# deryrahman/image-caption-emotion-indonesia

Measured on NVIDIA B200. Metric: decoder_train_tokens_per_sec, higher is better.
Workload: dtype bf16

## Files before the change

### image-caption-emotion-indonesia_b200/_lib.py

```python
import ctypes
import os
from ctypes import c_char_p, c_double, c_float, c_int32, c_int64, c_uint64, c_void_p

HERE = os.path.dirname(os.path.abspath(__file__))
LIB_PATH = os.path.join(HERE, "libsn100.so")

OP_NT, OP_NN, OP_TN = 0, 1, 2
CELL_FACTORED, CELL_LSTM = 0, 1

_P = c_void_p
_I32, _I64, _F, _D = c_int32, c_int64, c_float, c_double

SIGNATURES = {
    "sn_version": (_I32, []),
    "sn_last_error": (c_char_p, []),
    "sn_device_info": (_I32, [_P, _P, _P, _P]),
    "sn_gather_pack_fwd": (_I32, [_P, _I64, _P, _I64, _P, _I64, _I32, _P, _P, _P, _I64, _P, _I64, _F, c_uint64, _P, _P, _I64, _P]),
    "sn_gather_pack_bwd": (_I32, [_P, _I64, _P, _I64, _P, _I64, _I32, _P, _P, _P, _I64, _P, _I64, _F, c_uint64, _P, _I64, _P, _P, _P]),
    "sn_gemm": (_I32, [_I32, _I64, _I64, _I64, _P, _I64, _P, _I64, _P, _I64, _P, _F, _I32, _I64, _I64, _I64, _I64, _P]),
    "sn_gemm_bf16": (_I32, [_I32, _I64, _I64, _I64, _P, _I64, _P, _I64, _P, _I64, _P, _I64, _P, _F, _I32, _I64, _I64, _I64, _I64, _I64, _P]),
    "sn_gemm_bf16_splitk": (_I32, [_I32, _I64, _I64, _I64, _P, _I64, _P, _I64, _P, _I64, _P, _I64, _P, _F, _I32, _I64, _I64, _I64, _I64, _I64, _I32, _P]),
    "sn_gemm2_ws_bytes": (_I64, [_I64, _I64, _I32, _I32]),
    "sn_gemm2_bf16": (_I32, [_I32, _I64, _I64, _I64, _P, _I64, _P, _I64, _P, _I64, _P, _I64, _P, _F, _I32, _I64, _I64, _I64, _I64, _I64, _I32, _P, _I64, _I32, _P]),
    "sn_vocab_ws_bytes": (_I64, [_I64, _I64]),
    "sn_vocab_nll_fwd": (_I32, [_I64, _I64, _I64, _P, _I64, _P, _I64, _P, _P, _P, _I64, _P, _P, _P, _P, _P, _P]),
    "sn_vocab_nll_bwd": (_I32, [_I64, _I64, _I64, _P, _I64, _P, _I64, _P, _P, _P, _P, _F, _P, _P, _I64, _P, _P, _P]),
    "sn_cast_bf16": (_I32, [_P, _I64, _I64, _I64, _P, _I64, _I64, _P]),
    "sn_cast_bf16_ex": (_I32, [_P, _I64, _I64, _I64, _P, _I64, _I64, _I32, _P]),
    "sn_colsum": (_I32, [_P, _I64, _I64, _I64, _P, _F, _P]),
    "sn_colsum_ex": (_I32, [_P, _I64, _I64, _I64, _P, _F, _I32, _P]),
    "sn_colsum_bf16_ex": (_I32, [_P, _I64, _I64, _I64, _P, _F, _I32, _P]),
    "sn_embed_plan": (_I32, [_P, _I64, _I32, _P, _P, _P, _I64, _I64, _P, _P]),
    "sn_embed_grad": (_I32, [_P, _I64, _P, _I64, _I32, _P, _P, _P, _I64, _P, _I64, _F, c_uint64, _P, _I64, _P, _P, _I32, _P]),
    "sn_adam_clamp_dev_ex": (_I32, [_P, _P, _P, _P, _I32, _P, _P, _P, _P, _P, _F, _F, _F, _F, _I32, _P]),
    "sn_recur_ws_bytes": (_I64, [_I64, _I64]),
    "sn_recur_fwd": (_I32, [_I32, _I64, _I64, _P, _P, _I32, _I32, _P, _P, _P, _P, _P, _P, _P, _P, _P, _P, _P]),
    "sn_recur_bwd": (_I32, [_I32, _I64, _I64, _P, _P, _I32, _I32, _P, _P, _P, _P, _P, _P, _P, _P, _P, _P]),
    "sn_recur_fwd_bf16": (_I32, [_I32, _I64, _I64, _P, _P, _I32, _I32] + [_P] * 12),
    "sn_recur_bwd_bf16": (_I32, [_I32, _I64, _I64, _P, _P, _I32, _I32] + [_P] * 11),
    "sn_recur_cl_max_clusters": (_I32, [_I64]),
    "sn_recur_fwd_cl": (_I32, [_I32, _I64, _I64, _P, _P, _I32, _I32] + [_P] * 11),
    "sn_recur_bwd_cl": (_I32, [_I32, _I64, _I64, _P, _P, _I32, _I32] + [_P] * 11),
    "sn_gate_wait": (_I32, [_P, _I64, _P]),
    "sn_cast_bf16_gate_interleave": (_I32, [_P, _I64, _I64, _I64, _P, _I64, _P]),
    "sn_recur_fwd_gemm": (_I32, [_I32, _I64, _I64, _P, _P, _I32, _P, _P, _P, _P, _P, _P, _P, _P, _P]),
    "sn_recur_hprev": (_I32, [_P, _P, _P, _P, _I64, _I64, _P, _P]),
    "sn_recur_bwd_gemm": (_I32, [_I32, _I64, _I64, _P, _P, _I32, _P, _P, _P, _P, _P, _P, _P, _P, _P]),
    "sn_softmax_nll": (_I32, [_P, _I64, _I64, _I64, _P, _P, _P, _I64, _F, _P, _P, _P, _P, _I64, _P]),
    "sn_colsum_bf16": (_I32, [_P, _I64, _I64, _I64, _P, _F, _P]),
    "sn_reduce_sum": (_I32, [_P, _I64, _F, _P, _P, _I32, _P]),
    "sn_adam_clamp": (_I32, [_P, _P, _P, _P, _I32, _P, _P, _P, _F, _F, _F, _F, _P]),
    "sn_adam_clamp_dev": (_I32, [_P, _P, _P, _P, _I32, _P, _P, _P, _P, _P, _F, _F, _F, _F, _P]),
    "sn_enable_peer_access": (_I32, [_I32]),
    "sn_ipc_export": (_I32, [_P, _P, _P]),
    "sn_ipc_open": (_I32, [_P, _P]),
    "sn_ipc_close": (_I32, [_P]),
    "sn_dp_adam_fused": (_I32, [_I32, _I32, _P, _P, _P, _P, _P, _I32, _P, _P, _P, _P, _P, _F, _F, _F, _F, _P]),
    "sn_dp_slot_elems": (_I64, [_I64, _I32]),
    "sn_dp_push": (_I32, [_I32, _I32, _P, _P, _I64, _I32, _P, _I32, _P, _I32, _P]),
    "sn_dp_adam_recv": (_I32, [_I32, _I32, _P, _P, _P, _I64, _I32, _P, _P, _I32, _P, _P, _I32, _P, _P, _P, _P, _P, _F, _F, _F, _F, _I32, _P]),
    "sn_att_step_fwd": (_I32, [_P, _P, _P, _P, _F, _P, _I64, _I64, _I64, _I64, _P, _I64, _P, _I64, _P]),
    "sn_att_step_bwd": (_I32, [_P, _P, _P, _P, _F, _P, _P, _I64, _P, _I64, _P, _I64, _I64, _I64, _I64, _I64, _P, _P, _P, _P, _P, _P]),
    "sn_att_step_fwd_b16": (_I32, [_P, _P, _P, _P, _F, _P, _I64, _I64, _I64, _I64, _P, _I64, _P, _I64, _P]),
    "sn_att_step_bwd_b16": (_I32, [_P, _P, _P, _P, _P, _P, _I64, _P, _I64, _P, _I64, _I64, _I64, _I64, _I64, _P, _P, _P, _P, _P]),
    "sn_mean_pixels": (_I32, [_P, _I64, _I64, _I64, _P, _P]),
    "sn_beam_split_ws_floats": (_I64, [_I32, _I32, _I32]),
    "sn_beam_step_split": (_I32, [_P, _I64, _I64, _I32, _I32, _I32, _I32, _I32] + [_P] * 14 + [_I32, _P, _I32, _P]),
    "sn_split_limbs_cols": (_I32, [_P, _I64, _I64, _I64, _I64, _P, _I64, _I32, _P]),
    "sn_split_limbs_rows": (_I32, [_P, _I64, _I64, _I64, _I64, _P, _I64, _I64, _I32, _P]),
    "sn_skinny_max_rows": (_I32, []),
    "sn_skinny_linear": (_I32, [_P, _I64, _I64, _I64, _P, _I64, _I64, _I64, _I64, _P, _P, _I64, _P, _P]),
    "sn_decode_cell": (_I32, [_I32, _I64, _I64, _P, _I64, _I64, _P, _I64, _I64, _P, _P, _P, _P, _P, _P, _P, _P, _P, _P]),
    "sn_decode_cell_groups": (_I32, [_I32, _I64, _I64, _P, _I64, _P, _I64, _I64, _I64, _P, _I64, _I64, _P, _I64, _P, _P,
                                     _P, _P, _P, _P, _P, _P, _P]),
    "sn_pool_nhwc_fwd": (_I32, [_P, _I64, _I64, _I64, _I64, _I64, _P, _P, _P, _P]),
    "sn_pool_nhwc_bwd": (_I32, [_P, _I64, _I64, _I64, _I64, _I64, _P, _P]),
    "sn_bn1d_fwd": (_I32, [_P, _I64, _I64, _P, _P, _P, _P, _F, _F, _I32, _P, _P, _P, _P]),
    "sn_bn1d_bwd": (_I32, [_P, _P, _I64, _I64, _P, _P, _P, _I32, _P, _P, _P, _P]),
    "sn_beam_step": (_I32, [_P, _I64, _I64, _I32, _I32, _I32, _I32, _I32] + [_P] * 15),
    "sn_bleu_counts": (_I32, [_P, _P, _I64, _P, _P, _P, _I32, _I64, _P, _P]),
    "sn_cider_df": (_I32, [_P, _P, _P, _I64, _I32, _I32, _I64, _P, _P, _I64, _P, _P]),
    "sn_cider_scores": (_I32, [_P, _P, _I64, _P, _P, _P, _I32, _D, _I32, _I64, _P, _P, _I64, _P, _P, _P]),
    "sn_cider_scores_rows": (_I32, [_P, _I64, _P, _I64, _I32, _P, _I64, _P, _P, _P, _I32, _D, _I32, _I64, _P, _P, _I64,
                                    _P, _P]),
    "sn_rouge_l": (_I32, [_P, _P, _I64, _P, _P, _P, _I32, _D, _P, _P]),
    "sn_rouge_l_rows": (_I32, [_P, _I64, _P, _I64, _I32, _P, _I64, _P, _P, _P, _I32, _D, _P, _P]),
    "sn_sample_step": (_I32, [_P, _I64, _I64, _I32, _I32, _I32, _D, _I32] + [_P] * 9),
}

_lib = None


def load():
    global _lib
    if _lib is not None:
        return _lib
    if not os.path.exists(LIB_PATH):
        raise RuntimeError(
            "libsn100.so is not built (%s). Run `python -c 'import __graft_entry__ as g; g.build()'`; "
# ... 31 lines not shown
```

### image-caption-emotion-indonesia_b200/csrc/sn_common.cu

```cuda
#include <stdlib.h>

#include "sn_common.cuh"

#include <cuda.h>

#include <mutex>
#include <string.h>

namespace sn {

char* err_buf() {
  static thread_local char buf[512] = {0};
  return buf;
}

int32_t fail(int32_t code, const char* fmt, ...) {
  va_list ap;
  va_start(ap, fmt);
  vsnprintf(err_buf(), 512, fmt, ap);
  va_end(ap);
  return code;
}

int32_t check_launch(const char* what) {
  cudaError_t e = cudaGetLastError();
  if (e != cudaSuccess) return fail((int32_t)e, "%s: %s", what, cudaGetErrorString(e));
  return 0;
}

static DevInfo g_info[64];
static std::once_flag g_once[64];

const DevInfo& dev_info() {
  int dev = 0;
  cudaGetDevice(&dev);
  if (dev < 0 || dev >= 64) dev = 0;
  std::call_once(g_once[dev], [dev]() {
    DevInfo& d = g_info[dev];
    cudaDeviceGetAttribute(&d.sm_count, cudaDevAttrMultiProcessorCount, dev);
    cudaDeviceGetAttribute(&d.smem_optin, cudaDevAttrMaxSharedMemoryPerBlockOptin, dev);
    cudaDeviceGetAttribute(&d.cc_major, cudaDevAttrComputeCapabilityMajor, dev);
    cudaDeviceGetAttribute(&d.cc_minor, cudaDevAttrComputeCapabilityMinor, dev);
  });
  return g_info[dev];
}

}

namespace sn {
bool recur_cooperative() {
  static const bool coop = [] {
    const char* e = getenv("SN_RECUR_COOP");
    return e && e[0] == '1';
  }();
  return coop;
}
}

extern "C" {

int32_t sn_version(void) { return SN_VERSION; }
const char* sn_last_error(void) { return sn::err_buf(); }

int32_t sn_device_info(int32_t* sm_count, int32_t* smem_optin, int32_t* cc_major, int32_t* cc_minor) {
  int n = 0;
  cudaError_t e = cudaGetDeviceCount(&n);
  if (e != cudaSuccess || n == 0) return sn::fail(e ? (int32_t)e : -2, "no CUDA device (libsn100 has no CPU fallback)");
  const sn::DevInfo& d = sn::dev_info();
  if (sm_count) *sm_count = d.sm_count;
  if (smem_optin) *smem_optin = d.smem_optin;
  if (cc_major) *cc_major = d.cc_major;
  if (cc_minor) *cc_minor = d.cc_minor;
  if (d.cc_major != 10) return sn::fail(-3, "device is sm_%d%d; libsn100 is built for sm_100a only", d.cc_major, d.cc_minor);
  return 0;
}

int32_t sn_ipc_export(const void* ptr, uint8_t* handle64, int64_t* offset) {
  SN_REQUIRE(ptr && handle64 && offset, "sn_ipc_export: null argument");
  CUdeviceptr base = 0;
  size_t size = 0;
  typedef CUresult (*RangeFn)(CUdeviceptr*, size_t*, CUdeviceptr);
  static RangeFn range_fn = nullptr;
  if (!range_fn) {
    void* fp = nullptr;
    cudaDriverEntryPointQueryResult q;
    if (cudaGetDriverEntryPoint("cuMemGetAddressRange", &fp, cudaEnableDefault, &q) != cudaSuccess || !fp)
      return sn::fail(-6, "cuMemGetAddressRange entry point not available");
    range_fn = (RangeFn)fp;
  }
  CUresult r = range_fn(&base, &size, (CUdeviceptr)ptr);
  if (r != CUDA_SUCCESS) return sn::fail(-6, "cuMemGetAddressRange failed (%d)", (int)r);
  cudaIpcMemHandle_t h;
  cudaError_t e = cudaIpcGetMemHandle(&h, (void*)base);
  if (e != cudaSuccess) return sn::fail((int32_t)e, "cudaIpcGetMemHandle: %s (expandable segments are not IPC-exportable)", cudaGetErrorString(e));
  memcpy(handle64, &h, sizeof(h));
  *offset = (int64_t)((CUdeviceptr)ptr - base);
  return 0;
}

int32_t sn_ipc_open(const uint8_t* handle64, void** base_out) {
  SN_REQUIRE(handle64 && base_out, "sn_ipc_open: null argument");
  cudaIpcMemHandle_t h;
  memcpy(&h, handle64, sizeof(h));
  cudaError_t e = cudaIpcOpenMemHandle(base_out, h, cudaIpcMemLazyEnablePeerAccess);
  if (e != cudaSuccess) return sn::fail((int32_t)e, "cudaIpcOpenMemHandle: %s", cudaGetErrorString(e));
  return 0;
}

int32_t sn_ipc_close(void* base) {
  cudaError_t e = cudaIpcCloseMemHandle(base);
  if (e != cudaSuccess) return sn::fail((int32_t)e, "cudaIpcCloseMemHandle: %s", cudaGetErrorString(e));
  return 0;
}

}
```

### image-caption-emotion-indonesia_b200/csrc/sn_common.cuh

```cuda
#pragma once
#include <cuda_runtime.h>
#include <stdint.h>
#include <stdio.h>
#include <stdarg.h>

#include "../../include/sn100.h"

namespace sn {

char* err_buf();
int32_t fail(int32_t code, const char* fmt, ...);
int32_t check_launch(const char* what);

struct DevInfo {
  int sm_count;
  int smem_optin;
  int cc_major, cc_minor;
};
const DevInfo& dev_info();
bool recur_cooperative();

#define SN_REQUIRE(cond, ...)                         \
  do {                                                \
    if (!(cond)) return sn::fail(-1, __VA_ARGS__);    \
  } while (0)

#define SN_CUDA(expr)                                                           \
  do {                                                                          \
    cudaError_t e__ = (expr);                                                   \
    if (e__ != cudaSuccess)                                                     \
      return sn::fail((int32_t)e__, "%s: %s", #expr, cudaGetErrorString(e__));  \
  } while (0)

__device__ __forceinline__ float sigmoidf_(float x) { return 1.0f / (1.0f + expf(-x)); }

__device__ __forceinline__ float warp_sum(float v) {
#pragma unroll
  for (int o = 16; o > 0; o >>= 1) v += __shfl_xor_sync(0xffffffffu, v, o);
  return v;
}
__device__ __forceinline__ float warp_max(float v) {
#pragma unroll
  for (int o = 16; o > 0; o >>= 1) v = fmaxf(v, __shfl_xor_sync(0xffffffffu, v, o));
  return v;
}

__device__ __forceinline__ uint32_t hash_u32(uint64_t seed, uint32_t row, uint32_t col) {
  uint64_t x = seed ^ ((uint64_t)row << 32 | col);
  x ^= x >> 33; x *= 0xff51afd7ed558ccdULL;
  x ^= x >> 33; x *= 0xc4ceb9fe1a85ec53ULL;
  x ^= x >> 33;
  return (uint32_t)x;
}
__device__ __forceinline__ float dropout_scale(uint64_t seed, uint32_t row, uint32_t col, float p,
                                               float inv_keep) {
  if (p <= 0.f) return 1.f;
  float u = (hash_u32(seed, row, col) >> 8) * (1.0f / 16777216.0f);
  return u >= p ? inv_keep : 0.f;
}

__device__ __forceinline__ int ld_acquire(const int* p) {
  int v;
  asm volatile("ld.acquire.gpu.global.s32 %0, [%1];" : "=r"(v) : "l"(p) : "memory");
  return v;
}
__device__ __forceinline__ void red_release_add(int* p, int v) {
  asm volatile("red.release.gpu.global.add.s32 [%0], %1;" ::"l"(p), "r"(v) : "memory");
}

}
```

### image-caption-emotion-indonesia_b200/csrc/sn_elementwise.cu

```cuda
#include <stdlib.h>
#include <string.h>
#include <cuda_bf16.h>

#include "sn_common.cuh"

namespace {

__global__ void gather_pack_fwd_kernel(const int64_t* __restrict__ captions, int64_t cap_ld,
                                       const float* __restrict__ table, int E,
                                       const float* __restrict__ features, int64_t feat_ld, int has_feat,
                                       const int32_t* __restrict__ row_b, const int32_t* __restrict__ row_t,
                                       const int32_t* __restrict__ tok_override, int64_t N,
                                       float* __restrict__ X, int64_t ldx, float p, float inv_keep,
                                       uint64_t seed, const uint64_t* __restrict__ seed_dev,
                                       __nv_bfloat16* __restrict__ Xb, int64_t ldxb, int Ep) {
  if (seed_dev) seed += *seed_dev;
  int64_t row = (int64_t)blockIdx.x * (blockDim.x >> 5) + (threadIdx.x >> 5);
  if (row >= N) return;
  int lane = threadIdx.x & 31;
  int b = row_b[row], t = row_t[row];
  int ov = tok_override ? tok_override[row] : -1;
  float* dst = X ? X + row * ldx : nullptr;
  __nv_bfloat16* dstb = Xb ? Xb + row * ldxb : nullptr;
  const float* src;
  float pp = 0.f;
  if (ov < 0 && has_feat && t == 0) {
    src = features + (int64_t)b * feat_ld;
  } else {
    int64_t tok = ov >= 0 ? (int64_t)ov : captions[(int64_t)b * cap_ld + (t - has_feat)];
    src = table + tok * E;
    pp = ov >= 0 ? 0.f : p;
  }
  for (int c = lane; c < Ep; c += 32) {
    float v = c < E ? src[c] * sn::dropout_scale(seed, (uint32_t)row, (uint32_t)c, pp, inv_keep) : 0.f;
    if (dst && c < E) dst[c] = v;
    if (dstb) dstb[c] = __float2bfloat16(v);
  }
}

__global__ void gather_pack_bwd_kernel(const int64_t* __restrict__ captions, int64_t cap_ld,
                                       float* __restrict__ dtable, int E, float* __restrict__ dfeatures,
                                       int64_t feat_ld, int has_feat, const int32_t* __restrict__ row_b,
                                       const int32_t* __restrict__ row_t,
                                       const int32_t* __restrict__ tok_override, int64_t N,
                                       const float* __restrict__ dX, int64_t ldx, float p, float inv_keep,
                                       uint64_t seed, const uint64_t* __restrict__ seed_dev) {
  if (seed_dev) seed += *seed_dev;
  int64_t row = (int64_t)blockIdx.x * (blockDim.x >> 5) + (threadIdx.x >> 5);
  if (row >= N) return;
  int lane = threadIdx.x & 31;
  int b = row_b[row], t = row_t[row];
  int ov = tok_override ? tok_override[row] : -1;
  const float* src = dX + row * ldx;
  if (ov < 0 && has_feat && t == 0) {
    if (dfeatures) {
      float* dst = dfeatures + (int64_t)b * feat_ld;
      for (int c = lane; c < E; c += 32) dst[c] = src[c];
    }
    return;
  }
}

__device__ __forceinline__ int64_t packed_token(int64_t i, const int64_t* __restrict__ captions, int64_t cap_ld,
                                                int has_feat, const int32_t* __restrict__ row_b,
                                                const int32_t* __restrict__ row_t,
                                                const int32_t* __restrict__ tok_override) {
  int ov = tok_override ? tok_override[i] : -1;
  if (ov >= 0) return ov;
  int t = row_t[i];
  if (has_feat && t == 0) return -1;
  return captions[(int64_t)row_b[i] * cap_ld + (t - has_feat)];
}

constexpr int EB_CHUNK = 32;
constexpr int EB_K = 16;

__global__ void embed_count_kernel(const int64_t* __restrict__ captions, int64_t cap_ld, int has_feat,
                                   const int32_t* __restrict__ row_b, const int32_t* __restrict__ row_t,
                                   const int32_t* __restrict__ tok_override, int64_t N, int32_t* __restrict__ tok32,
                                   int32_t* __restrict__ cnt) {
  const int64_t r = (int64_t)blockIdx.x * blockDim.x + threadIdx.x;
  if (r >= N) return;
  const int64_t t = packed_token(r, captions, cap_ld, has_feat, row_b, row_t, tok_override);
  tok32[r] = (int32_t)t;
  if (t >= 0) atomicAdd(cnt + t, 1);
}

__global__ void __launch_bounds__(1024) embed_scan_kernel(const int32_t* __restrict__ cnt, int64_t V,
                                                          int32_t* __restrict__ start, int32_t* __restrict__ cursor,
                                                          int32_t* __restrict__ cstart) {
  __shared__ int32_t s1[1024], s2[1024];
  const int tid = threadIdx.x;
  const int64_t per = (V + 1023) / 1024, lo = tid * per, hi = lo + per < V ? lo + per : V;
  int32_t a = 0, c = 0;
  for (int64_t v = lo; v < hi; ++v) {
    const int32_t n = cnt[v];
    a += n;
    c += n > EB_CHUNK ? (n + EB_CHUNK - 1) / EB_CHUNK : 0;
// ... 3 lines not shown
  for (int off = 1; off < 1024; off <<= 1) {
    const int32_t x = tid >= off ? s1[tid - off] : 0, y = tid >= off ? s2[tid - off] : 0;
    __syncthreads();
    s1[tid] += x; s2[tid] += y;
    __syncthreads();
  }
  a = s1[tid] - a; c = s2[tid] - c;
  for (int64_t v = lo; v < hi; ++v) {
    const int32_t n = cnt[v];
    start[v] = a; cursor[v] = a; cstart[v] = c;
    a += n;
    c += n > EB_CHUNK ? (n + EB_CHUNK - 1) / EB_CHUNK : 0;
  }
  if (tid == 1023) start[V] = s1[1023];
}

__global__ void embed_place_kernel(const int32_t* __restrict__ tok32, int64_t N, int32_t* __restrict__ cursor,
                                   int32_t* __restrict__ perm) {
  const int64_t r = (int64_t)blockIdx.x * blockDim.x + threadIdx.x;
  if (r >= N) return;
  const int32_t t = tok32[r];
  if (t >= 0) perm[atomicAdd(cursor + t, 1)] = (int32_t)r;
}

__global__ void embed_order_kernel(const int32_t* __restrict__ tok32, const int32_t* __restrict__ start,
                                   const int32_t* __restrict__ perm, int64_t N, int64_t V,
                                   int32_t* __restrict__ sorted) {
  const int64_t i = (int64_t)blockIdx.x * blockDim.x + threadIdx.x;
  if (i >= start[V]) return;
  const int32_t r = perm[i], t = tok32[r], s = start[t], e = start[t + 1];
  int32_t rank = 0;
  for (int32_t j = s; j < e; ++j) rank += perm[j] < r;
  sorted[s + rank] = r;
}

__global__ void embed_chunk_kernel(const int32_t* __restrict__ tok32, const int32_t* __restrict__ start,
                                   const int32_t* __restrict__ cstart, const int32_t* __restrict__ sorted, int64_t V,
                                   const int32_t* __restrict__ tok_override, const float* __restrict__ dX, int64_t ldx,
                                   int E, float p, float inv_keep, uint64_t seed, const uint64_t* __restrict__ seed_dev,
                                   float* __restrict__ dtable, float* __restrict__ part) {
  if (seed_dev) seed += *seed_dev;
  const int64_t i = (int64_t)blockIdx.x * (blockDim.x >> 5) + (threadIdx.x >> 5);
  if (i >= start[V]) return;
  const int lane = threadIdx.x & 31;
  const int32_t t = tok32[sorted[i]], s = start[t], e = start[t + 1];
  if ((i - s) % EB_CHUNK) return;
  const int32_t n = (int32_t)(e - i < EB_CHUNK ? e - i : EB_CHUNK);
  const int32_t my = lane < n ? sorted[i + lane] : 0;
  float* dst = e - s <= EB_CHUNK ? dtable + (int64_t)t * E : part + (int64_t)(cstart[t] + (i - s) / EB_CHUNK) * E;
  for (int c0 = 0; c0 < E; c0 += 32 * EB_K) {
    float acc[EB_K];
#pragma unroll
    for (int k = 0; k < EB_K; ++k) acc[k] = 0.f;
    for (int q = 0; q < n; ++q) {
      const int64_t j = __shfl_sync(0xffffffffu, my, q);
      const float pp = (tok_override && tok_override[j] >= 0) ? 0.f : p;
      const float* src = dX + j * ldx;
#pragma unroll
      for (int k = 0; k < EB_K; ++k) {
        const int c = c0 + k * 32 + lane;
        if (c < E) {
          const float sc = sn::dropout_scale(seed, (uint32_t)j, (uint32_t)c, pp, inv_keep);
          if (sc != 0.f) acc[k] += src[c] * sc;
        }
      }
    }
#pragma unroll
    for (int k = 0; k < EB_K; ++k) {
      const int c = c0 + k * 32 + lane;
      if (c < E) {
        if (e - s <= EB_CHUNK) dst[c] += acc[k];
        else dst[c] = acc[k];
      }
    }
  }
}

constexpr int EBW_BATCH = 16;
__global__ void __launch_bounds__(512) embed_chunk_wide_kernel(
    const int32_t* __restrict__ tok32, const int32_t* __restrict__ start, const int32_t* __restrict__ cstart,
    const int32_t* __restrict__ sorted, int64_t V, const int32_t* __restrict__ tok_override,
    const float* __restrict__ dX, int64_t ldx, int E, float p, float inv_keep, uint64_t seed,
    const uint64_t* __restrict__ seed_dev, float* __restrict__ dtable, float* __restrict__ part) {
  __shared__ int32_t rows[EB_CHUNK];
  __shared__ float rate[EB_CHUNK];
  const int64_t i = blockIdx.x;
  if (i >= start[V]) return;
  const int32_t t = tok32[sorted[i]], s = start[t], e = start[t + 1];
  if ((i - s) % EB_CHUNK) return;
  if (seed_dev) seed += *seed_dev;
  const int32_t n = (int32_t)(e - i < EB_CHUNK ? e - i : EB_CHUNK);
  if (threadIdx.x < n) {
    const int32_t j = sorted[i + threadIdx.x];
    rows[threadIdx.x] = j;
    rate[threadIdx.x] = (tok_override && tok_override[j] >= 0) ? 0.f : p;
  }
  __syncthreads();
  const int c = threadIdx.x;
  if (c >= E) return;
  float acc = 0.f;
  for (int q0 = 0; q0 < n; q0 += EBW_BATCH) {
    float x[EBW_BATCH], sc[EBW_BATCH];
#pragma unroll
    for (int u = 0; u < EBW_BATCH; ++u) {
      const int q = q0 + u;
      x[u] = 0.f; sc[u] = 0.f;
      if (q < n) {
        const int64_t j = rows[q];
        x[u] = dX[j * ldx + c];
        sc[u] = sn::dropout_scale(seed, (uint32_t)j, (uint32_t)c, rate[q], inv_keep);
      }
    }
#pragma unroll
    for (int u = 0; u < EBW_BATCH; ++u)
      if (sc[u] != 0.f) acc = __fmaf_rn(x[u], sc[u], acc);
  }
  if (e - s <= EB_CHUNK) dtable[(int64_t)t * E + c] += acc;
  else part[(int64_t)(cstart[t] + (i - s) / EB_CHUNK) * E + c] = acc;
}

__global__ void embed_combine_kernel(const int32_t* __restrict__ cnt, const int32_t* __restrict__ cstart, int64_t V,
                                     int E, const float* __restrict__ part, float* __restrict__ dtable) {
  const int64_t t = (int64_t)blockIdx.x * (blockDim.x >> 5) + (threadIdx.x >> 5);
  if (t >= V || cnt[t] <= EB_CHUNK) return;
  const int lane = threadIdx.x & 31;
  const int32_t nq = (cnt[t] + EB_CHUNK - 1) / EB_CHUNK;
  const float* src = part + (int64_t)cstart[t] * E;
  for (int c = lane; c < E; c += 32) {
    float a = 0.f;
    for (int32_t q = 0; q < nq; ++q) a += src[(int64_t)q * E + c];
    dtable[t * E + c] += a;
  }
}

__global__ void __launch_bounds__(256) softmax_nll_kernel(const float* __restrict__ logits, int64_t V, int64_t ld,
                                                          const int64_t* __restrict__ targets,
                                                          float* __restrict__ row_loss, float* dlogits, int64_t ldd,
                                                          float grad_scale, const float* __restrict__ row_weight,
                                                          int64_t* __restrict__ argmax,
                                                          int32_t* __restrict__ top5hit, int use_smem,
                                                          __nv_bfloat16* __restrict__ dlb, int64_t lddb) {
  extern __shared__ float srow[];
  __shared__ float red_v[8];
  __shared__ int red_i[8];
  __shared__ float bc_f[2];
  __shared__ int bc_i;
  const int64_t row = blockIdx.x;
  const float* src = logits + row * ld;
  const int tid = threadIdx.x, lane = tid & 31, warp = tid >> 5;

  float mx = -INFINITY;
  int mi = 0x7fffffff;
  for (int64_t c = tid; c < V; c += 256) {
    float v = src[c];
    if (use_smem) srow[c] = v;
    if (v > mx) { mx = v; mi = (int)c; }
  }
#pragma unroll
  for (int o = 16; o > 0; o >>= 1) {
    float ov = __shfl_xor_sync(0xffffffffu, mx, o);
    int oi = __shfl_xor_sync(0xffffffffu, mi, o);
    if (ov > mx || (ov == mx && oi < mi)) { mx = ov; mi = oi; }
  }
  if (lane == 0) { red_v[warp] = mx; red_i[warp] = mi; }
  __syncthreads();
  if (tid == 0) {
    float bm = red_v[0]; int bi = red_i[0];
    for (int w = 1; w < 8; ++w)
      if (red_v[w] > bm || (red_v[w] == bm && red_i[w] < bi)) { bm = red_v[w]; bi = red_i[w]; }
    bc_f[0] = bm; bc_i = bi;
  }
  __syncthreads();
  mx = bc_f[0];
  if (tid == 0 && argmax) argmax[row] = bc_i;
  if (!targets) return;

  const float* rd = use_smem ? srow : src;
  const int64_t tgt = targets[row];
  const float tv = rd[tgt];
  float se = 0.f;
  int above = 0;
  for (int64_t c = tid; c < V; c += 256) {
    float v = rd[c];
    se += expf(v - mx);
    above += (v > tv);
  }
  se = sn::warp_sum(se);
#pragma unroll
  for (int o = 16; o > 0; o >>= 1) above += __shfl_xor_sync(0xffffffffu, above, o);
  __syncthreads();
  if (lane == 0) { red_v[warp] = se; red_i[warp] = above; }
  __syncthreads();
  if (tid == 0) {
    float s = 0.f; int a = 0;
    for (int w = 0; w < 8; ++w) { s += red_v[w]; a += red_i[w]; }
    float lse = mx + logf(s);
    bc_f[1] = lse;
    if (row_loss) row_loss[row] = lse - tv;
    if (top5hit) top5hit[row] = a < 5 ? 1 : 0;
  }
  __syncthreads();
  if (dlogits || dlb) {
    const float lse = bc_f[1];
    const float gs = row_weight ? grad_scale * row_weight[row] : grad_scale;
    float* dst = dlogits ? dlogits + row * ldd : nullptr;
    __nv_bfloat16* dstb = dlb ? dlb + row * lddb : nullptr;
    for (int64_t c = tid; c < V; c += 256) {
      float pr = expf(rd[c] - lse);
      float gr = (pr - (c == tgt ? 1.f : 0.f)) * gs;
      if (dst) dst[c] = gr;
      if (dstb) dstb[c] = __float2bfloat16(gr);
    }
    if (dstb) for (int64_t c = V + tid; c < lddb; c += 256) dstb[c] = __float2bfloat16(0.f);
  }
}

__global__ void __launch_bounds__(1024) reduce_sum_kernel(const float* __restrict__ x, int64_t N, float scale,
                                                           const float* __restrict__ w, float* out, int accumulate) {
  __shared__ double part[32];
  double s = 0.0;
  if (w)
    for (int64_t i = threadIdx.x; i < N; i += 1024) s += (double)x[i] * (double)w[i];
  else
    for (int64_t i = threadIdx.x; i < N; i += 1024) s += (double)x[i];
#pragma unroll
  for (int o = 16; o > 0; o >>= 1) s += __shfl_xor_sync(0xffffffffu, s, o);
  if ((threadIdx.x & 31) == 0) part[threadIdx.x >> 5] = s;
  __syncthreads();
  if (threadIdx.x == 0) {
    double t = 0.0;
    for (int w = 0; w < 32; ++w) t += part[w];
    float r = (float)(t * (double)scale);
    *out = accumulate ? *out + r : r;
  }
}

struct AdamRanges {
  static constexpr int MAX = 128;
  int64_t off[MAX];
  int32_t len[MAX];
  float step_size[MAX], bc2_sqrt[MAX];
  int step_idx[MAX];
  int32_t chunk_start[MAX + 1];
  int n;
};
static_assert(sizeof(AdamRanges) <= 3700, "AdamRanges must leave room for the other kernel parameters below 4 KB");

__global__ void adam_prepare_kernel(AdamRanges R, int32_t* __restrict__ steps, const float* __restrict__ lr,
                                    float* __restrict__ coef, float beta1, float beta2) {
  int r = threadIdx.x;
  if (r >= R.n) return;
  int st = steps[R.step_idx[r]] + 1;
  steps[R.step_idx[r]] = st;
  double bc1 = 1.0 - pow((double)beta1, (double)st);
  double bc2 = 1.0 - pow((double)beta2, (double)st);
  coef[2 * R.step_idx[r]] = (float)((double)(*lr) / bc1);
  coef[2 * R.step_idx[r] + 1] = (float)sqrt(bc2);
}
constexpr int ADAM_CHUNK = 4096;
constexpr int64_t ADAM_MAX_LEN = (1LL << 31) - 2 * ADAM_CHUNK;

__global__ void __launch_bounds__(256) adam_clamp_kernel(float* __restrict__ p, float* __restrict__ g,
                                                         float* __restrict__ m, float* __restrict__ v,
                                                         AdamRanges R, const float* __restrict__ coef, float beta1,
                                                         float beta2, float eps, float clip) {
  const int64_t total_chunks = R.chunk_start[R.n];
  for (int64_t ch = blockIdx.x; ch < total_chunks; ch += gridDim.x) {
    int r = 0;
    while (ch >= R.chunk_start[r + 1]) ++r;
    const int64_t base = R.off[r] + (ch - R.chunk_start[r]) * ADAM_CHUNK;
    const int64_t end = R.off[r] + R.len[r];
    const float ss = coef ? coef[2 * R.step_idx[r]] : R.step_size[r], bc = coef ? coef[2 * R.step_idx[r] + 1] : R.bc2_sqrt[r];
    const int64_t lim = base + ADAM_CHUNK < end ? base + ADAM_CHUNK : end;
    if ((base & 3) == 0 && lim - base == ADAM_CHUNK) {
#pragma unroll
      for (int it = 0; it < ADAM_CHUNK / (256 * 4); ++it) {
        const int64_t i = base + (int64_t)(it * 256 + threadIdx.x) * 4;
        float4 g4 = *reinterpret_cast<const float4*>(g + i);
        float4 m4 = *reinterpret_cast<const float4*>(m + i);
        float4 v4 = *reinterpret_cast<const float4*>(v + i);
        float4 p4 = *reinterpret_cast<const float4*>(p + i);
        float* gp = &g4.x; float* mp = &m4.x; float* vp = &v4.x; float* pp = &p4.x;
#pragma unroll
        for (int e = 0; e < 4; ++e) {
          float gi = gp[e];
          if (clip > 0.f) gi = fminf(fmaxf(gi, -clip), clip);
          gp[e] = gi;
          float mi = mp[e] + (1.f - beta1) * (gi - mp[e]);
          float vi = vp[e] * beta2 + (1.f - beta2) * gi * gi;
          float denom = sqrtf(vi) / bc + eps;
          pp[e] = pp[e] - ss * (mi / denom);
          mp[e] = mi; vp[e] = vi;
        }
        if (clip > 0.f) *reinterpret_cast<float4*>(g + i) = g4;
        *reinterpret_cast<float4*>(m + i) = m4;
        *reinterpret_cast<float4*>(v + i) = v4;
        *reinterpret_cast<float4*>(p + i) = p4;
      }
      continue;
    }
    for (int64_t i = base + threadIdx.x; i < lim; i += 256) {
      float gi = g[i];
      if (clip > 0.f) { gi = fminf(fmaxf(gi, -clip), clip); g[i] = gi; }
      float mi = m[i], vi = v[i];
      mi = mi + (1.f - beta1) * (gi - mi);
      vi = vi * beta2 + (1.f - beta2) * gi * gi;
      float denom = sqrtf(vi) / bc + eps;
      p[i] = p[i] - ss * (mi / denom);
      m[i] = mi; v[i] = vi;
    }
  }
}

struct DpPeers {
  float* grad[8];
  float* param[8];
  int* pad[8];
  int world, rank;
  void* recv[8];
  int64_t slot_elems;
  int* wait_pad[4];
  int n_wait;
};
constexpr int PAD_ARRIVE = 0, PAD_DONE = 8, PAD_COUNTER = 16, PAD_EPOCH = 17, PAD_DONE_COUNTER = 18;

__device__ __forceinline__ int ld_acquire_sys(const int* p) {
  int v;
  asm volatile("ld.acquire.sys.global.s32 %0, [%1];" : "=r"(v) : "l"(p) : "memory");
  return v;
}
__device__ __forceinline__ void st_release_sys(int* p, int v) {
  asm volatile("st.release.sys.global.s32 [%0], %1;" ::"l"(p), "r"(v) : "memory");
}

constexpr int DP_SUB = 4;
template <typename TT>
__global__ void __launch_bounds__(256 * DP_SUB) dp_push_kernel(DpPeers P, AdamRanges R, const float* __restrict__ g) {
  const int W = P.world;
  __shared__ int s_last;
  int* mypad = P.pad[P.rank];
  const int64_t total_chunks = R.chunk_start[R.n];
  const int sub = threadIdx.x >> 8, tid = threadIdx.x & 255;
  for (int64_t ch = (int64_t)blockIdx.x * DP_SUB + sub; ch < total_chunks; ch += (int64_t)gridDim.x * DP_SUB) {
    int r = 0;
    while (ch >= R.chunk_start[r + 1]) ++r;
    const int64_t aid = R.off[r] / ADAM_CHUNK + (ch - R.chunk_start[r]);
    const int owner = (int)(aid % W);
    if (owner == P.rank) continue;
// ... 204 lines not shown
#pragma unroll
        for (int k = 0; k < 4; ++k) {
          float gi = gp[k];
          if (clip > 0.f) gi = fminf(fmaxf(gi, -clip), clip);
          const float mi = mp[k] + (1.f - beta1) * (gi - mp[k]);
          const float vi = vp[k] * beta2 + (1.f - beta2) * gi * gi;
          pp[k] = pp[k] - ss * (mi / (sqrtf(vi) / bc + eps));
          mp[k] = mi; vp[k] = vi;
        }
        *reinterpret_cast<float4*>(m + i) = m4;
        *reinterpret_cast<float4*>(v + i) = v4;
#pragma unroll
        for (int q = 0; q < W; ++q) *reinterpret_cast<float4*>(P.param[q] + i) = p4;
      }
      continue;
    }
    for (int64_t i = base + tid; i < lim; i += 256) {
      float gi = 0.f;
#pragma unroll
      for (int q = 0; q < W; ++q) {
        float gq;
        if (q == rank) gq = __ldcg(g + i);
        else if constexpr (sizeof(TT) == 4) gq = __ldcg(recv + q * P.slot_elems + rbase + i);
        else gq = __bfloat162float(recv[q * P.slot_elems + rbase + i]);
        gi = q == 0 ? gq : gi + gq;
      }
      if (clip > 0.f) gi = fminf(fmaxf(gi, -clip), clip);
      const float mi = m[i] + (1.f - beta1) * (gi - m[i]);
      const float vi = v[i] * beta2 + (1.f - beta2) * gi * gi;
      const float pn = p_loc[i] - ss * (mi / (sqrtf(vi) / bc + eps));
      m[i] = mi; v[i] = vi;
#pragma unroll
      for (int q = 0; q < W; ++q) P.param[q][i] = pn;
    }
  }
  __syncthreads();
  if (threadIdx.x == 0) {
    __threadfence_system();
    s_last = (atomicAdd(mypad + PAD_DONE_COUNTER, 1) == (int)gridDim.x - 1);
  }
  __syncthreads();
  if (s_last) {
    if (threadIdx.x == 0) __threadfence_system();
    __syncthreads();
    if (threadIdx.x < W) {
      st_release_sys(P.pad[threadIdx.x] + PAD_DONE + rank, e);
      while (ld_acquire_sys(mypad + PAD_DONE + threadIdx.x) < e) { }
    }
    __syncthreads();
    if (threadIdx.x == 0) {
      mypad[PAD_DONE_COUNTER] = 0; mypad[PAD_EPOCH] = e;
      for (int k = 1; k < P.n_wait; ++k) P.wait_pad[k][PAD_EPOCH] = P.wait_pad[k][PAD_EPOCH] + 1;
    }
  }
}

__global__ void mean_pixels_kernel(const float* __restrict__ feat, int64_t P, int64_t D, float* __restrict__ out) {
  int64_t b = blockIdx.y;
  int64_t d = (int64_t)blockIdx.x * blockDim.x + threadIdx.x;
  if (d >= D) return;
  const float* src = feat + b * P * D + d;
  float s = 0.f;
  for (int64_t pz = 0; pz < P; ++pz) s += src[pz * D];
  out[b * D + d] = s / (float)P;
}

}

extern "C" {

int32_t sn_gather_pack_fwd(const int64_t* captions, int64_t cap_ld, const float* table, int64_t E,
                           const float* features, int64_t feat_ld, int32_t has_feat,
                           const int32_t* row_b, const int32_t* row_t, const int32_t* tok_override,
                           int64_t N, float* X, int64_t ldx, float p_drop, uint64_t seed, const uint64_t* seed_dev,
                           void* Xb, int64_t ldxb, void* stream) {
  SN_REQUIRE(N >= 0 && E > 0 && (X || Xb), "sn_gather_pack_fwd: bad dims N=%lld E=%lld", (long long)N, (long long)E);
  SN_REQUIRE(!X || ldx >= E, "sn_gather_pack_fwd: ldx=%lld < E", (long long)ldx);
  SN_REQUIRE(!Xb || ldxb >= E, "sn_gather_pack_fwd: ldxb=%lld < E", (long long)ldxb);
  SN_REQUIRE(p_drop >= 0.f && p_drop < 1.f, "sn_gather_pack_fwd: dropout p=%f out of [0,1)", p_drop);
  SN_REQUIRE(!has_feat || features, "sn_gather_pack_fwd: has_feat without features");
  if (N == 0) return 0;
  float inv_keep = 1.f / (1.f - p_drop);
  unsigned grid = (unsigned)((N + 7) / 8);
  gather_pack_fwd_kernel<<<grid, 256, 0, (cudaStream_t)stream>>>(captions, cap_ld, table, (int)E, features, feat_ld,
                                                                 has_feat, row_b, row_t, tok_override, N, X, ldx,
                                                                 p_drop, inv_keep, seed, seed_dev,
                                                                 (__nv_bfloat16*)Xb, ldxb, Xb ? (int)ldxb : (int)E);
  return sn::check_launch("sn_gather_pack_fwd");
}

int32_t sn_gather_pack_bwd(const int64_t* captions, int64_t cap_ld, float* dtable, int64_t E,
                           float* dfeatures, int64_t feat_ld, int32_t has_feat, const int32_t* row_b,
                           const int32_t* row_t, const int32_t* tok_override, int64_t N,
                           const float* dX, int64_t ldx, float p_drop, uint64_t seed, const uint64_t* seed_dev,
                           int64_t V, int32_t* ws_int, float* ws_part, void* stream) {
  SN_REQUIRE(N >= 0 && E > 0 && ldx >= E && V > 0, "sn_gather_pack_bwd: bad dims");
  SN_REQUIRE(p_drop >= 0.f && p_drop < 1.f, "sn_gather_pack_bwd: dropout p=%f out of [0,1)", p_drop);
  SN_REQUIRE(N < (int64_t)1 << 30, "sn_gather_pack_bwd: N=%lld rows", (long long)N);
  if (N == 0) return 0;
  SN_REQUIRE(ws_int && ws_part, "sn_gather_pack_bwd: null work space");
  if (int32_t rc = sn_embed_plan(captions, cap_ld, has_feat, row_b, row_t, tok_override, N, V, ws_int, stream)) return rc;
  return sn_embed_grad(dtable, E, dfeatures, feat_ld, has_feat, row_b, row_t, tok_override, N, dX, ldx, p_drop, seed,
                       seed_dev, V, ws_int, ws_part, 0, stream);
}

namespace {
struct EmbedWs {
  int32_t *cnt, *start, *cursor, *cstart, *tok32, *perm, *sorted;
  EmbedWs(int32_t* ws, int64_t V, int64_t N)
      : cnt(ws), start(cnt + V), cursor(start + V + 1), cstart(cursor + V), tok32(cstart + V), perm(tok32 + N),
        sorted(perm + N) {}
};
}

int32_t sn_embed_plan(const int64_t* captions, int64_t cap_ld, int32_t has_feat, const int32_t* row_b,
                      const int32_t* row_t, const int32_t* tok_override, int64_t N, int64_t V, int32_t* ws_int,
                      void* stream) {
  SN_REQUIRE(N >= 0 && N < (int64_t)1 << 30 && V > 0, "sn_embed_plan: bad dims N=%lld V=%lld", (long long)N, (long long)V);
  if (N == 0) return 0;
  SN_REQUIRE(ws_int, "sn_embed_plan: null work space");
  cudaStream_t st = (cudaStream_t)stream;
  EmbedWs w(ws_int, V, N);
  SN_CUDA(cudaMemsetAsync(w.cnt, 0, sizeof(int32_t) * (size_t)V, st));
  const unsigned g_rows = (unsigned)((N + 255) / 256);
  embed_count_kernel<<<g_rows, 256, 0, st>>>(captions, cap_ld, has_feat, row_b, row_t, tok_override, N, w.tok32, w.cnt);
  embed_scan_kernel<<<1, 1024, 0, st>>>(w.cnt, V, w.start, w.cursor, w.cstart);
  embed_place_kernel<<<g_rows, 256, 0, st>>>(w.tok32, N, w.cursor, w.perm);
  embed_order_kernel<<<g_rows, 256, 0, st>>>(w.tok32, w.start, w.perm, N, V, w.sorted);
  return sn::check_launch("sn_embed_plan");
}

int32_t sn_embed_grad(float* dtable, int64_t E, float* dfeatures, int64_t feat_ld, int32_t has_feat,
                      const int32_t* row_b, const int32_t* row_t, const int32_t* tok_override, int64_t N,
                      const float* dX, int64_t ldx, float p_drop, uint64_t seed, const uint64_t* seed_dev, int64_t V,
                      const int32_t* ws_int, float* ws_part, int32_t wide, void* stream) {
  SN_REQUIRE(N >= 0 && N < (int64_t)1 << 30 && E > 0 && ldx >= E && V > 0, "sn_embed_grad: bad dims");
  SN_REQUIRE(p_drop >= 0.f && p_drop < 1.f, "sn_embed_grad: dropout p=%f out of [0,1)", p_drop);
  if (N == 0) return 0;
  SN_REQUIRE(ws_int && ws_part, "sn_embed_grad: null work space");
  cudaStream_t st = (cudaStream_t)stream;
  float inv_keep = 1.f / (1.f - p_drop);
  if (has_feat && dfeatures)
    gather_pack_bwd_kernel<<<(unsigned)((N + 7) / 8), 256, 0, st>>>(nullptr, 0, dtable, (int)E, dfeatures,
                                                                     feat_ld, has_feat, row_b, row_t, tok_override, N,
                                                                     dX, ldx, p_drop, inv_keep, seed, seed_dev);
  EmbedWs w(const_cast<int32_t*>(ws_int), V, N);
  if (wide && E <= 512)
    embed_chunk_wide_kernel<<<(unsigned)N, (unsigned)((E + 31) / 32 * 32), 0, st>>>(
        w.tok32, w.start, w.cstart, w.sorted, V, tok_override, dX, ldx, (int)E, p_drop, inv_keep, seed, seed_dev,
        dtable, ws_part);
  else
    embed_chunk_kernel<<<(unsigned)((N + 7) / 8), 256, 0, st>>>(w.tok32, w.start, w.cstart, w.sorted, V, tok_override,
                                                                 dX, ldx, (int)E, p_drop, inv_keep, seed, seed_dev,
                                                                 dtable, ws_part);
  embed_combine_kernel<<<(unsigned)((V + 7) / 8), 256, 0, st>>>(w.cnt, w.cstart, V, (int)E, ws_part, dtable);
  return sn::check_launch("sn_embed_grad");
}

int32_t sn_softmax_nll(const float* logits, int64_t N, int64_t V, int64_t ld, const int64_t* targets,
                       float* row_loss, float* dlogits, int64_t ldd, float grad_scale, const float* row_weight,
                       int64_t* argmax, int32_t* top5hit, void* dlogits_bf16, int64_t lddb, void* stream) {
  SN_REQUIRE(N >= 0 && V > 0 && ld >= V, "sn_softmax_nll: bad dims");
  SN_REQUIRE(!dlogits_bf16 || lddb >= V, "sn_softmax_nll: lddb < V");
  if (N == 0) return 0;
  size_t smem = (size_t)V * sizeof(float);
  int use_smem = smem <= 200 * 1024;
  if (use_smem && smem > 48 * 1024) {
    static thread_local size_t configured = 0;
    if (configured < smem) {
      SN_CUDA(cudaFuncSetAttribute(softmax_nll_kernel, cudaFuncAttributeMaxDynamicSharedMemorySize, 200 * 1024));
      configured = 200 * 1024;
    }
  }
  softmax_nll_kernel<<<(unsigned)N, 256, use_smem ? smem : 0, (cudaStream_t)stream>>>(
      logits, V, ld, targets, row_loss, dlogits, ldd, grad_scale, row_weight, argmax, top5hit, use_smem,
      (__nv_bfloat16*)dlogits_bf16, lddb);
  return sn::check_launch("sn_softmax_nll");
}

int32_t sn_reduce_sum(const float* x, int64_t N, float scale, const float* row_weight, float* out, int32_t accumulate,
                      void* stream) {
  SN_REQUIRE(N >= 0 && out, "sn_reduce_sum: bad args");
  reduce_sum_kernel<<<1, 1024, 0, (cudaStream_t)stream>>>(x, N, scale, row_weight, out, accumulate);
  return sn::check_launch("sn_reduce_sum");
}

int32_t sn_adam_clamp(float* p, float* g, float* m, float* v, int32_t n_ranges, const int64_t* ranges,
                      const float* step_size, const float* bc2_sqrt, float beta1, float beta2, float eps,
                      float clip, void* stream) {
  SN_REQUIRE(n_ranges >= 0, "sn_adam_clamp: n_ranges < 0");
  int done = 0;
  while (done < n_ranges) {
    AdamRanges R;
    R.n = 0;
    R.chunk_start[0] = 0;
    while (done < n_ranges && R.n < AdamRanges::MAX) {
      int64_t off = ranges[2 * done], len = ranges[2 * done + 1];
      SN_REQUIRE(off >= 0 && len >= 0 && len < ADAM_MAX_LEN, "sn_adam_clamp: bad range %d", done);
      R.off[R.n] = off; R.len[R.n] = (int32_t)len;
      R.step_size[R.n] = step_size[done]; R.bc2_sqrt[R.n] = bc2_sqrt[done];
      R.chunk_start[R.n + 1] = R.chunk_start[R.n] + (len + ADAM_CHUNK - 1) / ADAM_CHUNK;
      ++R.n; ++done;
    }
    int64_t chunks = R.chunk_start[R.n];
    if (chunks == 0) continue;
    int64_t cap = (int64_t)sn::dev_info().sm_count * 8;
    unsigned grid = (unsigned)(chunks < cap ? chunks : cap);
    adam_clamp_kernel<<<grid, 256, 0, (cudaStream_t)stream>>>(p, g, m, v, R, nullptr, beta1, beta2, eps, clip);
    int32_t rc = sn::check_launch("sn_adam_clamp");
    if (rc) return rc;
  }
  return 0;
}

int32_t sn_adam_clamp_dev(float* p, float* g, float* m, float* v, int32_t n_ranges, const int64_t* ranges,
                          const int32_t* step_idx, int32_t* steps_dev, const float* lr_dev, float* coef_ws,
                          float beta1, float beta2, float eps, float clip, void* stream) {
  return sn_adam_clamp_dev_ex(p, g, m, v, n_ranges, ranges, step_idx, steps_dev, lr_dev, coef_ws, beta1, beta2, eps,
                              clip, 0, stream);
}

int32_t sn_adam_clamp_dev_ex(float* p, float* g, float* m, float* v, int32_t n_ranges, const int64_t* ranges,
                             const int32_t* step_idx, int32_t* steps_dev, const float* lr_dev, float* coef_ws,
                             float beta1, float beta2, float eps, float clip, int32_t max_ctas, void* stream) {
  SN_REQUIRE(max_ctas >= 0, "sn_adam_clamp_dev: max_ctas < 0");
  SN_REQUIRE(n_ranges >= 0 && n_ranges <= AdamRanges::MAX, "sn_adam_clamp_dev: at most %d ranges per call", AdamRanges::MAX);
  SN_REQUIRE(steps_dev && lr_dev && coef_ws, "sn_adam_clamp_dev: null argument");
  if (n_ranges == 0) return 0;
  AdamRanges R;
  R.n = n_ranges;
  R.chunk_start[0] = 0;
  for (int i = 0; i < n_ranges; ++i) {
    SN_REQUIRE(ranges[2 * i] >= 0 && ranges[2 * i + 1] >= 0 && ranges[2 * i + 1] < ADAM_MAX_LEN, "sn_adam_clamp_dev: bad range %d", i);
    R.off[i] = ranges[2 * i]; R.len[i] = (int32_t)ranges[2 * i + 1]; R.step_idx[i] = step_idx[i];
    R.step_size[i] = 0.f; R.bc2_sqrt[i] = 1.f;
    R.chunk_start[i + 1] = R.chunk_start[i] + (R.len[i] + ADAM_CHUNK - 1) / ADAM_CHUNK;
  }
  cudaStream_t st = (cudaStream_t)stream;
  adam_prepare_kernel<<<1, AdamRanges::MAX, 0, st>>>(R, steps_dev, lr_dev, coef_ws, beta1, beta2);
  int64_t chunks = R.chunk_start[R.n];
  if (chunks == 0) return sn::check_launch("sn_adam_clamp_dev");
  int64_t cap = (int64_t)sn::dev_info().sm_count * 8;
  if (max_ctas > 0 && max_ctas < cap) cap = max_ctas;
  unsigned grid = (unsigned)(chunks < cap ? chunks : cap);
  adam_clamp_kernel<<<grid, 256, 0, st>>>(p, g, m, v, R, coef_ws, beta1, beta2, eps, clip);
  return sn::check_launch("sn_adam_clamp_dev");
}

int32_t sn_enable_peer_access(int32_t peer_device) {
  int cur = 0;
  SN_CUDA(cudaGetDevice(&cur));
  if (peer_device == cur) return 0;
  int can = 0;
  SN_CUDA(cudaDeviceCanAccessPeer(&can, cur, peer_device));
  SN_REQUIRE(can, "sn_enable_peer_access: device %d cannot access peer %d", cur, peer_device);
  cudaError_t e = cudaDeviceEnablePeerAccess(peer_device, 0);
  if (e == cudaErrorPeerAccessAlreadyEnabled) { cudaGetLastError(); return 0; }
  if (e != cudaSuccess) return sn::fail((int32_t)e, "cudaDeviceEnablePeerAccess(%d): %s", peer_device, cudaGetErrorString(e));
  return 0;
}

int32_t sn_dp_adam_fused(int32_t world, int32_t rank, void* const* grad_ptrs, void* const* param_ptrs,
                         void* const* pad_ptrs, float* m, float* v, int32_t n_ranges, const int64_t* ranges,
                         const int32_t* step_idx, int32_t* steps_dev, const float* lr_dev, float* coef_ws, float beta1,
                         float beta2, float eps, float clip, void* stream) {
  SN_REQUIRE(world >= 1 && world <= 8 && rank >= 0 && rank < world, "sn_dp_adam_fused: bad world/rank %d/%d", world, rank);
  SN_REQUIRE(n_ranges >= 0 && n_ranges <= AdamRanges::MAX, "sn_dp_adam_fused: at most %d ranges per call", AdamRanges::MAX);
  SN_REQUIRE(grad_ptrs && param_ptrs && pad_ptrs && steps_dev && lr_dev && coef_ws && m && v, "sn_dp_adam_fused: null argument");
  DpPeers P;
  memset(&P, 0, sizeof(P));
  P.world = world; P.rank = rank;
  for (int q = 0; q < 8; ++q) {
    P.grad[q] = q < world ? (float*)grad_ptrs[q] : nullptr;
    P.param[q] = q < world ? (float*)param_ptrs[q] : nullptr;
    P.pad[q] = q < world ? (int*)pad_ptrs[q] : nullptr;
    SN_REQUIRE(q >= world || (P.grad[q] && P.param[q] && P.pad[q]), "sn_dp_adam_fused: null peer pointer %d", q);
  }
  AdamRanges R;
  R.n = n_ranges;
  R.chunk_start[0] = 0;
  for (int i = 0; i < n_ranges; ++i) {
    SN_REQUIRE(ranges[2 * i] >= 0 && ranges[2 * i + 1] >= 0 && ranges[2 * i + 1] < ADAM_MAX_LEN, "sn_dp_adam_fused: bad range %d", i);
    R.off[i] = ranges[2 * i]; R.len[i] = (int32_t)ranges[2 * i + 1]; R.step_idx[i] = step_idx[i];
    R.step_size[i] = 0.f; R.bc2_sqrt[i] = 1.f;
    R.chunk_start[i + 1] = R.chunk_start[i] +
        (R.len[i] > 0 ? (R.off[i] + R.len[i] - 1) / ADAM_CHUNK - R.off[i] / ADAM_CHUNK + 1 : 0);
  }
  cudaStream_t st = (cudaStream_t)stream;
  if (n_ranges > 0) adam_prepare_kernel<<<1, AdamRanges::MAX, 0, st>>>(R, steps_dev, lr_dev, coef_ws, beta1, beta2);
  int64_t mine = (R.chunk_start[R.n] + world - 1) / world;
  int64_t cap = (int64_t)sn::dev_info().sm_count * 3;
  unsigned grid = (unsigned)(mine < 1 ? 1 : (mine < cap ? mine : cap));
  static const int dbg = [] { const char* e = getenv("SN_DP_DEBUG"); return e ? atoi(e) : 0; }();
#define SN_DP_LAUNCH(WW) dp_adam_fused_kernel<WW><<<grid, 256, 0, st>>>(P, R, coef_ws, m, v, beta1, beta2, eps, clip, dbg)
  switch (world) {
    case 1: SN_DP_LAUNCH(1); break;
    case 2: SN_DP_LAUNCH(2); break;
    case 3: SN_DP_LAUNCH(3); break;
    case 4: SN_DP_LAUNCH(4); break;
    case 5: SN_DP_LAUNCH(5); break;
    case 6: SN_DP_LAUNCH(6); break;
    case 7: SN_DP_LAUNCH(7); break;
    default: SN_DP_LAUNCH(8); break;
  }
#undef SN_DP_LAUNCH
  return sn::check_launch("sn_dp_adam_fused");
}

static int32_t dp_fill_ranges(AdamRanges& R, int32_t n_ranges, const int64_t* ranges, const int32_t* step_idx, const char* who) {
  SN_REQUIRE(n_ranges >= 0 && n_ranges <= AdamRanges::MAX, "%s: at most %d ranges per call", who, AdamRanges::MAX);
  R.n = n_ranges;
  R.chunk_start[0] = 0;
  for (int i = 0; i < n_ranges; ++i) {
    SN_REQUIRE(ranges[2 * i] >= 0 && ranges[2 * i + 1] >= 0 && ranges[2 * i + 1] < ADAM_MAX_LEN, "%s: bad range %d", who, i);
    R.off[i] = ranges[2 * i]; R.len[i] = (int32_t)ranges[2 * i + 1]; R.step_idx[i] = step_idx ? step_idx[i] : 0;
    R.step_size[i] = 0.f; R.bc2_sqrt[i] = 1.f;
    R.chunk_start[i + 1] = R.chunk_start[i] +
        (R.len[i] > 0 ? (R.off[i] + R.len[i] - 1) / ADAM_CHUNK - R.off[i] / ADAM_CHUNK + 1 : 0);
  }
  return 0;
}

int64_t sn_dp_slot_elems(int64_t arena_elems, int32_t world) {
  if (arena_elems < 0 || world < 1) return -1;
  int64_t chunks = (arena_elems + ADAM_CHUNK - 1) / ADAM_CHUNK;
  return ((chunks + world - 1) / world) * ADAM_CHUNK;
}

int32_t sn_dp_push(int32_t world, int32_t rank, const float* grad, void* const* recv_ptrs, int64_t slot_elems,
                   int32_t elem_size, void* const* pad_ptrs, int32_t n_ranges, const int64_t* ranges, int32_t max_ctas,
                   void* stream) {
  SN_REQUIRE(world >= 1 && world <= 8 && rank >= 0 && rank < world, "sn_dp_push: bad world/rank %d/%d", world, rank);
  SN_REQUIRE(grad && recv_ptrs && pad_ptrs && ranges, "sn_dp_push: null argument");
  SN_REQUIRE(elem_size == 4 || elem_size == 2, "sn_dp_push: elem_size must be 4 (fp32) or 2 (bf16)");
  SN_REQUIRE(slot_elems > 0 && slot_elems % ADAM_CHUNK == 0, "sn_dp_push: slot_elems must be a positive multiple of %d", ADAM_CHUNK);
  DpPeers P;
  memset(&P, 0, sizeof(P));
  P.world = world; P.rank = rank; P.slot_elems = slot_elems;
  for (int q = 0; q < world; ++q) {
    P.recv[q] = recv_ptrs[q]; P.pad[q] = (int*)pad_ptrs[q];
    SN_REQUIRE(P.recv[q] && P.pad[q], "sn_dp_push: null peer pointer %d", q);
  }
  AdamRanges R;
  if (int32_t rc = dp_fill_ranges(R, n_ranges, ranges, nullptr, "sn_dp_push")) return rc;
  for (int i = 0; i < n_ranges; ++i)
    SN_REQUIRE(R.len[i] == 0 || (R.off[i] + R.len[i] - 1) / ADAM_CHUNK / world < slot_elems / ADAM_CHUNK,
               "sn_dp_push: range %d does not fit the receive slots", i);
  int64_t chunks = R.chunk_start[R.n];
  int64_t cap = (int64_t)sn::dev_info().sm_count;
  if (max_ctas > 0 && max_ctas < cap) cap = max_ctas;
  int64_t want = (chunks + DP_SUB - 1) / DP_SUB;
  unsigned grid = (unsigned)(want < 1 ? 1 : (want < cap ? want : cap));
  cudaStream_t st = (cudaStream_t)stream;
  if (elem_size == 4) dp_push_kernel<float><<<grid, 256 * DP_SUB, 0, st>>>(P, R, grad);
  else dp_push_kernel<__nv_bfloat16><<<grid, 256 * DP_SUB, 0, st>>>(P, R, grad);
  return sn::check_launch("sn_dp_push");
}

int32_t sn_dp_adam_recv(int32_t world, int32_t rank, float* grad, void* const* param_ptrs, void* recv, int64_t slot_elems,
                        int32_t elem_size, void* const* pad_ptrs, void* const* wait_pads, int32_t n_wait, float* m, float* v,
                        int32_t n_ranges, const int64_t* ranges, const int32_t* step_idx, int32_t* steps_dev,
                        const float* lr_dev, float* coef_ws, float beta1, float beta2, float eps, float clip,
                        int32_t max_ctas, void* stream) {
  SN_REQUIRE(world >= 1 && world <= 8 && rank >= 0 && rank < world, "sn_dp_adam_recv: bad world/rank %d/%d", world, rank);
  SN_REQUIRE(grad && param_ptrs && recv && pad_ptrs && wait_pads && steps_dev && lr_dev && coef_ws && m && v && ranges && step_idx,
             "sn_dp_adam_recv: null argument");
  SN_REQUIRE(elem_size == 4 || elem_size == 2, "sn_dp_adam_recv: elem_size must be 4 (fp32) or 2 (bf16)");
  SN_REQUIRE(n_wait >= 1 && n_wait <= 4, "sn_dp_adam_recv: 1..4 push buckets per call (got %d)", n_wait);
  SN_REQUIRE(slot_elems > 0 && slot_elems % ADAM_CHUNK == 0, "sn_dp_adam_recv: slot_elems must be a positive multiple of %d", ADAM_CHUNK);
  SN_REQUIRE(n_ranges >= 1, "sn_dp_adam_recv: no ranges");
  DpPeers P;
  memset(&P, 0, sizeof(P));
  P.world = world; P.rank = rank; P.slot_elems = slot_elems; P.n_wait = n_wait;
  for (int q = 0; q < world; ++q) {
    P.param[q] = (float*)param_ptrs[q]; P.pad[q] = (int*)pad_ptrs[q];
    SN_REQUIRE(P.param[q] && P.pad[q], "sn_dp_adam_recv: null peer pointer %d", q);
  }
  P.grad[rank] = grad;
  P.recv[rank] = recv;
  for (int k = 0; k < n_wait; ++k) {
    P.wait_pad[k] = (int*)wait_pads[k];
    SN_REQUIRE(P.wait_pad[k], "sn_dp_adam_recv: null wait pad %d", k);
  }
  SN_REQUIRE(P.wait_pad[0] == P.pad[rank], "sn_dp_adam_recv: pad_ptrs must be every rank's pad of wait bucket 0");
  AdamRanges R;
  if (int32_t rc = dp_fill_ranges(R, n_ranges, ranges, step_idx, "sn_dp_adam_recv")) return rc;
  for (int i = 0; i < n_ranges; ++i) {
    int64_t own = 0;
    if (R.len[i] > 0) {
      const int64_t a0 = R.off[i] / ADAM_CHUNK, a1 = (R.off[i] + R.len[i] - 1) / ADAM_CHUNK;
      const int64_t first = a0 + ((rank - a0) % world + world) % world;
      own = first <= a1 ? (a1 - first) / world + 1 : 0;
      SN_REQUIRE(a1 / world < slot_elems / ADAM_CHUNK, "sn_dp_adam_recv: range %d does not fit the receive slots", i);
    }
    R.chunk_start[i + 1] = R.chunk_start[i] + own;
  }
  cudaStream_t st = (cudaStream_t)stream;
  adam_prepare_kernel<<<1, AdamRanges::MAX, 0, st>>>(R, steps_dev, lr_dev, coef_ws, beta1, beta2);
  int64_t mine = (R.chunk_start[R.n] + DP_RSUB - 1) / DP_RSUB;
  int64_t cap = (int64_t)sn::dev_info().sm_count * 2;
  if (max_ctas > 0 && max_ctas < cap) cap = max_ctas;
  unsigned grid = (unsigned)(mine < 1 ? 1 : (mine < cap ? mine : cap));
  const float* p_loc = P.param[rank];
#define SN_DP_LAUNCH(WW)                                                                                                   \
  if (elem_size == 4) dp_recv_adam_kernel<WW, float><<<grid, 256 * DP_RSUB, 0, st>>>(P, R, coef_ws, grad, (const float*)recv, p_loc, m, v, beta1, beta2, eps, clip); \
  else dp_recv_adam_kernel<WW, __nv_bfloat16><<<grid, 256 * DP_RSUB, 0, st>>>(P, R, coef_ws, grad, (const __nv_bfloat16*)recv, p_loc, m, v, beta1, beta2, eps, clip)
  switch (world) {
    case 1: SN_DP_LAUNCH(1); break;
    case 2: SN_DP_LAUNCH(2); break;
    case 3: SN_DP_LAUNCH(3); break;
    case 4: SN_DP_LAUNCH(4); break;
    case 5: SN_DP_LAUNCH(5); break;
    case 6: SN_DP_LAUNCH(6); break;
    case 7: SN_DP_LAUNCH(7); break;
    default: SN_DP_LAUNCH(8); break;
  }
#undef SN_DP_LAUNCH
  return sn::check_launch("sn_dp_adam_recv");
}

int32_t sn_mean_pixels(const float* feat, int64_t B, int64_t P, int64_t D, float* out, void* stream) {
  SN_REQUIRE(B >= 0 && P > 0 && D > 0, "sn_mean_pixels: bad dims");
  if (B == 0) return 0;
  dim3 grid((unsigned)((D + 255) / 256), (unsigned)B);
  mean_pixels_kernel<<<grid, 256, 0, (cudaStream_t)stream>>>(feat, P, D, out);
  return sn::check_launch("sn_mean_pixels");
}

}
```

### image-caption-emotion-indonesia_b200/csrc/sn_gemm2.cu

```cuda
#include <cuda.h>
#include <cuda_bf16.h>
#include <math.h>
#include <math_constants.h>

#include "sn_common.cuh"

namespace {

constexpr int BMC = 128;
constexpr int BM = 2 * BMC;
constexpr int BN = 256;
constexpr int BK = 64;
constexpr int UMMA_K = 16;
constexpr int A_BYTES = BMC * BK * 2;
constexpr int ACC_STAGES = 2;
constexpr int EPI_WARPS = 16;
constexpr int NTHREADS = 64 + 32 * EPI_WARPS;
constexpr int XPOSE_BYTES = 32 * 32 * 4;
template <int BN_>
struct Geo {
  static constexpr int BNC = BN_ / 2;
  static constexpr int B_BYTES = BNC * BK * 2;
  static constexpr int STAGE_BYTES = A_BYTES + B_BYTES;
  static constexpr int STAGES = BN_ == 256 ? 5 : 6;
// ... 174 lines not shown
  __syncwarp();
  const int u = lane & 3;
  const int n8 = nb + 8 * u;
#pragma unroll
  for (int i = 0; i < 4; ++i) {
    const int r = 8 * i + (lane >> 2);
    const uint4 pk = *reinterpret_cast<const uint4*>(buf + r * 64 + ((u ^ ((r >> 1) & 3)) << 4));
    const int rr = row0 + r;
    if (rr >= M || n8 >= ncols) continue;
    __nv_bfloat16* dst = base + (int64_t)rr * ld + n8;
    if (vec_ok && n8 + 8 <= ncols) {
      *reinterpret_cast<uint4*>(dst) = pk;
    } else {
      const __nv_bfloat16* e = reinterpret_cast<const __nv_bfloat16*>(&pk);
#pragma unroll
      for (int k = 0; k < 8; ++k)
        if (n8 + k < ncols) dst[k] = e[k];
    }
  }
}

struct Tile { int m0, n0, grp, split, kb0, nkb; };

__device__ __forceinline__ Tile decode_tile(const G2Args& g, int tile, int tiles_m, int tiles_n, int total_kb, int bn) {
  Tile t;
  int mt, nt, rest;
  if (g.M > g.N) {
    nt = tile % tiles_n; rest = tile / tiles_n;
    mt = rest % tiles_m; rest /= tiles_m;
  } else {
    mt = tile % tiles_m; rest = tile / tiles_m;
    nt = rest % tiles_n; rest /= tiles_n;
  }
  t.split = rest % g.splits;
  t.grp = rest / g.splits;
  t.m0 = mt * BM;
  t.n0 = nt * bn;
  if (g.splits == 1) {
    t.kb0 = 0; t.nkb = total_kb;
  } else {
    t.kb0 = (total_kb * t.split) / g.splits;
    t.nkb = (total_kb * (t.split + 1)) / g.splits - t.kb0;
  }
  return t;
}


template <int EPI, int BN_>
__global__ void __cluster_dims__(2, 1, 1) __launch_bounds__(NTHREADS, 1)
gemm2_kernel(const __grid_constant__ TmaSet tma_a, const __grid_constant__ TmaSet tma_b, const G2Args g) {
  constexpr int BNC = Geo<BN_>::BNC, B_BYTES = Geo<BN_>::B_BYTES, STAGE_BYTES = Geo<BN_>::STAGE_BYTES;
  constexpr int STAGES = Geo<BN_>::STAGES, TMEM_COLS = Geo<BN_>::TMEM_COLS, EPI_COLS = Geo<BN_>::EPI_COLS;
  extern __shared__ uint8_t smem_raw[];
  uint8_t* smem = reinterpret_cast<uint8_t*>((reinterpret_cast<uintptr_t>(smem_raw) + 1023) & ~(uintptr_t)1023);
  float* xpose0 = reinterpret_cast<float*>(smem + STAGES * STAGE_BYTES);
  uint64_t* bars = reinterpret_cast<uint64_t*>(smem + STAGES * STAGE_BYTES + EPI_WARPS * XPOSE_BYTES);
  uint32_t* tmem_slot = reinterpret_cast<uint32_t*>(bars + 2 * STAGES + 2 * ACC_STAGES);
  const uint32_t smem_base = smem_u32(smem);
  const uint32_t full0 = smem_u32(bars), empty0 = smem_u32(bars + STAGES);
  const uint32_t tfull0 = smem_u32(bars + 2 * STAGES), tempty0 = smem_u32(bars + 2 * STAGES + ACC_STAGES);
  const int warp = threadIdx.x >> 5, lane = threadIdx.x & 31;
  const uint32_t rank = cluster_ctarank();
  const int pair = blockIdx.x >> 1, npairs = gridDim.x >> 1;
  const int tiles_m = (g.M + BM - 1) / BM, tiles_n = (g.N + BN_ - 1) / BN_;
  const int total_tiles = tiles_m * tiles_n * g.groups * g.splits;
  const int total_kb = (g.K + BK - 1) / BK;

  if (threadIdx.x == 0) {
    for (int s = 0; s < STAGES; ++s) { mbar_init(full0 + 8 * s, 1); mbar_init(empty0 + 8 * s, 1); }
    for (int s = 0; s < ACC_STAGES; ++s) { mbar_init(tfull0 + 8 * s, 1); mbar_init(tempty0 + 8 * s, 2 * EPI_WARPS); }
    asm volatile("fence.mbarrier_init.release.cluster;" ::: "memory");
  }
  if (warp == 0 && lane == 0) {
    for (int i = 0; i < g.groups; ++i) {
      asm volatile("prefetch.tensormap [%0];" ::"l"(&tma_a.m[i]) : "memory");
      asm volatile("prefetch.tensormap [%0];" ::"l"(&tma_b.m[i]) : "memory");
    }
  }
  if (warp == 1) tmem_alloc2(smem_u32(tmem_slot), TMEM_COLS);
  tc_fence_before();
  cluster_sync();
  tc_fence_after();
  const uint32_t tmem_base = *tmem_slot;

  if (warp == 0) {
    if (lane == 0) {
      int s = 0;
      uint32_t ph = 0;
      for (int tile = pair; tile < total_tiles; tile += npairs) {
        const Tile t = decode_tile(g, tile, tiles_m, tiles_n, total_kb, BN_);
        const CUtensorMap* map_a = &tma_a.m[t.grp];
        const CUtensorMap* map_b = &tma_b.m[t.grp];
        const int m0 = t.m0 + (int)rank * BMC, n0 = t.n0 + (int)rank * BNC;
        int k0 = t.kb0 * BK;
        for (int kb = 0; kb < t.nkb; ++kb, k0 += BK) {
          mbar_wait(empty0 + 8 * s, ph ^ 1);
          const uint32_t sa = smem_base + s * STAGE_BYTES, sb = sa + A_BYTES;
          const uint32_t lbar = mapa(full0 + 8 * s, 0);
          if (rank == 0) mbar_expect_tx(full0 + 8 * s, 2 * STAGE_BYTES);
          if (!g.a_mn_major) {
            tma_load_2d_2sm(sa, map_a, lbar, k0, m0);
          } else {
            tma_load_2d_2sm(sa, map_a, lbar, m0, k0);
            tma_load_2d_2sm(sa + A_BYTES / 2, map_a, lbar, m0 + 64, k0);
          }
          if (!g.b_mn_major) {
            tma_load_2d_2sm(sb, map_b, lbar, k0, n0);
          } else {
            tma_load_2d_2sm(sb, map_b, lbar, n0, k0);
            if (BNC == 128) tma_load_2d_2sm(sb + B_BYTES / 2, map_b, lbar, n0 + 64, k0);
          }
          if (++s == STAGES) { s = 0; ph ^= 1; }
        }
      }
    }
  } else if (warp == 1) {
    if (rank == 0 && lane == 0) {
      const uint32_t idesc = (1u << 4) | (1u << 7) | (1u << 10) | ((uint32_t)g.a_mn_major << 15) |
                             ((uint32_t)g.b_mn_major << 16) | ((uint32_t)(BN_ >> 3) << 17) | ((uint32_t)(BM >> 4) << 24);
      const uint64_t adesc0 = g.a_mn_major ? make_desc(smem_base, A_BYTES / 2, 1024) : make_desc(smem_base, 16, 1024);
      const uint64_t bdesc0 = g.b_mn_major ? make_desc(smem_base + A_BYTES, BNC == 128 ? B_BYTES / 2 : 16, 1024)
                                           : make_desc(smem_base + A_BYTES, 16, 1024);
      const uint64_t astep = (g.a_mn_major ? 2048 : 32) >> 4, bstep = (g.b_mn_major ? 2048 : 32) >> 4;
      int s = 0, as = 0;
      uint32_t ph = 0, aph = 0;
      for (int tile = pair; tile < total_tiles; tile += npairs) {
        const Tile t = decode_tile(g, tile, tiles_m, tiles_n, total_kb, BN_);
        mbar_wait_cluster(tempty0 + 8 * as, aph ^ 1);
        tc_fence_after();
        const uint32_t tmem_d = tmem_base + (uint32_t)(as * BN_);
        for (int kb = 0; kb < t.nkb; ++kb) {
          mbar_wait(full0 + 8 * s, ph);
          tc_fence_after();
          const uint64_t ad = adesc0 + (uint64_t)(s * (STAGE_BYTES >> 4)), bd = bdesc0 + (uint64_t)(s * (STAGE_BYTES >> 4));
          umma2_bf16(tmem_d, ad, bd, idesc, kb ? 1u : 0u);
#pragma unroll
          for (int k = 1; k < BK / UMMA_K; ++k) umma2_bf16(tmem_d, ad + k * astep, bd + k * bstep, idesc, 1u);
          umma2_commit_mc(empty0 + 8 * s);
          if (kb == t.nkb - 1) umma2_commit_mc(tfull0 + 8 * as);
          if (++s == STAGES) { s = 0; ph ^= 1; }
        }
        if (++as == ACC_STAGES) { as = 0; aph ^= 1; }
      }
    }
    __syncwarp();
  } else {
    const int q = warp & 3;
    const int slice = (warp - 2) >> 2;
    float* xbuf = xpose0 + (warp - 2) * (XPOSE_BYTES / 4);
    const uint32_t tempty_leader0 = mapa(tempty0, 0);
    int acc_it = 0;
    for (int tile = pair; tile < total_tiles; tile += npairs, ++acc_it) {
      const Tile t = decode_tile(g, tile, tiles_m, tiles_n, total_kb, BN_);
      const int as = acc_it & 1;
      const uint32_t aph = (acc_it >> 1) & 1;
      if (EPI == EPI_CELL_FWD || EPI == EPI_CELL_BWD) {
        const int H = g.Hdim;
        const int prow0 = t.m0 + (int)rank * BMC + q * 32;
        if (EPI == EPI_CELL_FWD) {
          const int U0 = t.n0 >> 2;
          for (int idx = lane; idx < 80; idx += 32) {
            const int ph = idx / 40, rem = idx - ph * 40, k = rem / 5, a = rem - k * 5;
            const int rr = prow0 + slice * 8 + k;
            const float* p = a < 4 ? g.xp + (int64_t)rr * 4 * H + a * H + U0 + 32 * ph
                                   : (g.c_prev ? g.c_prev + (int64_t)rr * H + U0 + 32 * ph : nullptr);
            if (rr < g.M && p) prefetch_l2(p);
          }
        } else {
          const int u0 = t.n0 + slice * EPI_COLS;
          for (int idx = lane; idx < 32 * 8; idx += 32) {
            const int rr = prow0 + (idx >> 3), a = idx & 7;
            const float* p = a < 4 ? g.gates_in + (int64_t)rr * 4 * H + a * H + u0
                           : a == 4 ? g.c_cur + (int64_t)rr * H + u0
                           : a == 5 ? (g.c_prev ? g.c_prev + (int64_t)rr * H + u0 : nullptr)
                           : a == 6 ? g.dh_in + (int64_t)rr * H + u0 : g.dc_carry + (int64_t)rr * H + u0;
            if (rr < g.M && u0 < g.N && p) prefetch_l2(p);
          }
        }
      }
      mbar_wait(tfull0 + 8 * as, aph);
      tc_fence_after();
      const int row0 = t.m0 + (int)rank * BMC + q * 32;
      const int row = row0 + lane;
      const int ncol0 = t.n0 + slice * EPI_COLS;
      const uint32_t taddr = tmem_base + ((uint32_t)(q * 32) << 16) + (uint32_t)(as * BN_ + slice * EPI_COLS);
      const bool row_ok = row < g.M;

      if (EPI == EPI_STORE || EPI == EPI_PARTIAL) {
        float* Cg = nullptr;
        __nv_bfloat16* Cbg = nullptr;
        const float* bias = nullptr;
        int64_t ldc = g.ldc;
        float beta = 0.f;
        if (EPI == EPI_PARTIAL) {
          Cg = g.ws + (int64_t)(t.grp * g.splits + t.split) * g.M * g.N;
          ldc = g.N;
        } else {
          Cg = g.C ? g.C + t.grp * g.strideC : nullptr;
          Cbg = g.Cb ? g.Cb + t.grp * g.strideCb : nullptr;
          bias = g.bias ? g.bias + t.grp * g.strideBias : nullptr;
          beta = g.beta;
        }
        const bool vec_c = Cg && ((ldc & 3) == 0) && ((reinterpret_cast<uintptr_t>(Cg) & 15) == 0);
        const bool vec_cb = Cbg && ((g.ldcb & 3) == 0) && ((reinterpret_cast<uintptr_t>(Cbg) & 7) == 0);
        const bool bf16_only = (EPI == EPI_STORE) && !Cg && Cbg && ((g.ldcb & 7) == 0) &&
                               ((reinterpret_cast<uintptr_t>(Cbg) & 15) == 0);
#pragma unroll 1
        for (int c0 = 0; c0 < EPI_COLS; c0 += 32) {
          uint32_t r[32];
          tmem_ld32_issue(taddr + c0, r);
          const int nb = ncol0 + c0;
          if (bf16_only) {
            float v[32];
            if (bias && nb + 32 <= g.N && ((reinterpret_cast<uintptr_t>(bias + nb) & 15) == 0)) {
#pragma unroll
              for (int j = 0; j < 32; j += 4) {
                const float4 b = __ldg(reinterpret_cast<const float4*>(bias + nb + j));
                v[j] = b.x; v[j + 1] = b.y; v[j + 2] = b.z; v[j + 3] = b.w;
              }
            } else {
#pragma unroll
              for (int j = 0; j < 32; ++j) v[j] = (bias && nb + j < g.N) ? __ldg(bias + nb + j) : 0.f;
            }
            tmem_ld_wait(r);
            if (nb >= g.N || row0 >= g.M) continue;
#pragma unroll
// ... 240 lines not shown
              uint2 pk;
              pk.x = *reinterpret_cast<uint32_t*>(&p0); pk.y = *reinterpret_cast<uint32_t*>(&p1);
              *reinterpret_cast<uint2*>(g.dzb_out + (int64_t)rr * 4 * H + qq * H + u4) = pk;
            }
          }
        }
      } else {
        constexpr bool kW = EPI == EPI_GRADW;
        const int64_t tgt = row_ok ? g.targets[row] : -1;
        const float escale = row_ok ? (kW ? g.scale_log2 + log2f(fabsf(__ldg(g.row_weight + row))) : g.scale_log2) -
                                          g.lse[row] * LOG2E
                                    : 0.f;
        const float tl = row_ok ? g.tlogit[row] : 0.f;
        int cnt = 0;
#pragma unroll 1
        for (int c0 = 0; c0 < EPI_COLS; c0 += 32) {
          uint32_t r[32];
          tmem_ld32_issue(taddr + c0, r);
          const int nb = ncol0 + c0;
          float v[32];
          if (nb + 32 <= g.N && ((reinterpret_cast<uintptr_t>(g.bias + nb) & 15) == 0)) {
#pragma unroll
            for (int j = 0; j < 32; j += 4) {
              const float4 b = __ldg(reinterpret_cast<const float4*>(g.bias + nb + j));
              v[j] = b.x; v[j + 1] = b.y; v[j + 2] = b.z; v[j + 3] = b.w;
            }
          } else {
#pragma unroll
            for (int j = 0; j < 32; ++j) v[j] = (nb + j < g.N) ? __ldg(g.bias + nb + j) : 0.f;
          }
          tmem_ld_wait(r);
          if (nb >= g.lddl || row0 >= g.M) continue;
          if (nb + 32 <= g.N) {
#pragma unroll
            for (int j = 0; j < 32; ++j) {
              const float x = v[j] + __uint_as_float(r[j]);
              cnt += (x > tl);
              v[j] = ex2(fmaf(x, LOG2E, escale));
            }
            if (tgt >= nb && tgt < nb + 32) {
#pragma unroll
              for (int j = 0; j < 32; ++j) if (nb + j == (int)tgt) v[j] -= kW ? wscale(g, row) : g.scale;
            }
            if (!row_ok) {
              cnt = 0;
#pragma unroll
              for (int j = 0; j < 32; ++j) v[j] = 0.f;
            }
          } else {
#pragma unroll
            for (int j = 0; j < 32; ++j) {
              const int n = nb + j;
              const float x = v[j] + __uint_as_float(r[j]);
              const bool in = row_ok && n < g.N;
              cnt += (in && x > tl);
              const float p = ex2(fmaf(x, LOG2E, escale));
              v[j] = in ? p - (n == (int)tgt ? (kW ? wscale(g, row) : g.scale) : 0.f) : 0.f;
            }
          }
          if (kW && row_ok && __ldg(g.row_weight + row) < 0.f) {
#pragma unroll
            for (int j = 0; j < 32; ++j) v[j] = -v[j];
          }
          if (g.dL) store_block_bf16(xbuf, lane, v, g.dL, g.lddl, row0, g.M, nb, (int)g.lddl, true);
        }
        if (g.above && cnt) atomicAdd(g.above + row, cnt);
      }
      tc_fence_before();
      __syncwarp();
      if (lane == 0) mbar_arrive_cluster(tempty_leader0 + 8 * as);
    }
  }
  tc_fence_before();
  cluster_sync();
  if (warp == 1) {
    tc_fence_after();
    tmem_dealloc2(tmem_base, TMEM_COLS);
  }
}

__global__ void __launch_bounds__(256) splitk_reduce_kernel(const float* __restrict__ ws, int splits, int64_t M, int64_t N,
                                                            float* C, int64_t ldc, __nv_bfloat16* Cb, int64_t ldcb,
                                                            const float* __restrict__ bias, float beta) {
  const int64_t total4 = M * N / 4;
  const int64_t MN = M * N;
  for (int64_t i = (int64_t)blockIdx.x * blockDim.x + threadIdx.x; i < total4; i += (int64_t)gridDim.x * blockDim.x) {
    const int64_t e = i * 4;
    const int64_t m = e / N, n = e - m * N;
    float4 a = *reinterpret_cast<const float4*>(ws + e);
    for (int s = 1; s < splits; ++s) {
      const float4 b = *reinterpret_cast<const float4*>(ws + s * MN + e);
      a.x += b.x; a.y += b.y; a.z += b.z; a.w += b.w;
    }
    if (bias) { a.x += bias[n]; a.y += bias[n + 1]; a.z += bias[n + 2]; a.w += bias[n + 3]; }
    if (C) {
      float* dst = C + m * ldc + n;
      if (beta != 0.f) { a.x += beta * dst[0]; a.y += beta * dst[1]; a.z += beta * dst[2]; a.w += beta * dst[3]; }
      dst[0] = a.x; dst[1] = a.y; dst[2] = a.z; dst[3] = a.w;
    }
    if (Cb) {
      __nv_bfloat16* d = Cb + m * ldcb + n;
      d[0] = __float2bfloat16(a.x); d[1] = __float2bfloat16(a.y); d[2] = __float2bfloat16(a.z); d[3] = __float2bfloat16(a.w);
    }
  }
}

__global__ void __launch_bounds__(256) vocab_combine_kernel(const float* __restrict__ pmax, const float* __restrict__ psum,
                                                            const int32_t* __restrict__ pidx, int nchunks, int64_t N,
                                                            const float* __restrict__ tlogit, float* __restrict__ lse,
                                                            float* __restrict__ row_loss, int64_t* __restrict__ argmax,
                                                            int32_t* __restrict__ above) {
  const int lane = threadIdx.x & 31;
  const int64_t row = (int64_t)blockIdx.x * 8 + (threadIdx.x >> 5);
  if (row >= N) return;
  float mx = -CUDART_INF_F;
  int mi = 0x7fffffff;
  for (int c = lane; c < nchunks; c += 32) {
    const float v = pmax[row * nchunks + c];
    const int i = pidx[row * nchunks + c];
    if (v > mx || (v == mx && i < mi)) { mx = v; mi = i; }
  }
#pragma unroll
  for (int o = 16; o > 0; o >>= 1) {
    const float ov = __shfl_xor_sync(0xffffffffu, mx, o);
    const int oi = __shfl_xor_sync(0xffffffffu, mi, o);
    if (ov > mx || (ov == mx && oi < mi)) { mx = ov; mi = oi; }
  }
  float s = 0.f;
  for (int c = lane; c < nchunks; c += 32) s += psum[row * nchunks + c] * expf(pmax[row * nchunks + c] - mx);
  s = sn::warp_sum(s);
  if (lane == 0) {
    const float l = mx + logf(s);
    lse[row] = l;
    if (row_loss) row_loss[row] = l - tlogit[row];
    if (argmax) argmax[row] = mi;
    if (above) above[row] = 0;
  }
}

__global__ void rank_hit_kernel(const int32_t* __restrict__ above, int64_t N, int32_t k, int32_t* __restrict__ hit) {
  const int64_t i = (int64_t)blockIdx.x * blockDim.x + threadIdx.x;
  if (i < N) hit[i] = above[i] < k ? 1 : 0;
}

typedef CUresult (*EncodeFn)(CUtensorMap*, CUtensorMapDataType, cuuint32_t, void*, const cuuint64_t*, const cuuint64_t*,
                             const cuuint32_t*, const cuuint32_t*, CUtensorMapInterleave, CUtensorMapSwizzle,
                             CUtensorMapL2promotion, CUtensorMapFloatOOBfill);

EncodeFn get_encode() {
  static EncodeFn fn = nullptr;
  static bool tried = false;
  if (!tried) {
    tried = true;
    void* p = nullptr;
    cudaDriverEntryPointQueryResult qres;
    if (cudaGetDriverEntryPoint("cuTensorMapEncodeTiled", &p, cudaEnableDefault, &qres) == cudaSuccess &&
        qres == cudaDriverEntryPointSuccess)
      fn = reinterpret_cast<EncodeFn>(p);
  }
  return fn;
}

int32_t encode_2d(CUtensorMap* map, const void* base, int64_t inner, int64_t rows, int64_t pitch_elems, int box_inner,
                  int box_rows) {
  EncodeFn enc = get_encode();
  if (!enc) return sn::fail(-4, "cuTensorMapEncodeTiled entry point not available");
  cuuint64_t dims[2] = {(cuuint64_t)inner, (cuuint64_t)rows};
  cuuint64_t strides[1] = {(cuuint64_t)pitch_elems * 2};
  cuuint32_t box[2] = {(cuuint32_t)box_inner, (cuuint32_t)box_rows};
  cuuint32_t estr[2] = {1, 1};
  CUresult r = enc(map, CU_TENSOR_MAP_DATA_TYPE_BFLOAT16, 2, const_cast<void*>(base), dims, strides, box, estr,
                   CU_TENSOR_MAP_INTERLEAVE_NONE, CU_TENSOR_MAP_SWIZZLE_128B, CU_TENSOR_MAP_L2_PROMOTION_L2_256B,
                   CU_TENSOR_MAP_FLOAT_OOB_FILL_NONE);
  if (r != CUDA_SUCCESS) return sn::fail(-5, "cuTensorMapEncodeTiled failed (%d): base=%p inner=%lld rows=%lld pitch=%lld", (int)r,
                                         base, (long long)inner, (long long)rows, (long long)pitch_elems);
  return 0;
}

int32_t make_maps(int32_t op, int64_t M, int64_t N, int64_t K, const void* A, int64_t lda, const void* B, int64_t ldb,
                  int32_t batch, int64_t strideA, int64_t strideB, TmaSet& ta, TmaSet& tb, G2Args& g, int64_t a_rows = -1, int bn = BN) {
  if (a_rows < 0) a_rows = M;
  g.a_mn_major = (op == SN_OP_TN) ? 1 : 0;
  g.b_mn_major = (op == SN_OP_NT) ? 0 : 1;
  const __nv_bfloat16* Ab = (const __nv_bfloat16*)A;
  const __nv_bfloat16* Bb = (const __nv_bfloat16*)B;
  for (int i = 0; i < 4; ++i) {
    int gi = i < batch ? i : 0;
    int32_t rc;
    if (!g.a_mn_major) rc = encode_2d(&ta.m[i], Ab + gi * strideA, K, a_rows, lda, BK, BMC);
    else rc = encode_2d(&ta.m[i], Ab + gi * strideA, M, K, lda, 64, BK);
    if (rc) return rc;
    if (!g.b_mn_major) rc = encode_2d(&tb.m[i], Bb + gi * strideB, K, N, ldb, BK, bn / 2);
    else rc = encode_2d(&tb.m[i], Bb + gi * strideB, N, K, ldb, 64, BK);
    if (rc) return rc;
  }
  return 0;
}

template <int EPI, int BN_ = BN>
int32_t launch(const TmaSet& ta, const TmaSet& tb, const G2Args& g, cudaStream_t st, const char* what, int max_pairs = 0) {
  static thread_local bool configured = false;
  if (!configured) {
    SN_CUDA(cudaFuncSetAttribute(gemm2_kernel<EPI, BN_>, cudaFuncAttributeMaxDynamicSharedMemorySize, Geo<BN_>::SMEM_BYTES));
    configured = true;
  }
  const int64_t tiles = (int64_t)((g.M + BM - 1) / BM) * ((g.N + BN_ - 1) / BN_) * g.groups * g.splits;
  int64_t pairs = sn::dev_info().sm_count / 2;
  if (max_pairs > 0 && max_pairs < pairs) pairs = max_pairs;
  if (tiles < pairs) pairs = tiles;
  gemm2_kernel<EPI, BN_><<<(unsigned)(2 * pairs), NTHREADS, Geo<BN_>::SMEM_BYTES, st>>>(ta, tb, g);
  return sn::check_launch(what);
}

int32_t check_operands(const char* what, const void* A, int64_t lda, const void* B, int64_t ldb, int64_t strideA,
                       int64_t strideB) {
  SN_REQUIRE(A && B, "%s: null operand", what);
  SN_REQUIRE((lda % 8) == 0 && (ldb % 8) == 0 && (strideA % 8) == 0 && (strideB % 8) == 0,
             "%s: bf16 leading dimensions / group strides must be multiples of 8 elements (TMA 16-byte rule): "
             "lda=%lld ldb=%lld", what, (long long)lda, (long long)ldb);
  SN_REQUIRE(((uintptr_t)A & 15) == 0 && ((uintptr_t)B & 15) == 0, "%s: operands must be 16-byte aligned", what);
  return 0;
}

}

extern "C" int64_t sn_gemm2_ws_bytes(int64_t M, int64_t N, int32_t batch, int32_t splits) {
  if (splits <= 1) return 0;
  return (int64_t)sizeof(float) * M * N * batch * splits;
}

extern "C" int32_t sn_gemm2_bf16(int32_t op, int64_t M, int64_t N, int64_t K, const void* A, int64_t lda, const void* B,
                                 int64_t ldb, float* C, int64_t ldc, void* Cb, int64_t ldcb, const float* bias, float beta,
                                 int32_t batch, int64_t strideA, int64_t strideB, int64_t strideC, int64_t strideCb,
                                 int64_t strideBias, int32_t splits, void* ws, int64_t ws_bytes, int32_t max_pairs,
                                 void* stream) {
  SN_REQUIRE(op >= 0 && op <= 2, "sn_gemm2_bf16: bad op %d", op);
  SN_REQUIRE(batch >= 1 && batch <= 4, "sn_gemm2_bf16: 1..4 groups supported, got %d", batch);
  SN_REQUIRE(M >= 0 && N >= 0 && K > 0, "sn_gemm2_bf16: bad dims");
  if (M == 0 || N == 0) return 0;
  SN_REQUIRE(C || Cb, "sn_gemm2_bf16: no output");
  int32_t rc = check_operands("sn_gemm2_bf16", A, lda, B, ldb, strideA, strideB);
  if (rc) return rc;
  const int64_t total_kb = (K + BK - 1) / BK;
  if (splits < 1) splits = 1;
  if (splits > total_kb) splits = (int32_t)total_kb;
  TmaSet ta, tb;
  G2Args g = {};
  g.M = (int)M; g.N = (int)N; g.K = (int)K; g.groups = batch; g.splits = splits;
  rc = make_maps(op, M, N, K, A, lda, B, ldb, batch, strideA, strideB, ta, tb, g);
  if (rc) return rc;
  g.C = C; g.Cb = (__nv_bfloat16*)Cb; g.ldc = ldc; g.ldcb = ldcb; g.bias = bias; g.beta = beta;
  g.strideC = strideC; g.strideCb = strideCb; g.strideBias = strideBias;
  cudaStream_t st = (cudaStream_t)stream;
  if (splits == 1) return launch<EPI_STORE>(ta, tb, g, st, "sn_gemm2_bf16", max_pairs);
  SN_REQUIRE((N % 4) == 0, "sn_gemm2_bf16: split-K needs N %% 4 == 0");
  SN_REQUIRE(ws && ws_bytes >= sn_gemm2_ws_bytes(M, N, batch, splits), "sn_gemm2_bf16: split-K work space too small");
  SN_REQUIRE(((uintptr_t)ws & 15) == 0, "sn_gemm2_bf16: work space must be 16-byte aligned");
  g.ws = (float*)ws;
  rc = launch<EPI_PARTIAL>(ta, tb, g, st, "sn_gemm2_bf16(split-K)", max_pairs);
  if (rc) return rc;
  for (int gi = 0; gi < batch; ++gi) {
    int64_t blocks = (M * N / 4 + 255) / 256;
    int64_t cap = (int64_t)sn::dev_info().sm_count * 8;
    if (blocks > cap) blocks = cap;
    splitk_reduce_kernel<<<(unsigned)blocks, 256, 0, st>>>(
        g.ws + (int64_t)gi * splits * M * N, splits, M, N, C ? C + gi * strideC : nullptr, ldc,
        Cb ? (__nv_bfloat16*)Cb + gi * strideCb : nullptr, ldcb, bias ? bias + gi * strideBias : nullptr, beta);
    rc = sn::check_launch("sn_gemm2_bf16(reduce)");
    if (rc) return rc;
  }
  return 0;
}

extern "C" int64_t sn_vocab_ws_bytes(int64_t N, int64_t V) {
  const int64_t nchunks = (V + 63) / 64;
  return N * nchunks * 12;
}

extern "C" int32_t sn_vocab_nll_fwd(int64_t N, int64_t V, int64_t H, const void* Hb, int64_t ldh, const void* Wb,
                                    int64_t ldw, const float* bias, const int64_t* targets, void* ws, int64_t ws_bytes,
                                    float* tlogit, float* lse, float* row_loss, int64_t* argmax, int32_t* above,
                                    void* stream) {
  SN_REQUIRE(N >= 0 && V > 0 && H > 0, "sn_vocab_nll_fwd: bad dims");
  if (N == 0) return 0;
  SN_REQUIRE(bias && targets && tlogit && lse, "sn_vocab_nll_fwd: null argument");
  SN_REQUIRE(ws && ws_bytes >= sn_vocab_ws_bytes(N, V), "sn_vocab_nll_fwd: work space too small");
  int32_t rc = check_operands("sn_vocab_nll_fwd", Hb, ldh, Wb, ldw, 0, 0);
  if (rc) return rc;
  const int nchunks = (int)((V + 63) / 64);
  TmaSet ta, tb;
  G2Args g = {};
  g.M = (int)N; g.N = (int)V; g.K = (int)H; g.groups = 1; g.splits = 1;
  rc = make_maps(SN_OP_NT, N, V, H, Hb, ldh, Wb, ldw, 1, 0, 0, ta, tb, g);
  if (rc) return rc;
  g.bias = bias; g.targets = targets; g.nchunks = nchunks;
  g.pmax = (float*)ws; g.psum = g.pmax + N * nchunks; g.pidx = (int32_t*)(g.psum + N * nchunks);
  g.tlogit = tlogit;
  cudaStream_t st = (cudaStream_t)stream;
  rc = launch<EPI_STATS>(ta, tb, g, st, "sn_vocab_nll_fwd");
  if (rc) return rc;
  vocab_combine_kernel<<<(unsigned)((N + 7) / 8), 256, 0, st>>>(g.pmax, g.psum, g.pidx, nchunks, N, tlogit, lse, row_loss,
                                                               argmax, above);
  return sn::check_launch("sn_vocab_nll_fwd(combine)");
}

extern "C" int32_t sn_vocab_nll_bwd(int64_t N, int64_t V, int64_t H, const void* Hb, int64_t ldh, const void* Wb,
                                    int64_t ldw, const float* bias, const int64_t* targets, const float* tlogit,
                                    const float* lse, float grad_scale, const float* row_weight, void* dL,
                                    int64_t lddl, int32_t* above, int32_t* top5hit, void* stream) {
  SN_REQUIRE(N >= 0 && V > 0 && H > 0, "sn_vocab_nll_bwd: bad dims");
  if (N == 0) return 0;
  SN_REQUIRE(bias && targets && tlogit && lse, "sn_vocab_nll_bwd: null argument");
  SN_REQUIRE(!dL || (lddl >= V && (lddl % 8) == 0 && ((uintptr_t)dL & 15) == 0),
             "sn_vocab_nll_bwd: dL pitch must be >= V, a multiple of 8, base 16-byte aligned");
  SN_REQUIRE(!top5hit || above, "sn_vocab_nll_bwd: top5hit needs the `above` counter");
  int32_t rc = check_operands("sn_vocab_nll_bwd", Hb, ldh, Wb, ldw, 0, 0);
  if (rc) return rc;
  TmaSet ta, tb;
  G2Args g = {};
  g.M = (int)N; g.N = (int)V; g.K = (int)H; g.groups = 1; g.splits = 1;
  rc = make_maps(SN_OP_NT, N, V, H, Hb, ldh, Wb, ldw, 1, 0, 0, ta, tb, g);
  if (rc) return rc;
  g.bias = bias; g.targets = targets; g.tlogit = (float*)tlogit; g.lse = lse; g.scale = grad_scale; g.scale_log2 = log2f(grad_scale);
  g.row_weight = row_weight;
  g.dL = (__nv_bfloat16*)dL; g.lddl = dL ? lddl : V; g.above = above;
  cudaStream_t st = (cudaStream_t)stream;
  rc = row_weight ? launch<EPI_GRADW>(ta, tb, g, st, "sn_vocab_nll_bwd") : launch<EPI_GRAD>(ta, tb, g, st, "sn_vocab_nll_bwd");
  if (rc) return rc;
  if (top5hit) {
    rank_hit_kernel<<<(unsigned)((N + 255) / 256), 256, 0, st>>>(above, N, 5, top5hit);
    return sn::check_launch("sn_vocab_nll_bwd(top5)");
  }
  return 0;
}

namespace {

__global__ void gate_interleave_kernel(const float* __restrict__ W, int64_t H, int64_t K, int64_t ldw,
                                       __nv_bfloat16* __restrict__ Wp, int64_t ldp) {
  const int64_t total = 4 * H * ldp;
  for (int64_t i = (int64_t)blockIdx.x * blockDim.x + threadIdx.x; i < total; i += (int64_t)gridDim.x * blockDim.x) {
    const int64_t n = i / ldp, k = i - n * ldp;
    const int64_t ublk = n >> 8, q = (n >> 6) & 3, uu = n & 63;
    const int64_t src_row = q * H + ublk * 64 + uu;
    Wp[n * ldp + k] = __float2bfloat16(k < K ? W[src_row * ldw + k] : 0.f);
  }
}

__global__ void hprev_gather_kernel(const __nv_bfloat16* __restrict__ Hb, const int32_t* __restrict__ row_b,
                                    const int32_t* __restrict__ row_t, const int32_t* __restrict__ off, int64_t N,
                                    int64_t H, __nv_bfloat16* __restrict__ Hprevb) {
  const int64_t per_row = H >> 3;
  const int64_t total = N * per_row;
  for (int64_t i = (int64_t)blockIdx.x * blockDim.x + threadIdx.x; i < total; i += (int64_t)gridDim.x * blockDim.x) {
    const int64_t r = i / per_row, c = (i - r * per_row) << 3;
    const int t = row_t[r];
    uint4 v = make_uint4(0u, 0u, 0u, 0u);
    if (t > 0) v = *reinterpret_cast<const uint4*>(Hb + ((int64_t)off[t - 1] + row_b[r]) * H + c);
    *reinterpret_cast<uint4*>(Hprevb + r * H + c) = v;
  }
}

}

extern "C" int32_t sn_cast_bf16_gate_interleave(const float* W, int64_t H, int64_t K, int64_t ldw, void* Wp, int64_t ldp,
                                                void* stream) {
  SN_REQUIRE(W && Wp && H > 0 && (H % 64) == 0 && K > 0 && ldw >= K && ldp >= K && (ldp % 8) == 0,
             "sn_cast_bf16_gate_interleave: bad arguments");
  int64_t blocks = (4 * H * ldp + 255) / 256;
  int64_t cap = (int64_t)sn::dev_info().sm_count * 16;
  if (blocks > cap) blocks = cap;
  gate_interleave_kernel<<<(unsigned)blocks, 256, 0, (cudaStream_t)stream>>>(W, H, K, ldw, (__nv_bfloat16*)Wp, ldp);
  return sn::check_launch("sn_cast_bf16_gate_interleave");
}

extern "C" int32_t sn_recur_fwd_gemm(int32_t cell, int64_t H, int64_t B, const int32_t* bs_host, const int32_t* off_host,
                                     int32_t T, const float* XP, const void* Wp_bf16, const float* bhh, float* Hall,
                                     void* Hb, float* Call, float* gates, const void* zeros_bf16, void* stream) {
  SN_REQUIRE(cell == SN_CELL_FACTORED || cell == SN_CELL_LSTM, "sn_recur_fwd_gemm: bad cell %d", cell);
  SN_REQUIRE(H > 0 && (H % 64) == 0 && B > 0 && T > 0, "sn_recur_fwd_gemm: hidden size must be a multiple of 64");
  SN_REQUIRE(bs_host && off_host && XP && Wp_bf16 && Hb && Call && zeros_bf16, "sn_recur_fwd_gemm: null argument");
  int32_t rc = check_operands("sn_recur_fwd_gemm", Hb, H, Wp_bf16, H, 0, 0);
  if (rc) return rc;
  cudaStream_t st = (cudaStream_t)stream;
  __nv_bfloat16* Hbb = (__nv_bfloat16*)Hb;
  for (int t = 0; t < T; ++t) {
    const int64_t M = bs_host[t], r0 = off_host[t];
    if (M <= 0) break;
    TmaSet ta, tb;
    G2Args g = {};
    g.M = (int)M; g.N = (int)(4 * H); g.K = (int)H; g.groups = 1; g.splits = 1;
    const void* A = t == 0 ? zeros_bf16 : (const void*)(Hbb + (int64_t)off_host[t - 1] * H);
    rc = make_maps(SN_OP_NT, M, 4 * H, H, A, H, Wp_bf16, H, 1, 0, 0, ta, tb, g);
    if (rc) return rc;
    g.cell = cell; g.Hdim = (int)H;
    g.xp = XP + r0 * 4 * H; g.bhh = bhh;
    g.c_prev = t == 0 ? nullptr : Call + (int64_t)off_host[t - 1] * H;
    g.h_out = Hall ? Hall + r0 * H : nullptr; g.hb_out = Hbb + r0 * H;
    g.c_out = Call + r0 * H; g.gates_out = gates ? gates + r0 * 4 * H : nullptr;
    rc = launch<EPI_CELL_FWD>(ta, tb, g, st, "sn_recur_fwd_gemm");
    if (rc) return rc;
  }
  return 0;
}

extern "C" int32_t sn_recur_hprev(const void* Hb, const int32_t* row_b, const int32_t* row_t, const int32_t* offsets,
                                  int64_t N, int64_t H, void* Hprevb, void* stream) {
  SN_REQUIRE(Hb && row_b && row_t && offsets && Hprevb && N >= 0 && H > 0 && (H % 8) == 0, "sn_recur_hprev: bad arguments");
  if (N == 0) return 0;
  int64_t blocks = (N * (H >> 3) + 255) / 256;
  int64_t cap = (int64_t)sn::dev_info().sm_count * 16;
  if (blocks > cap) blocks = cap;
  hprev_gather_kernel<<<(unsigned)blocks, 256, 0, (cudaStream_t)stream>>>((const __nv_bfloat16*)Hb, row_b, row_t, offsets, N, H,
// ... 38 lines not shown
```

### image-caption-emotion-indonesia_b200/csrc/sn_gemm_tc.cu

```cuda
#include <cuda.h>
#include <cuda_bf16.h>

#include "sn_common.cuh"

namespace {

constexpr int BM = 128, BN = 128, BK = 64;
constexpr int STAGES = 3;
constexpr int UMMA_K = 16;
constexpr int A_BYTES = BM * BK * 2, B_BYTES = BN * BK * 2;
constexpr int STAGE_BYTES = A_BYTES + B_BYTES;
constexpr int SMEM_BYTES = STAGES * STAGE_BYTES + 1024  + 256 ;
constexpr int TMEM_COLS = 128;
constexpr int NTHREADS = 192;

struct TmaSet { CUtensorMap m[4]; };

struct TcArgs {
  int M, N, K;
  int splits;
  int a_mn_major, b_mn_major;
  float* C; __nv_bfloat16* Cb; int64_t ldc, ldcb;
  const float* bias; float beta;
  int64_t strideC, strideCb, strideBias;
// ... 266 lines not shown
                                       int64_t strideC, int64_t strideCb, int64_t strideBias, int32_t splits,
                                       void* stream);

extern "C" int32_t sn_gemm_bf16(int32_t op, int64_t M, int64_t N, int64_t K, const void* A, int64_t lda, const void* B,
                                int64_t ldb, float* C, int64_t ldc, void* Cb, int64_t ldcb, const float* bias, float beta,
                                int32_t batch, int64_t strideA, int64_t strideB, int64_t strideC, int64_t strideCb,
                                int64_t strideBias, void* stream) {
  return sn_gemm_bf16_splitk(op, M, N, K, A, lda, B, ldb, C, ldc, Cb, ldcb, bias, beta, batch, strideA, strideB, strideC,
                             strideCb, strideBias, 1, stream);
}

extern "C" int32_t sn_gemm_bf16_splitk(int32_t op, int64_t M, int64_t N, int64_t K, const void* A, int64_t lda,
                                       const void* B, int64_t ldb, float* C, int64_t ldc, void* Cb, int64_t ldcb,
                                       const float* bias, float beta, int32_t batch, int64_t strideA, int64_t strideB,
                                       int64_t strideC, int64_t strideCb, int64_t strideBias, int32_t splits,
                                       void* stream) {
  SN_REQUIRE(op >= 0 && op <= 2, "sn_gemm_bf16: bad op %d", op);
  SN_REQUIRE(batch >= 1 && batch <= 4, "sn_gemm_bf16: 1..4 groups supported, got %d", batch);
  SN_REQUIRE(M >= 0 && N >= 0 && K > 0, "sn_gemm_bf16: bad dims");
  if (M == 0 || N == 0) return 0;
  SN_REQUIRE(A && B && (C || Cb), "sn_gemm_bf16: null operand");
  SN_REQUIRE((lda % 8) == 0 && (ldb % 8) == 0 && (strideA % 8) == 0 && (strideB % 8) == 0,
             "sn_gemm_bf16: bf16 leading dimensions / group strides must be multiples of 8 elements (TMA 16-byte rule): "
             "lda=%lld ldb=%lld", (long long)lda, (long long)ldb);
  SN_REQUIRE(((uintptr_t)A & 15) == 0 && ((uintptr_t)B & 15) == 0, "sn_gemm_bf16: operands must be 16-byte aligned");
  const int64_t total_kb = (K + BK - 1) / BK;
  if (splits <= 0) {
    const int64_t tiles = ((M + BM - 1) / BM) * ((N + BN - 1) / BN) * batch;
    splits = 1;
    if (!Cb && beta == 0.f && tiles < 100 && total_kb >= 8) {
      int64_t want = (2 * (int64_t)sn::dev_info().sm_count + tiles / 2) / tiles;
      int64_t cap = total_kb / 4;
      if (want > cap) want = cap;
      if (want > 8) want = 8;
      if (want > 1) splits = (int)want;
    }
  }
  if (splits > total_kb) splits = (int)total_kb;
  if (splits < 1) splits = 1;
  if (splits > 1) {
    SN_REQUIRE(C && !Cb && beta == 0.f, "sn_gemm_bf16: split-K needs an fp32-only output and beta == 0");
    for (int gi = 0; gi < batch; ++gi) {
      float* base = C + gi * strideC;
      if (ldc == N) {
        SN_CUDA(cudaMemsetAsync(base, 0, sizeof(float) * (size_t)M * (size_t)N, (cudaStream_t)stream));
      } else {
        SN_CUDA(cudaMemset2DAsync(base, sizeof(float) * (size_t)ldc, 0, sizeof(float) * (size_t)N, (size_t)M,
                                  (cudaStream_t)stream));
      }
    }
  }
  TmaSet ta, tb;
  TcArgs g;
  g.M = (int)M; g.N = (int)N; g.K = (int)K; g.splits = splits;
  g.a_mn_major = (op == SN_OP_TN) ? 1 : 0;
  g.b_mn_major = (op == SN_OP_NT) ? 0 : 1;
  g.C = C; g.Cb = (__nv_bfloat16*)Cb; g.ldc = ldc; g.ldcb = ldcb; g.bias = bias; g.beta = beta;
  g.strideC = strideC; g.strideCb = strideCb; g.strideBias = strideBias;
  const __nv_bfloat16* Ab = (const __nv_bfloat16*)A;
  const __nv_bfloat16* Bb = (const __nv_bfloat16*)B;
  for (int i = 0; i < 4; ++i) {
    int gi = i < batch ? i : 0;
    int32_t rc;
    if (!g.a_mn_major) rc = encode_2d(&ta.m[i], Ab + gi * strideA, K, M, lda, BK, BM);
    else rc = encode_2d(&ta.m[i], Ab + gi * strideA, M, K, lda, 64, BK);
    if (rc) return rc;
    if (!g.b_mn_major) rc = encode_2d(&tb.m[i], Bb + gi * strideB, K, N, ldb, BK, BN);
    else rc = encode_2d(&tb.m[i], Bb + gi * strideB, N, K, ldb, 64, BK);
    if (rc) return rc;
  }
  static thread_local bool configured = false;
  if (!configured) {
    SN_CUDA(cudaFuncSetAttribute(gemm_tc_kernel, cudaFuncAttributeMaxDynamicSharedMemorySize, SMEM_BYTES));
    configured = true;
  }
  dim3 grid((unsigned)((N + BN - 1) / BN), (unsigned)((M + BM - 1) / BM), (unsigned)(batch * splits));
  gemm_tc_kernel<<<grid, NTHREADS, SMEM_BYTES, (cudaStream_t)stream>>>(ta, tb, g);
  return sn::check_launch("sn_gemm_bf16");
}

namespace {
__global__ void cast_pad_kernel(const float* __restrict__ src, int64_t R, int64_t Cc, int64_t lds,
                                __nv_bfloat16* __restrict__ dst, int64_t Cp, int64_t ldd) {
  const int64_t total = R * Cp;
  for (int64_t i = (int64_t)blockIdx.x * blockDim.x + threadIdx.x; i < total; i += (int64_t)gridDim.x * blockDim.x) {
    int64_t r = i / Cp, c = i - r * Cp;
    dst[r * ldd + c] = __float2bfloat16(c < Cc ? src[r * lds + c] : 0.f);
  }
}
__global__ void cast_vec8_kernel(const float* __restrict__ src, int64_t n8, __nv_bfloat16* __restrict__ dst) {
  for (int64_t i = (int64_t)blockIdx.x * blockDim.x + threadIdx.x; i < n8; i += (int64_t)gridDim.x * blockDim.x) {
    const float4 a = __ldg(reinterpret_cast<const float4*>(src) + 2 * i);
    const float4 b = __ldg(reinterpret_cast<const float4*>(src) + 2 * i + 1);
    __nv_bfloat162 p0 = __floats2bfloat162_rn(a.x, a.y), p1 = __floats2bfloat162_rn(a.z, a.w);
    __nv_bfloat162 p2 = __floats2bfloat162_rn(b.x, b.y), p3 = __floats2bfloat162_rn(b.z, b.w);
    uint4 pk;
    pk.x = *reinterpret_cast<uint32_t*>(&p0); pk.y = *reinterpret_cast<uint32_t*>(&p1);
    pk.z = *reinterpret_cast<uint32_t*>(&p2); pk.w = *reinterpret_cast<uint32_t*>(&p3);
    reinterpret_cast<uint4*>(dst)[i] = pk;
  }
}
}

extern "C" int32_t sn_cast_bf16_ex(const float* src, int64_t R, int64_t Cc, int64_t lds, void* dst, int64_t Cp, int64_t ldd,
                                   int32_t max_blocks, void* stream) {
  SN_REQUIRE(R >= 0 && Cc >= 0 && Cp >= Cc && ldd >= Cp, "sn_cast_bf16: bad dims");
  if (R == 0 || Cp == 0) return 0;
  int64_t total = R * Cp;
  int64_t cap = (int64_t)sn::dev_info().sm_count * 16;
  if (max_blocks > 0 && max_blocks < cap) cap = max_blocks;
  const bool dense = Cc == Cp && lds == Cc && ldd == Cp && (total % 8) == 0 && ((uintptr_t)src & 15) == 0 &&
                     ((uintptr_t)dst & 15) == 0;
  if (dense) {
    int64_t blocks = (total / 8 + 255) / 256;
    if (blocks > cap) blocks = cap;
    cast_vec8_kernel<<<(unsigned)blocks, 256, 0, (cudaStream_t)stream>>>(src, total / 8, (__nv_bfloat16*)dst);
    return sn::check_launch("sn_cast_bf16");
  }
  int64_t blocks = (total + 255) / 256;
  if (blocks > cap) blocks = cap;
  cast_pad_kernel<<<(unsigned)blocks, 256, 0, (cudaStream_t)stream>>>(src, R, Cc, lds, (__nv_bfloat16*)dst, Cp, ldd);
  return sn::check_launch("sn_cast_bf16");
}

extern "C" int32_t sn_cast_bf16(const float* src, int64_t R, int64_t Cc, int64_t lds, void* dst, int64_t Cp, int64_t ldd,
                                void* stream) {
  return sn_cast_bf16_ex(src, R, Cc, lds, dst, Cp, ldd, 0, stream);
}
```

### image-caption-emotion-indonesia_b200/csrc/sn_recur_cl.cu

```cuda
#include <cuda_bf16.h>

#include "sn_common.cuh"

namespace {

constexpr int NTH = 512;
constexpr int NS = 16;
constexpr int RP = 132;
constexpr int DP = 136;

struct CArgs {
  int cell, B, t0, t1;
  const int* bs; const int* off;
  const float* XP; const __nv_bfloat16* Wb; const float* bhh; const float* h_init;
  float* Hall; __nv_bfloat16* Hb; __nv_bfloat16* Hprevb; float* Call; float* gates; float* c_state;
  const float* c_init; const float* dHall; float* dZ; __nv_bfloat16* dZb; float* dh_carry; float* dc_carry;
  int* start_flag;
};

__device__ __forceinline__ uint32_t smem_u32(const void* p) { return (uint32_t)__cvta_generic_to_shared(p); }
__device__ __forceinline__ uint32_t cluster_ctarank() {
  uint32_t r;
  asm volatile("mov.u32 %0, %%cluster_ctarank;" : "=r"(r));
  return r;
// ... 17 lines not shown
}
__device__ __forceinline__ void mbar_expect_tx(uint32_t bar, uint32_t bytes) {
  asm volatile("mbarrier.arrive.expect_tx.shared::cta.b64 _, [%0], %1;" ::"r"(bar), "r"(bytes) : "memory");
}
__device__ __forceinline__ void mbar_wait_cluster(uint32_t bar, uint32_t parity) {
  asm volatile(
      "{\n\t.reg .pred p;\n\t"
      "CL_WAIT_LOOP:\n\t"
      "mbarrier.try_wait.parity.acquire.cluster.shared::cta.b64 p, [%0], %1;\n\t"
      "@p bra CL_WAIT_DONE;\n\t"
      "bra CL_WAIT_LOOP;\n\t"
      "CL_WAIT_DONE:\n\t}" ::"r"(bar), "r"(parity) : "memory");
}
__device__ __forceinline__ void st_async16(uint32_t dst_cluster, uint32_t v0, uint32_t v1, uint32_t v2, uint32_t v3,
                                           uint32_t bar_cluster) {
  asm volatile("st.async.weak.shared::cluster.mbarrier::complete_tx::bytes.v4.b32 [%0], {%1, %2, %3, %4}, [%5];"
               ::"r"(dst_cluster), "r"(v0), "r"(v1), "r"(v2), "r"(v3), "r"(bar_cluster) : "memory");
}
__device__ __forceinline__ void st_async8(uint32_t dst_cluster, uint32_t v0, uint32_t v1, uint32_t bar_cluster) {
  asm volatile("st.async.weak.shared::cluster.mbarrier::complete_tx::bytes.v2.b32 [%0], {%1, %2}, [%3];"
               ::"r"(dst_cluster), "r"(v0), "r"(v1), "r"(bar_cluster) : "memory");
}
__device__ __forceinline__ void ldmatrix_x4(uint32_t (&r)[4], uint32_t saddr) {
  asm volatile("ldmatrix.sync.aligned.m8n8.x4.shared.b16 {%0,%1,%2,%3}, [%4];"
               : "=r"(r[0]), "=r"(r[1]), "=r"(r[2]), "=r"(r[3]) : "r"(saddr));
}
__device__ __forceinline__ void mma_bf16(float (&d)[4], const uint32_t (&a)[4], uint32_t b0, uint32_t b1) {
  asm volatile("mma.sync.aligned.m16n8k16.row.col.f32.bf16.bf16.f32 {%0,%1,%2,%3}, {%4,%5,%6,%7}, {%8,%9}, {%0,%1,%2,%3};"
               : "+f"(d[0]), "+f"(d[1]), "+f"(d[2]), "+f"(d[3])
               : "r"(a[0]), "r"(a[1]), "r"(a[2]), "r"(a[3]), "r"(b0), "r"(b1));
}
__device__ __forceinline__ void ldmatrix_x4_trans(uint32_t (&r)[4], uint32_t saddr) {
  asm volatile("ldmatrix.sync.aligned.m8n8.x4.trans.shared.b16 {%0,%1,%2,%3}, [%4];"
               : "=r"(r[0]), "=r"(r[1]), "=r"(r[2]), "=r"(r[3]) : "r"(saddr));
}
__device__ __forceinline__ void cp_async16(uint32_t dst, const void* src) {
  asm volatile("cp.async.cg.shared.global [%0], [%1], 16;" ::"r"(dst), "l"(src) : "memory");
}
__device__ __forceinline__ void cp_async_wait_all() {
  asm volatile("cp.async.commit_group;" ::: "memory");
  asm volatile("cp.async.wait_group 0;" ::: "memory");
}
__device__ __forceinline__ int clampi(int v, int lo, int hi) { return v < lo ? lo : (v > hi ? hi : v); }
__device__ __forceinline__ float sigmoid_fast(float x) { return __fdividef(1.f, 1.f + __expf(-x)); }
__device__ __forceinline__ float tanh_fast(float x) { return 1.f - __fdividef(2.f, 1.f + __expf(2.f * x)); }

template <int H, typename RowFn>
__device__ __forceinline__ void stage_rows(uint32_t stage, const __nv_bfloat16* Wb, RowFn grow) {
  constexpr int CH = H / 8;
  for (int i = threadIdx.x; i < 64 * CH; i += NTH) {
    const int r = i / CH, c = i - r * CH;
    cp_async16(stage + (uint32_t)(r * (H + 8) + c * 8) * 2, Wb + (int64_t)grow(r) * H + c * 8);
  }
  cp_async_wait_all();
  __syncthreads();
}

template <int H>
struct FwdSmem {
  static constexpr int HP = H + 8;
  static constexpr size_t hbuf = 0;
  static constexpr size_t red = hbuf + (size_t)2 * NS * HP * 2;
  static constexpr size_t hst = red + (size_t)2 * 4 * NS * RP * 4;
  static constexpr size_t bars = hst + (size_t)NS * 32 * 2;
  static constexpr size_t tab = bars + 16;
  static constexpr size_t total = tab;
};

template <int H>
__global__ void __launch_bounds__(NTH, 1) recur_fwd_cl_kernel(CArgs a) {
  constexpr int CS = H / 32, KT = H / 64, HP = FwdSmem<H>::HP, KQ = H / 4;
  extern __shared__ __align__(128) unsigned char smem[];
  __nv_bfloat16* hbuf = reinterpret_cast<__nv_bfloat16*>(smem + FwdSmem<H>::hbuf);
  float* red = reinterpret_cast<float*>(smem + FwdSmem<H>::red);
  __nv_bfloat16* hst = reinterpret_cast<__nv_bfloat16*>(smem + FwdSmem<H>::hst);
  const uint32_t bar0 = smem_u32(smem + FwdSmem<H>::bars);

  const int tid = threadIdx.x, lane = tid & 31, warp = tid >> 5;
  const int rank = (int)cluster_ctarank();
  const int s0 = (int)cluster_id_x() * NS, u0 = rank * 32;
  const int oct = warp & 3, kq = warp >> 2;
  const int pos_o = a.cell == SN_CELL_LSTM ? 3 : 2, pos_c = a.cell == SN_CELL_LSTM ? 2 : 3;

  uint32_t Wr[4][KT][2];
  {
    const uint32_t stage = smem_u32(smem);
#pragma unroll
    for (int rd = 0; rd < 2; ++rd) {
      stage_rows<H>(stage, a.Wb, [&](int r) { return (2 * rd + (r >> 5)) * H + u0 + (r & 31); });
#pragma unroll
      for (int gg = 0; gg < 2; ++gg) {
        const uint32_t base = stage + (uint32_t)((gg * 32 + oct * 8 + (lane & 7)) * HP + kq * KQ + (lane >> 3) * 8) * 2;
#pragma unroll
        for (int kt = 0; kt < KT; kt += 2) {
          uint32_t f[4];
          ldmatrix_x4(f, base + kt * 32);
          Wr[2 * rd + gg][kt][0] = f[0]; Wr[2 * rd + gg][kt][1] = f[1];
          Wr[2 * rd + gg][kt + 1][0] = f[2]; Wr[2 * rd + gg][kt + 1][1] = f[3];
        }
      }
      __syncthreads();
    }
  }

  const int fs = warp, fu = lane, gs = s0 + fs, ug = u0 + fu;
  const bool live = gs < a.B;
  float c_reg = live ? a.c_state[(int64_t)gs * H + ug] : 0.f;
  const int nv_first = clampi(a.bs[a.t0] - s0, 0, NS);
  __nv_bfloat16 hprev = __float2bfloat16((fs < nv_first && a.h_init) ? a.h_init[(int64_t)gs * H + ug] : 0.f);
  float bh[4];
#pragma unroll
  for (int g = 0; g < 4; ++g) bh[g] = a.bhh ? __ldg(a.bhh + g * H + ug) : 0.f;

  int2* tab = reinterpret_cast<int2*>(smem + FwdSmem<H>::tab);
  for (int i = tid; i < a.t1 - a.t0; i += NTH)
    tab[i] = make_int2(clampi(a.bs[a.t0 + i] - s0, 0, NS), a.off[a.t0 + i] + s0);
  {
    const int p0 = a.t0 & 1;
    for (int i = tid; i < NS * (H / 2); i += NTH) {
      const int r = i / (H / 2), c = (i - r * (H / 2)) * 2;
      float2 v = make_float2(0.f, 0.f);
      if (a.h_init && r < nv_first) v = *reinterpret_cast<const float2*>(a.h_init + (int64_t)(s0 + r) * H + c);
      *reinterpret_cast<__nv_bfloat162*>(hbuf + ((size_t)p0 * NS + r) * HP + c) = __floats2bfloat162_rn(v.x, v.y);
      *reinterpret_cast<__nv_bfloat162*>(hbuf + ((size_t)(p0 ^ 1) * NS + r) * HP + c) = __floats2bfloat162_rn(0.f, 0.f);
    }
  }
  if (tid == 0) {
    mbar_init(bar0, 1);
    mbar_init(bar0 + 8, 1);
    asm volatile("fence.mbarrier_init.release.cluster;" ::: "memory");
  }
  cluster_sync();

  uint32_t ph0 = 0, ph1 = 0;
  for (int t = a.t0; t < a.t1; ++t) {
    const int2 tb = tab[t - a.t0];
    const int nv = tb.x;
    if (nv == 0) break;
    const int nvn = (t + 1 < a.t1) ? tab[t + 1 - a.t0].x : 0;
    const int p = t & 1, pn = p ^ 1;
    if (tid == 0 && nvn > 0) mbar_expect_tx(bar0 + 8 * pn, (uint32_t)(CS * nvn * 64));
    const bool valid = fs < nv;
    const int64_t row = (int64_t)tb.y + fs;
    float xp[4] = {0.f, 0.f, 0.f, 0.f};
    if (valid) {
      const float* x = a.XP + row * 4 * H + ug;
#pragma unroll
      for (int g = 0; g < 4; ++g) xp[g] = __ldg(x + g * H);
    }
    if (t > a.t0) {
      if (p) { mbar_wait_cluster(bar0 + 8, ph1); ph1 ^= 1; } else { mbar_wait_cluster(bar0, ph0); ph0 ^= 1; }
    }
    float acc[4][4];
#pragma unroll
    for (int g = 0; g < 4; ++g) acc[g][0] = acc[g][1] = acc[g][2] = acc[g][3] = 0.f;
    {
      const uint32_t abase = smem_u32(hbuf + ((size_t)p * NS + (lane & 15)) * HP + kq * KQ + (lane >> 4) * 8);
#pragma unroll
      for (int kt = 0; kt < KT; ++kt) {
        uint32_t af[4];
        ldmatrix_x4(af, abase + kt * 32);
#pragma unroll
        for (int g = 0; g < 4; ++g) mma_bf16(acc[g], af, Wr[g][kt][0], Wr[g][kt][1]);
      }
    }
    {
      float* rp = red + (((size_t)p * 4 + kq) * NS + (lane >> 2)) * RP + (oct * 8 + (lane & 3) * 2) * 4;
      *reinterpret_cast<float4*>(rp) = make_float4(acc[0][0], acc[1][0], acc[2][0], acc[3][0]);
      *reinterpret_cast<float4*>(rp + 4) = make_float4(acc[0][1], acc[1][1], acc[2][1], acc[3][1]);
      *reinterpret_cast<float4*>(rp + 8 * RP) = make_float4(acc[0][2], acc[1][2], acc[2][2], acc[3][2]);
      *reinterpret_cast<float4*>(rp + 8 * RP + 4) = make_float4(acc[0][3], acc[1][3], acc[2][3], acc[3][3]);
    }
    __syncthreads();
    __nv_bfloat16 hb = __float2bfloat16(0.f);
    if (valid) {
      float z[4];
      {
        const float* r = red + ((size_t)p * 4 * NS + fs) * RP + fu * 4;
        const float4 q0 = *reinterpret_cast<const float4*>(r), q1 = *reinterpret_cast<const float4*>(r + (size_t)NS * RP);
        const float4 q2 = *reinterpret_cast<const float4*>(r + (size_t)2 * NS * RP);
        const float4 q3 = *reinterpret_cast<const float4*>(r + (size_t)3 * NS * RP);
        z[0] = ((q0.x + q1.x) + (q2.x + q3.x)) + xp[0] + bh[0];
        z[1] = ((q0.y + q1.y) + (q2.y + q3.y)) + xp[1] + bh[1];
        z[2] = ((q0.z + q1.z) + (q2.z + q3.z)) + xp[2] + bh[2];
        z[3] = ((q0.w + q1.w) + (q2.w + q3.w)) + xp[3] + bh[3];
      }
      const float zo = a.cell == SN_CELL_LSTM ? z[3] : z[2], zc = a.cell == SN_CELL_LSTM ? z[2] : z[3];
      const float gi = sigmoid_fast(z[0]), gf = sigmoid_fast(z[1]), go = sigmoid_fast(zo), gc = tanh_fast(zc);
      const float c = gf * c_reg + gi * gc;
      const float h = a.cell == SN_CELL_LSTM ? go * tanh_fast(c) : go * c;
      c_reg = c;
      hb = __float2bfloat16(h);
      a.Hb[row * H + ug] = hb;
      if (a.Hprevb) a.Hprevb[row * H + ug] = hprev;
      if (a.Hall) a.Hall[row * H + ug] = h;
      if (a.Call) a.Call[row * H + ug] = c;
      if (a.gates) {
        float* gp = a.gates + row * 4 * H + ug;
        gp[0] = gi; gp[H] = gf; gp[pos_o * H] = go; gp[pos_c * H] = gc;
      }
      hprev = hb;
    }
    if (nvn > 0) {
      hst[fs * 32 + fu] = hb;
      __syncthreads();
      for (int j = lane; j < 4 * CS; j += 32) {
        const int i = warp * (4 * CS) + j;
        const int dest = i >> 6, ch = i & 63, srow = ch >> 2, part = ch & 3;
        if (srow < nvn) {
          const uint4 v = *reinterpret_cast<const uint4*>(hst + srow * 32 + part * 8);
          const uint32_t dst_local = smem_u32(hbuf + ((size_t)pn * NS + srow) * HP + u0 + part * 8);
          st_async16(mapa(dst_local, dest), v.x, v.y, v.z, v.w, mapa(bar0 + 8 * pn, dest));
        }
      }
    }
  }
  if (live) a.c_state[(int64_t)gs * H + ug] = c_reg;
  cluster_sync();
}

template <int H>
struct BwdSmem {
  static constexpr int CS = H / 32;
  static constexpr size_t recv = 0;
  static constexpr size_t dzs = recv + (size_t)2 * CS * NS * 32 * 2;
  static constexpr size_t bars = dzs + (size_t)2 * NS * DP * 2;
  static constexpr size_t tab = bars + 16;
  static constexpr size_t stage = (size_t)64 * (H + 8) * 2;
  static constexpr size_t total = tab > stage ? tab : stage;
};

template <int H>
__global__ void __launch_bounds__(NTH, 1) recur_bwd_cl_kernel(CArgs a) {
  constexpr int CS = H / 32, NTB = H / 128;
  extern __shared__ __align__(128) unsigned char smem[];
  __nv_bfloat16* recv = reinterpret_cast<__nv_bfloat16*>(smem + BwdSmem<H>::recv);
  __nv_bfloat16* dzs = reinterpret_cast<__nv_bfloat16*>(smem + BwdSmem<H>::dzs);
  const uint32_t bar0 = smem_u32(smem + BwdSmem<H>::bars);

  const int tid = threadIdx.x, lane = tid & 31, warp = tid >> 5;
  const int rank = (int)cluster_ctarank();
  const int s0 = (int)cluster_id_x() * NS, u0 = rank * 32;
  const int K4 = 4 * H;
  if (tid == 0 && a.start_flag) {
    if (atomicAdd(a.start_flag, 1) == (int)gridDim.x - 1) {
      a.start_flag[0] = 0;
      __threadfence();
      atomicAdd(a.start_flag + 1, 1);
    }
  }

  uint32_t Wr[8][NTB][2];
  {
    const uint32_t stage = smem_u32(smem);
    constexpr int HP = H + 8;
#pragma unroll
    for (int rd = 0; rd < 2; ++rd) {
      stage_rows<H>(stage, a.Wb, [&](int r) { return (2 * rd + (r >> 5)) * H + u0 + (r & 31); });
#pragma unroll
      for (int k2 = 0; k2 < 4; k2 += 2) {
#pragma unroll
        for (int nt = 0; nt < NTB; ++nt) {
          uint32_t f[4];
          ldmatrix_x4_trans(f, stage + (uint32_t)((k2 * 16 + (lane >> 3) * 8 + (lane & 7)) * HP + (warp * NTB + nt) * 8) * 2);
          Wr[4 * rd + k2][nt][0] = f[0]; Wr[4 * rd + k2][nt][1] = f[1];
          Wr[4 * rd + k2 + 1][nt][0] = f[2]; Wr[4 * rd + k2 + 1][nt][1] = f[3];
        }
      }
      __syncthreads();
    }
  }

  const int fs = warp, fu = lane, gs = s0 + fs, ug = u0 + fu;
  const bool live = gs < a.B;
  const int64_t sidx = (int64_t)gs * H + ug;
  float dc_reg = live ? a.dc_carry[sidx] : 0.f;
  const int fpos = (((fu >> 4) * 2 + ((fu >> 2) & 1)) * 8) + ((fu >> 3) & 1) * 4 + (fu & 3);

  int2* tab = reinterpret_cast<int2*>(smem + BwdSmem<H>::total);
  for (int i = tid; i < a.t1 - a.t0; i += NTH)
    tab[i] = make_int2(clampi(a.bs[a.t0 + i] - s0, 0, NS), a.off[a.t0 + i] + s0);
  const int row_before = a.t0 > 0 ? a.off[a.t0 - 1] + s0 : 0;
  for (int i = tid; i < 2 * NS * DP / 2; i += NTH) reinterpret_cast<uint32_t*>(dzs)[i] = 0u;
  if (tid == 0) {
    mbar_init(bar0, 1);
    mbar_init(bar0 + 8, 1);
    asm volatile("fence.mbarrier_init.release.cluster;" ::: "memory");
  }
  cluster_sync();

  uint32_t ph0 = 0, ph1 = 0;
  for (int t = a.t1 - 1; t >= a.t0; --t) {
    const int2 tb = tab[t - a.t0];
    const int nv = tb.x;
    if (nv == 0) continue;
    const int nrec = (t + 1 < a.t1) ? tab[t + 1 - a.t0].x : 0;
    const int p = t & 1, pr = p ^ 1;
    if (tid == 0) mbar_expect_tx(bar0 + 8 * p, (uint32_t)(CS * nv * 64));
    const bool valid = fs < nv;
    const int64_t row = (int64_t)tb.y + fs;
    float g4[4] = {0.f, 0.f, 0.f, 0.f}, cc = 0.f, cprev = 0.f, dhl = 0.f;
    if (valid) {
      const float* gp = a.gates + row * K4 + ug;
#pragma unroll
      for (int g = 0; g < 4; ++g) g4[g] = __ldg(gp + g * H);
      cc = __ldg(a.Call + row * H + ug);
      if (t > 0) cprev = __ldg(a.Call + ((int64_t)(t > a.t0 ? tab[t - 1 - a.t0].y : row_before) + fs) * H + ug);
      else cprev = a.c_init ? __ldg(a.c_init + sidx) : 0.f;
      dhl = __ldg(a.dHall + row * H + ug);
    }
    float dh_rec = 0.f;
    if (nrec > 0) {
      if (pr) { mbar_wait_cluster(bar0 + 8, ph1); ph1 ^= 1; } else { mbar_wait_cluster(bar0, ph0); ph0 ^= 1; }
      if (fs < nrec) {
        const __nv_bfloat16* r = recv + ((size_t)pr * CS * NS + fs) * 32 + fpos;
        float s = 0.f;
#pragma unroll
        for (int src = 0; src < CS; ++src) s += __bfloat162float(r[(size_t)src * NS * 32]);
        dh_rec = s;
      }
    }
    if (valid) {
      if (t == a.t1 - 1) dh_rec = a.dh_carry[sidx];
      const float gi = g4[0], gf = g4[1];
      const float go = a.cell == SN_CELL_LSTM ? g4[3] : g4[2], gc = a.cell == SN_CELL_LSTM ? g4[2] : g4[3];
      const float dh = dhl + dh_rec;
      float d_o, dc;
      if (a.cell == SN_CELL_LSTM) {
        const float tc = tanhf(cc);
        d_o = dh * tc;
        dc = dc_reg + dh * go * (1.f - tc * tc);
      } else {
        d_o = dh * cc;
        dc = dc_reg + dh * go;
      }
      const float di = dc * gc, df = dc * cprev, dg = dc * gi;
      dc_reg = dc * gf;
      float z[4];
      const float z_o = d_o * go * (1.f - go), z_c = dg * (1.f - gc * gc);
      z[0] = di * gi * (1.f - gi); z[1] = df * gf * (1.f - gf);
      z[2] = a.cell == SN_CELL_LSTM ? z_c : z_o; z[3] = a.cell == SN_CELL_LSTM ? z_o : z_c;
      __nv_bfloat16* dzb = a.dZb + row * K4 + ug;
      __nv_bfloat16* own = dzs + ((size_t)p * NS + fs) * DP + fu;
#pragma unroll
      for (int g = 0; g < 4; ++g) {
        const __nv_bfloat16 zb = __float2bfloat16(z[g]);
        dzb[g * H] = zb;
        own[g * 32] = zb;
        if (a.dZ) a.dZ[row * K4 + g * H + ug] = z[g];
      }
    }
    __syncthreads();
    {
      float acc[NTB][4];
#pragma unroll
      for (int nt = 0; nt < NTB; ++nt) acc[nt][0] = acc[nt][1] = acc[nt][2] = acc[nt][3] = 0.f;
      const uint32_t abase = smem_u32(dzs + ((size_t)p * NS + (lane & 15)) * DP + (lane >> 4) * 8);
#pragma unroll
      for (int kt = 0; kt < 8; ++kt) {
        uint32_t af[4];
        ldmatrix_x4(af, abase + kt * 32);
#pragma unroll
        for (int nt = 0; nt < NTB; ++nt) mma_bf16(acc[nt], af, Wr[kt][nt][0], Wr[kt][nt][1]);
      }
      const bool odd = lane & 1;
      const int srow = (lane >> 2) + (odd ? 8 : 0);
      const int ub = ((lane & 3) >> 1) * 4;
      uint32_t pk[NTB][2];
#pragma unroll
      for (int nt = 0; nt < NTB; ++nt) {
        const float x0 = odd ? acc[nt][0] : acc[nt][2], x1 = odd ? acc[nt][1] : acc[nt][3];
        const float y0 = __shfl_xor_sync(0xffffffffu, x0, 1), y1 = __shfl_xor_sync(0xffffffffu, x1, 1);
        const float v0 = odd ? y0 : acc[nt][0], v1 = odd ? y1 : acc[nt][1];
        const float v2 = odd ? acc[nt][2] : y0, v3 = odd ? acc[nt][3] : y1;
        __nv_bfloat162 lo = __floats2bfloat162_rn(v0, v1), hi = __floats2bfloat162_rn(v2, v3);
        pk[nt][0] = *reinterpret_cast<uint32_t*>(&lo);
        pk[nt][1] = *reinterpret_cast<uint32_t*>(&hi);
      }
      if (srow < nv) {
        const __nv_bfloat16* rowp = recv + (((size_t)p * CS + rank) * NS + srow) * 32;
        if (NTB >= 2) {
#pragma unroll
          for (int nt = 0; nt + 1 < NTB; nt += 2) {
            const int gnt = warp * NTB + nt;
            const int dest = gnt >> 2, lnt = gnt & 3;
            const uint32_t dst_local = smem_u32(rowp + ((lnt >> 1) * 2 + (ub >> 2)) * 8);
            st_async16(mapa(dst_local, dest), pk[nt][0], pk[nt][1], pk[nt + 1][0], pk[nt + 1][1], mapa(bar0 + 8 * p, dest));
          }
        } else {
          const int gnt = warp, dest = gnt >> 2, lnt = gnt & 3;
          const uint32_t dst_local = smem_u32(rowp + ((lnt >> 1) * 2 + (ub >> 2)) * 8 + (lnt & 1) * 4);
          st_async8(mapa(dst_local, dest), pk[0][0], pk[0][1], mapa(bar0 + 8 * p, dest));
        }
      }
    }
  }
  {
    const int nv0 = tab[0].x;
    float dh_rec = 0.f;
    if (nv0 > 0) {
      const int p = a.t0 & 1;
      if (p) mbar_wait_cluster(bar0 + 8, ph1); else mbar_wait_cluster(bar0, ph0);
      if (fs < nv0) {
        const __nv_bfloat16* r = recv + ((size_t)p * CS * NS + fs) * 32 + fpos;
        float s = 0.f;
#pragma unroll
        for (int src = 0; src < CS; ++src) s += __bfloat162float(r[(size_t)src * NS * 32]);
        dh_rec = s;
      }
    }
    if (live) {
      a.dh_carry[sidx] = dh_rec;
      a.dc_carry[sidx] = dc_reg;
    }
  }
  cluster_sync();
}

__global__ void gate_wait_kernel(int* flag, long long timeout_cycles) {
  const long long t0 = clock64();
  const int stale = sn::ld_acquire(flag + 1);
  if (stale > flag[2]) flag[2] = stale;
  const int target = flag[2] + 1;
  flag[2] = target;
  while (sn::ld_acquire(flag + 1) < target) {
    if (clock64() - t0 > timeout_cycles) {
      flag[2] = target - 1;
      return;
    }
    __nanosleep(200);
  }
}

template <typename Kern>
int32_t launch_cl(Kern kernel, int CS, size_t smem, const CArgs& a, cudaStream_t stream, const char* what, int* max_clusters) {
  cudaLaunchConfig_t cfg = {};
  const int nclusters = (a.B + NS - 1) / NS;
  cfg.gridDim = dim3((unsigned)(nclusters * CS));
  cfg.blockDim = dim3(NTH);
  smem += (size_t)(a.t1 - a.t0 + 1) * 8;
  cfg.dynamicSmemBytes = smem;
  cfg.stream = stream;
  cudaLaunchAttribute attr[1];
  attr[0].id = cudaLaunchAttributeClusterDimension;
  attr[0].val.clusterDim.x = (unsigned)CS;
  attr[0].val.clusterDim.y = 1;
  attr[0].val.clusterDim.z = 1;
  cfg.attrs = attr;
  cfg.numAttrs = 1;
  SN_CUDA(cudaFuncSetAttribute(kernel, cudaFuncAttributeMaxDynamicSharedMemorySize, (int)smem));
  if (CS > 8) SN_CUDA(cudaFuncSetAttribute(kernel, cudaFuncAttributeNonPortableClusterSizeAllowed, 1));
  if (max_clusters) {
    int n = 0;
    cudaError_t e = cudaOccupancyMaxActiveClusters(&n, kernel, &cfg);
    if (e != cudaSuccess) { cudaGetLastError(); n = 0; }
    *max_clusters = n;
    return 0;
  }
  CArgs args = a;
  cudaError_t e = cudaLaunchKernelEx(&cfg, kernel, args);
  if (e != cudaSuccess) return sn::fail((int32_t)e, "%s: cluster launch failed: %s", what, cudaGetErrorString(e));
  return 0;
}

int32_t dispatch(bool bwd, int64_t H, const CArgs& a, cudaStream_t st, int* max_clusters) {
  switch (H) {
    case 512:
      return bwd ? launch_cl(recur_bwd_cl_kernel<512>, 16, BwdSmem<512>::total, a, st, "sn_recur_bwd_cl", max_clusters)
                 : launch_cl(recur_fwd_cl_kernel<512>, 16, FwdSmem<512>::total, a, st, "sn_recur_fwd_cl", max_clusters);
    case 256:
      return bwd ? launch_cl(recur_bwd_cl_kernel<256>, 8, BwdSmem<256>::total, a, st, "sn_recur_bwd_cl", max_clusters)
                 : launch_cl(recur_fwd_cl_kernel<256>, 8, FwdSmem<256>::total, a, st, "sn_recur_fwd_cl", max_clusters);
    case 128:
      return bwd ? launch_cl(recur_bwd_cl_kernel<128>, 4, BwdSmem<128>::total, a, st, "sn_recur_bwd_cl", max_clusters)
                 : launch_cl(recur_fwd_cl_kernel<128>, 4, FwdSmem<128>::total, a, st, "sn_recur_fwd_cl", max_clusters);
    default:
      return sn::fail(-1, "sn_recur_*_cl: hidden size %lld not supported by the cluster form (128, 256, 512)", (long long)H);
  }
}

}

extern "C" {

int32_t sn_recur_cl_max_clusters(int64_t H) {
  if (H != 128 && H != 256 && H != 512) return 0;
  static int cache[3] = {-1, -1, -1};
  const int slot = H == 512 ? 0 : (H == 256 ? 1 : 2);
  if (cache[slot] >= 0) return cache[slot];
  CArgs a = {};
  a.B = NS;
  int nf = 0, nb = 0;
  if (dispatch(false, H, a, nullptr, &nf) != 0 || dispatch(true, H, a, nullptr, &nb) != 0) return 0;
  cache[slot] = nf < nb ? nf : nb;
  return cache[slot];
}

int32_t sn_recur_fwd_cl(int32_t cell, int64_t H, int64_t B, const int32_t* batch_sizes, const int32_t* offsets,
                        int32_t t0, int32_t t1, const float* XP, const void* Whh_bf16, const float* bhh,
                        const float* h_init, float* Hall, void* Hb, void* Hprevb, float* Call, float* gates,
                        float* c_state, void* stream) {
  SN_REQUIRE(cell == SN_CELL_FACTORED || cell == SN_CELL_LSTM, "sn_recur_fwd_cl: bad cell %d", cell);
  SN_REQUIRE(t0 >= 0 && t1 >= t0 && B > 0, "sn_recur_fwd_cl: bad step range");
  SN_REQUIRE(XP && Whh_bf16 && Hb && c_state && batch_sizes && offsets, "sn_recur_fwd_cl: null argument");
  if (t1 == t0) return 0;
  CArgs a = {};
  a.cell = cell; a.B = (int)B; a.t0 = t0; a.t1 = t1; a.bs = batch_sizes; a.off = offsets;
  a.XP = XP; a.Wb = (const __nv_bfloat16*)Whh_bf16; a.bhh = bhh; a.h_init = h_init; a.Hall = Hall;
  a.Hb = (__nv_bfloat16*)Hb; a.Hprevb = (__nv_bfloat16*)Hprevb; a.Call = Call; a.gates = gates; a.c_state = c_state;
  return dispatch(false, H, a, (cudaStream_t)stream, nullptr);
}

int32_t sn_recur_bwd_cl(int32_t cell, int64_t H, int64_t B, const int32_t* batch_sizes, const int32_t* offsets,
                        int32_t t0, int32_t t1, const void* Whh_bf16, const float* c_init, const float* Call,
                        const float* gates, const float* dHall, float* dZ, void* dZb, float* dh_carry,
                        float* dc_carry, int32_t* start_flag, void* stream) {
  SN_REQUIRE(cell == SN_CELL_FACTORED || cell == SN_CELL_LSTM, "sn_recur_bwd_cl: bad cell %d", cell);
  SN_REQUIRE(t0 >= 0 && t1 >= t0 && B > 0, "sn_recur_bwd_cl: bad step range");
  SN_REQUIRE(Whh_bf16 && Call && gates && dHall && dZb && dh_carry && dc_carry && batch_sizes && offsets,
             "sn_recur_bwd_cl: null argument");
  if (t1 == t0) return 0;
  CArgs a = {};
  a.cell = cell; a.B = (int)B; a.t0 = t0; a.t1 = t1; a.bs = batch_sizes; a.off = offsets;
  a.Wb = (const __nv_bfloat16*)Whh_bf16; a.c_init = c_init; a.Call = const_cast<float*>(Call);
  a.gates = const_cast<float*>(gates); a.dHall = dHall; a.dZ = dZ; a.dZb = (__nv_bfloat16*)dZb;
  a.dh_carry = dh_carry; a.dc_carry = dc_carry; a.start_flag = start_flag;
  return dispatch(true, H, a, (cudaStream_t)stream, nullptr);
}

int32_t sn_gate_wait(int32_t* flag3, int64_t timeout_us, void* stream) {
  SN_REQUIRE(flag3 && timeout_us > 0, "sn_gate_wait: bad argument");
  gate_wait_kernel<<<1, 1, 0, (cudaStream_t)stream>>>(flag3, (long long)timeout_us * 2000);
  return sn::check_launch("sn_gate_wait");
}

}
```

### image-caption-emotion-indonesia_b200/decoders.py

```python
import random
from collections import OrderedDict

import os

import torch
import torch.nn as nn

from . import ops
from .arena import ParamArena
from .packing import get_plan

GREEDY_GRAPH = [True]

GATES = ("i", "f", "o", "c")
STYLES = ("factual", "happy", "sad", "angry")


def style_attr(style, gate):
    return ("S_f" + gate) if style == "factual" else ("S_%s_%s" % (style, gate))


def _ref_init(module, emb, out):
    for p in module.parameters():
        if p.dim() >= 2:
# ... 138 lines not shown
            ev.record(side)
        return ev

    def _next_seed(self, dev, p_drop):
        base = int(self.__dict__.get("_seed", 0x5EED)) * 1000003
        if p_drop <= 0.0:
            return base, None
        sd = self.__dict__.get("_seed_dev")
        if sd is None or sd.device != dev:
            sd = torch.zeros(1, dtype=torch.int64, device=dev)
            self.__dict__["_seed_dev"] = sd
        sd.add_(1)
        return base, sd

    def _check_inputs(self, captions, features):
        if not captions.is_cuda:
            raise ops._lib.SnError("decoder inputs must be CUDA tensors: this path has no CPU fallback")
        ops.lib()

    def _emb(self):
        raise NotImplementedError

    def _out(self):
        raise NotImplementedError

    def _input_projection(self, c, X, mode, r0, n):
        raise NotImplementedError

    def _input_projection_bwd(self, c, dZ, gbuf):
        raise NotImplementedError

    def _coins(self, T, teacher_forcing_ratio):
        return [random.random() < teacher_forcing_ratio for _ in range(T)]

    def _run_forward(self, plan, captions, features, coins, mode, save):
        a = self.arena()
        dev = captions.device
        d = plan.dev(dev)
        H, N, B, T = self.hidden_size, plan.N, plan.B, plan.T
        emb = self._emb()
        E = emb.weight.shape[1]
        has_feat = features is not None
        c = _Ctx()
        c.plan, c.mode, c.has_feat, c.captions = plan, mode, has_feat, captions
        c.p_drop = float(self.dropout.p) if self.training else 0.0
        c.seed, c.seed_dev = self._next_seed(dev, c.p_drop)
        feats = None
        if has_feat:
            feats = features.detach()
            if feats.dtype != torch.float32 or not feats.is_contiguous():
                feats = feats.float().contiguous()
            if feats.dim() == 3:
                feats = feats.reshape(feats.shape[0], -1)
        all_tf = all(coins)
        c.tok_override = None
        if not all_tf:
            c.tok_override = torch.full((N,), -1, dtype=torch.int32, device=dev)
        c.emb_ws = c.emb_ev = c.emb_zeroed = None
        if self.__dict__.pop("_emb_early", False) and all_tf:
            V = emb.weight.shape[0]
            c.emb_ws = ops.embed_plan_ws(V, N, dev)
            c.emb_zeroed = a.gflat
            gE = self._gview(a.gflat, [self._emb_name()], emb.weight.shape)
            side = self._side(4)
            side.wait_stream(torch.cuda.current_stream())
            with torch.cuda.stream(side):
                ops.embed_plan(captions, has_feat, d["row_b"], d["row_t"], None, N, V, c.emb_ws)
                gE.zero_()
                c.emb_ev = torch.cuda.Event()
                c.emb_ev.record(side)
        c.Ein = E
        c.w16 = {}
        c.ev_early = c.ev_late = c.ev_first = None
        if self.bf16:
            early, late = self._shadow_specs(c, mode)
            first = c.__dict__.pop("first_specs", None)
            if first:
                c.ev_first = self._shadows_async(first, max_blocks=0)
            second = c.__dict__.pop("second_specs", None)
            c.ev_second = self._shadows_async(second, max_blocks=0) if second else None
            if early:
                c.ev_early = self._shadows_async(early)
            if late:
                c.ev_late = self._shadows_async(late)
            self.__dict__["_out_w16_ev"] = self._shadows_async([(self.__dict__, "_out_w16_pref", self._out().weight)])
        if self.bf16:
            X = None
            c.Xb = torch.empty(N, _pad8(E), dtype=torch.bfloat16, device=dev)
        else:
            X = torch.empty(N, E, dtype=torch.float32, device=dev)
            c.Xb = None
        ops.gather_pack_fwd(captions, emb.weight, feats, has_feat, d["row_b"], d["row_t"], None, N, X,
                            c.p_drop, c.seed, seed_dev=c.seed_dev, Xb=c.Xb)
        c.X = X
        c.XP = torch.empty(N, 4 * H, dtype=torch.float32, device=dev)
        self._input_projection(c, X, mode, 0, N)
        c.Hall = torch.empty(N, H, dtype=torch.float32, device=dev)
        c.Call = torch.empty(N, H, dtype=torch.float32, device=dev) if save else None
        c.Hprev = torch.empty(N, H, dtype=torch.float32, device=dev) if save else None
        c.gates = torch.empty(N, 4 * H, dtype=torch.float32, device=dev) if save else None
        c_state = torch.zeros(B, H, dtype=torch.float32, device=dev)
        c.aux_argmax = None
        Whh, bhh = self._recurrent_weights()
        c.Whh, c.bhh = Whh, bhh
        use_tc = self.bf16 and H % 32 == 0
        c.Hb = c.Hpb = None
        if c.ev_late is not None:
            torch.cuda.current_stream().wait_event(c.ev_late)
        if use_tc:
            if "Whh" not in c.w16:
                c.w16["Whh"] = self._shadow(Whh)
            c.Hb = torch.empty(N, H, dtype=torch.bfloat16, device=dev)
            c.Hpb = torch.empty(N, H, dtype=torch.bfloat16, device=dev) if save else None
            c.Hprev = None
        c.upper = self._upper_layers_init(c, save)
        c.top = c.upper[-1] if c.upper else c

        c.c_state = c_state

        def run(t0, t1):
            self._recur_fwd(c, c, t0, t1)
            if c.upper:
                self._upper_layers_fwd(c, t0, t1)

        if all_tf:
            run(0, T)
        else:
            out = self._out()
            V = out.weight.shape[0]
            pred = captions[:, 0].to(torch.int32).contiguous()
            am = torch.empty(B, dtype=torch.int64, device=dev)
            t = 0
            while t < T:
                if coins[t]:
                    t1 = t
                    while t1 < T and coins[t1]:
                        t1 += 1
                    run(t, t1)
                    t = t1
                else:
                    bt, r0 = plan.bs[t], plan.off[t]
                    if t > 0:
                        bp, rp = plan.bs[t - 1], plan.off[t - 1]
                        lg = torch.empty(bp, V, dtype=torch.float32, device=dev)
                        ops.gemm(ops.OP_NT, c.top.Hall, out.weight, lg, bp, V, H, H, H, V, bias=out.bias,
                                 a_off=rp * H)
                        ops.softmax_nll(lg, bp, V, argmax=am)
                        pred = am[:bp].to(torch.int32)
                    c.tok_override[r0:r0 + bt] = pred[:bt]
                    ops.gather_pack_fwd(captions, emb.weight, feats, has_feat, d["row_b"], d["row_t"],
                                        c.tok_override, bt, X, c.p_drop, c.seed, row_off=r0, seed_dev=c.seed_dev,
                                        Xb=c.Xb)
                    self._input_projection(c, X, mode, r0, bt)
                    run(t, t + 1)
                    t += 1
        c.grad_names = self._seq_grad_names(mode)
        c.feat_shape = None if features is None else features.shape
        if not save:
            c.X = c.XP = None
        return c

    def _recur_fwd(self, c, cl, t0, t1):
        plan = c.plan
        d = plan.dev(cl.XP.device)
        H, B, T = self.hidden_size, plan.B, plan.T
        Whh, bhh = cl.Whh, cl.bhh
        if cl.Hb is not None:
            if t0 == 0 and t1 == T and B >= ops.RECUR_GEMM_MIN_BATCH[0] and H % 64 == 0:
                if "Whh_il" not in cl.w16:
                    cl.w16["Whh_il"] = ops.cast_gate_interleave(Whh)
                if cl.Call is None:
                    cl.Call = torch.empty(plan.N, H, dtype=torch.float32, device=cl.XP.device)
                ops.recur_fwd_gemm(self.cell, H, B, plan, cl.XP, cl.w16["Whh_il"], bhh, cl.Hall, cl.Hb, cl.Call, cl.gates)
                if cl.Hpb is not None:
                    ops.recur_hprev(cl.Hb, d, plan.N, H, cl.Hpb)
                cl.recur_gemm = True
                return
            h_init = cl.Hall[plan.off[t0 - 1]:] if t0 > 0 else None
            ops.recur_fwd_bf16(self.cell, H, B, d["bs"], d["off"], t0, t1, cl.XP, cl.w16["Whh"], bhh, h_init,
                               cl.Hall, cl.Hb, cl.Hpb, cl.Call, cl.gates, cl.c_state)
        else:
            h_init = cl.Hall[plan.off[t0 - 1]:] if t0 > 0 else None
            ops.recur_fwd(self.cell, H, B, d["bs"], d["off"], t0, t1, cl.XP, Whh, bhh, h_init, cl.Hall,
                          cl.Call, cl.Hprev, cl.gates, cl.c_state)

    def _shadow_specs(self, c, mode):
        H = self.hidden_size
        late = []
        if H % 32 == 0:
            late.append((c.w16, "Whh", self._recurrent_weights()[0]))
        return [], late

    def _upper_layers_init(self, c, save):
        return []

    def _upper_layers_fwd(self, c, t0, t1):
        pass

    def _layer_bwd(self, c, cl, dHall, gbuf):
        plan = c.plan
        dev = dHall.device
        d = plan.dev(dev)
        H, N, B, T = self.hidden_size, plan.N, plan.B, plan.T
        L = getattr(cl, "layer", 0)
        Whh, _ = self._recurrent_weights(L)
        dZ = torch.empty(N, 4 * H, dtype=torch.float32, device=dev)
        dhc = torch.zeros(2, B, H, dtype=torch.float32, device=dev)
        dh, dc = dhc[0], dhc[1]
        gW, gbW = self._recurrent_grads(gbuf, L)
        if cl.Hpb is not None:
            cl.dZb = torch.empty(N, 4 * H, dtype=torch.bfloat16, device=dev)
            if getattr(cl, "recur_gemm", False):
                ops.recur_bwd_gemm(self.cell, H, B, plan, cl.w16["Whh"], cl.Call, cl.gates, dHall, dZ, cl.dZb, dc)
            else:
                ops.recur_bwd_bf16(self.cell, H, B, d["bs"], d["off"], 0, T, cl.w16["Whh"], None, cl.Call, cl.gates,
                                   dHall, dZ, cl.dZb, dh, dc, start_flag=self.__dict__.pop("_gate_armed", None))
            self._run_deferred()
            with torch.cuda.stream(self._fork()):
                ops.gemm_bf16(ops.OP_TN, cl.dZb, cl.Hpb, 4 * H, H, N, 4 * H, H, C=gW, ldc=H)
                ops.colsum(dZ, N, 4 * H, 4 * H, gbW, wide=bool(ops.TAIL_SCHEDULE[0]))
            cl.colsum_dZ = gbW if ops.TAIL_SCHEDULE[0] else None
            return self._input_projection_bwd(cl, dZ, gbuf)
        ops.recur_bwd(self.cell, H, B, d["bs"], d["off"], 0, T, Whh, None, cl.Call, cl.gates, dHall, dZ, dh, dc)
        if self.bf16:
            cl.dZb = ops.to_bf16_padded(dZ)
            Hpb = ops.to_bf16_padded(cl.Hprev)
            ops.gemm_bf16(ops.OP_TN, cl.dZb, Hpb, 4 * H, H, N, 4 * H, H, C=gW, ldc=H)
        else:
            ops.gemm(ops.OP_TN, dZ, cl.Hprev, gW, 4 * H, H, N, 4 * H, H, H)
        ops.colsum(dZ, N, 4 * H, 4 * H, gbW)
        return self._input_projection_bwd(cl, dZ, gbuf)

    def _run_backward(self, c, dHall, gbuf, need_dfeat):
        for cl in reversed(c.upper):
            dHall = self._layer_bwd(c, cl, dHall, gbuf)
        dX = self._layer_bwd(c, c, dHall, gbuf)
        out = self._embedding_bwd(c, dX, gbuf, need_dfeat)
        self._join()
        return out

    def _embedding_bwd(self, c, dX, gbuf, need_dfeat):
        plan = c.plan
        dev = dX.device
        d = plan.dev(dev)
        N, B = plan.N, plan.B
        emb = self._emb()
        E = emb.weight.shape[1]
        gE = self._gview(gbuf, [self._emb_name()], emb.weight.shape)
        dfeat = torch.empty(B, E, dtype=torch.float32, device=dev) if (need_dfeat and c.has_feat) else None
        if getattr(c, "emb_ws", None) is not None:
            torch.cuda.current_stream().wait_event(c.emb_ev)
            if gbuf is not c.emb_zeroed:
                gE.zero_()
            ops.embed_grad(gE, dfeat, c.has_feat, d["row_b"], d["row_t"], c.tok_override, N, dX, c.p_drop, c.seed,
                           c.emb_ws, seed_dev=c.seed_dev, wide=True)
        else:
            gE.zero_()
            ops.gather_pack_bwd(c.captions, gE, dfeat, c.has_feat, d["row_b"], d["row_t"], c.tok_override, N, dX,
                                c.p_drop, c.seed, seed_dev=c.seed_dev)
        if dfeat is not None and c.feat_shape is not None:
            dfeat = dfeat.view(c.feat_shape)
        self._bucket_final([self._emb_name()])
        return dfeat

    def _run_deferred(self):
        todo = self.__dict__.pop("_after_recur", None)
        for fn in todo or ():
            fn()

    def _bucket_final(self, names):
        hook = self.__dict__.get("_bucket_hook")
        if hook is None:
            return
        gbuf, fn = hook
        names = [n for n in names if n in self.arena().named]
        self._publish(names, gbuf)
        fn(names)

    def _gview(self, gbuf, names, shape):
        a = self.arena()
        o, n = a._span(names)
        return gbuf[o:o + n].view(shape)

    def _vocab_logits(self, Hall, Hb=None):
        out = self._out()
        if self.bf16:
            V, H = out.weight.shape
            N = Hall.shape[0]
            if Hb is None:
                Hb = ops.to_bf16_padded(Hall.contiguous())
# ... 700 lines not shown
```

### image-caption-emotion-indonesia_b200/ops.py

```python
import ctypes

import torch

from . import _lib
from ._lib import OP_NN, OP_NT, OP_TN, CELL_FACTORED, CELL_LSTM
from ._lib import check as _check


def check(rc, what=""):
    _check(rc, what)
    if what != "sn_device_info":
        LAUNCHES[0] += 1


LAUNCHES = [0]


class no_gc_during_capture:

    def __enter__(self):
        import gc
        gc.collect()
        self.was = gc.isenabled()
        gc.disable()

    def __exit__(self, *a):
        import gc
        if self.was:
            gc.enable()


def _stream():
    return ctypes.c_void_p(torch.cuda.current_stream().cuda_stream)


def _ptr(t):
    return ctypes.c_void_p(t.data_ptr()) if t is not None else None


def _req(t, dtype=torch.float32):
    if not t.is_cuda:
        raise _lib.SnError("libsn100 ops need CUDA tensors (no CPU fallback); got %s" % t.device)
    if t.dtype != dtype:
        raise _lib.SnError("expected %s, got %s" % (dtype, t.dtype))
    return t


def lib():
    l = _lib.load()
    _lib.require_device(torch.cuda.current_device())
    return l


FP32_GEMM = ["split"]
SPLIT_MIN_MACS = 1 << 22
SPLIT_MAX_ACC_K = 768


def _pad8(n):
    return (n + 7) // 8 * 8


def _split_cols(X, off, rows, K, ld, batch, s, pattern):
    Kp = _pad8(K)
    if batch > 1 and s < ld:
        if s != K or ld < batch * K:
            return None
        G, R = batch, rows
    elif batch > 1:
        if s != rows * ld:
            return None
        G, R = 1, rows * batch
    else:
        G, R = 1, rows
    out = torch.empty(R, G * 6 * Kp, dtype=torch.bfloat16, device=X.device)
    check(lib().sn_split_limbs_cols(ctypes.c_void_p(X.data_ptr() + 4 * off), R, G, K, ld, _ptr(out), Kp, pattern,
                                    _stream()), "sn_split_limbs_cols")
    return out, G * 6 * Kp, (6 * Kp if G > 1 else rows * 6 * Kp)


def _split_rows(X, off, K, cols, ld, batch, s, pattern):
    Kp, ldp = _pad8(K), _pad8(ld)
    if batch > 1 and s < ld:
        if s % 8 != 0:
            return None
        G = 1
    elif batch > 1:
        if s != K * ld:
            return None
        G = batch
    else:
        G = 1
    out = torch.empty(G * 6 * Kp, ldp, dtype=torch.bfloat16, device=X.device)
    check(lib().sn_split_limbs_rows(ctypes.c_void_p(X.data_ptr() + 4 * off), G, K, ld, ld, _ptr(out), Kp, ldp, pattern,
                                    _stream()), "sn_split_limbs_rows")
    return out, ldp, (s if (batch > 1 and s < ld) else 6 * Kp * ldp)


def _gemm_split(op, A, B, C, M, N, K, lda, ldb, ldc, bias, beta, batch, sA, sB, sC, sBias, a_off, b_off, c_off,
                bias_off):
    if K > 10900:
        return False
    Kp6 = 6 * _pad8(K)
    splits = 1
    if K > SPLIT_MAX_ACC_K:
        if M < 256 or N % 4 != 0:
            return False
        splits = -(-Kp6 // SPLIT_MAX_ACC_K)
        while splits > 1 and M * N * batch * splits * 4 > (1 << 30):
            splits -= 1
    ea = _split_cols(A, a_off, M, K, lda, batch, sA, 0) if op in (OP_NT, OP_NN) else _split_rows(A, a_off, K, M, lda, batch, sA, 0)
    if ea is None:
        return False
    eb = _split_cols(B, b_off, N, K, ldb, batch, sB, 1) if op == OP_NT else _split_rows(B, b_off, K, N, ldb, batch, sB, 1)
    if eb is None:
        return False
    LAUNCHES[0] += 2
    gemm_bf16(op, ea[0], eb[0], M, N, Kp6, ea[1], eb[1], C=C, ldc=ldc, bias=bias, beta=beta, batch=batch,
              sA=ea[2] if batch > 1 else 0, sB=eb[2] if batch > 1 else 0, sC=sC, sBias=sBias, c_off=c_off,
              bias_off=bias_off, splits=splits if splits > 1 else 1, impl="pair" if splits > 1 else None)
    return True


def gemm(op, A, B, C, M, N, K, lda, ldb, ldc, bias=None, beta=0.0, batch=1, sA=0, sB=0, sC=0, sBias=0,
         a_off=0, b_off=0, c_off=0, bias_off=0):
    _req(A); _req(B); _req(C)
    if (FP32_GEMM[0] == "split" and M * N * K * batch >= SPLIT_MIN_MACS and M >= 256 and N >= 16 and K >= 16
            and batch <= 4 and ldc % 4 == 0 and c_off % 4 == 0 and (batch == 1 or sC % 4 == 0)
            and _gemm_split(op, A, B, C, M, N, K, lda, ldb, ldc, bias, beta, batch, sA, sB, sC, sBias, a_off, b_off,
                            c_off, bias_off)):
        return C
    pa = ctypes.c_void_p(A.data_ptr() + 4 * a_off)
    pb = ctypes.c_void_p(B.data_ptr() + 4 * b_off)
    pc = ctypes.c_void_p(C.data_ptr() + 4 * c_off)
# ... 183 lines not shown
GEMM_IMPL = ["auto"]
_SM_PAIRS = 74


def _pick_splits(M, N, K, batch):
    tiles = ((M + 255) // 256) * ((N + 255) // 256) * batch
    kb = (K + 63) // 64
    if tiles * 2 > _SM_PAIRS or kb < 64:
        return 1
    return max(1, min(_SM_PAIRS // tiles, kb // 8, 16))


_g2_ws = {}


def _gemm2_ws(device, nbytes):
    key = (device, torch.cuda.current_stream().cuda_stream)
    ws = _g2_ws.get(key)
    if ws is None or ws.numel() * 4 < nbytes:
        ws = torch.empty(nbytes // 4 + 4, dtype=torch.float32, device=device)
        _g2_ws[key] = ws
    return ws


def gemm_bf16(op, A, B, M, N, K, lda, ldb, C=None, ldc=0, Cb=None, ldcb=0, bias=None, beta=0.0, batch=1,
              sA=0, sB=0, sC=0, sCb=0, sBias=0, a_off=0, b_off=0, c_off=0, cb_off=0, bias_off=0, splits=1,
              impl=None, max_pairs=0):
    _req(A, torch.bfloat16); _req(B, torch.bfloat16)
    impl = impl or GEMM_IMPL[0]
    if impl == "pair" or (impl == "auto" and M >= 256):
        sp = _pick_splits(M, N, K, batch) if splits in (0, 1) else splits
        if sp > 1 and N % 4 != 0:
            sp = 1
        ws, wsb = None, 0
        if sp > 1:
            wsb = lib().sn_gemm2_ws_bytes(M, N, batch, sp)
            ws = _gemm2_ws(A.device, wsb)
            LAUNCHES[0] += batch
        check(lib().sn_gemm2_bf16(op, M, N, K, _bptr(A, a_off, 2), lda, _bptr(B, b_off, 2), ldb,
                                  _bptr(C, c_off, 4), ldc, _bptr(Cb, cb_off, 2), ldcb, _bptr(bias, bias_off, 4),
                                  float(beta), batch, sA, sB, sC, sCb, sBias, sp, _ptr(ws), wsb, int(max_pairs),
                                  _stream()), "sn_gemm2_bf16")
        return
    check(lib().sn_gemm_bf16_splitk(op, M, N, K, _bptr(A, a_off, 2), lda, _bptr(B, b_off, 2), ldb,
                                    _bptr(C, c_off, 4), ldc, _bptr(Cb, cb_off, 2), ldcb, _bptr(bias, bias_off, 4),
                                    float(beta), batch, sA, sB, sC, sCb, sBias, splits, _stream()), "sn_gemm_bf16")


def vocab_nll_fwd(Hb, Wb, bias, targets, N, V, H, tlogit, lse, row_loss=None, argmax=None, above=None):
    _req(Hb, torch.bfloat16); _req(Wb, torch.bfloat16); _req(targets, torch.int64)
    nbytes = lib().sn_vocab_ws_bytes(N, V)
    ws = _gemm2_ws(Hb.device, nbytes)
    check(lib().sn_vocab_nll_fwd(N, V, H, _ptr(Hb), Hb.stride(0), _ptr(Wb), Wb.stride(0), _ptr(_req(bias)),
                                 _ptr(targets), _ptr(ws), nbytes, _ptr(tlogit), _ptr(lse), _ptr(row_loss),
                                 _ptr(argmax), _ptr(above), _stream()), "sn_vocab_nll_fwd")
    LAUNCHES[0] += 1


def vocab_nll_bwd(Hb, Wb, bias, targets, N, V, H, tlogit, lse, grad_scale, dLb=None, above=None, top5hit=None,
                  row_weight=None):
    _req(Hb, torch.bfloat16); _req(Wb, torch.bfloat16); _req(targets, torch.int64)
    check(lib().sn_vocab_nll_bwd(N, V, H, _ptr(Hb), Hb.stride(0), _ptr(Wb), Wb.stride(0), _ptr(_req(bias)),
                                 _ptr(targets), _ptr(tlogit), _ptr(lse), float(grad_scale),
                                 _ptr(None if row_weight is None else _req(row_weight)), _ptr(dLb),
                                 dLb.stride(0) if dLb is not None else 0, _ptr(above), _ptr(top5hit), _stream()),
          "sn_vocab_nll_bwd")
    if top5hit is not None:
        LAUNCHES[0] += 1


def cast_bf16(src, R, C, lds, dst, Cp, ldd, src_off=0, dst_off=0, max_blocks=0):
    check(lib().sn_cast_bf16_ex(_bptr(_req(src), src_off, 4), R, C, lds, _bptr(dst, dst_off, 2), Cp, ldd, max_blocks,
                                _stream()), "sn_cast_bf16")


def to_bf16_padded(x, pad_to=8):
    R, C = x.shape
    Cp = (C + pad_to - 1) // pad_to * pad_to
    out = torch.empty(R, Cp, dtype=torch.bfloat16, device=x.device)
    cast_bf16(x, R, C, x.stride(0), out, Cp, Cp)
    return out


import os as _os
DC_SCHEDULE = [int(_os.environ.get("SN_DC_SCHEDULE", "0"))]
DC_MAX_PAIRS = [int(_os.environ.get("SN_DC_MAX_PAIRS", "37"))]

TAIL_SCHEDULE = [int(_os.environ.get("SN_TAIL_SCHEDULE", "1"))]
ADAM_BG_CTAS = [int(_os.environ.get("SN_ADAM_BG_CTAS", "0"))]

GATE_DC = [int(_os.environ.get("SN_GATE_DC", "0"))]

RECUR_IMPL = ["auto"]
_cl_max = {}


def recur_cluster_ok(H, B):
    impl = RECUR_IMPL[0]
    if impl == "flags" or H not in (128, 256, 512):
        return False
    key = (torch.cuda.current_device(), H)
    n = _cl_max.get(key)
    if n is None:
        n = _cl_max[key] = int(lib().sn_recur_cl_max_clusters(H))
    if impl == "cluster":
        if n < 1:
            raise _lib.SnError("cluster form of the recurrence is not available for H=%d on this device" % H)
        return True
    return n >= 1 and (B + 15) // 16 <= n


def recur_fwd_bf16(cell, H, B, bs, off, t0, t1, XP, Whh_b, bhh, h_init, Hall, Hb, Hprevb, Call, gates, c_state):
    if recur_cluster_ok(H, B):
        check(lib().sn_recur_fwd_cl(cell, H, B, _ptr(bs), _ptr(off), t0, t1, _ptr(_req(XP)),
                                    _ptr(_req(Whh_b, torch.bfloat16)), _ptr(bhh), _ptr(h_init), _ptr(Hall),
                                    _ptr(_req(Hb, torch.bfloat16)), _ptr(Hprevb), _ptr(Call), _ptr(gates),
                                    _ptr(c_state), _stream()), "sn_recur_fwd_cl")
        return
    ws = _recur_ws(XP.device, t1 + 1)
    check(lib().sn_recur_fwd_bf16(cell, H, B, _ptr(bs), _ptr(off), t0, t1, _ptr(_req(XP)),
                                  _ptr(_req(Whh_b, torch.bfloat16)), _ptr(bhh), _ptr(h_init), _ptr(Hall),
                                  _ptr(_req(Hb, torch.bfloat16)), _ptr(Hprevb), _ptr(Call), _ptr(gates),
                                  _ptr(c_state), _ptr(ws), _stream()), "sn_recur_fwd_bf16")


def recur_bwd_bf16(cell, H, B, bs, off, t0, t1, Whh_b, c_init, Call, gates, dHall, dZ, dZb, dh_carry, dc_carry,
                   start_flag=None):
    if recur_cluster_ok(H, B):
        check(lib().sn_recur_bwd_cl(cell, H, B, _ptr(bs), _ptr(off), t0, t1, _ptr(_req(Whh_b, torch.bfloat16)),
                                    _ptr(c_init), _ptr(Call), _ptr(gates), _ptr(_req(dHall)), _ptr(dZ),
                                    _ptr(_req(dZb, torch.bfloat16)), _ptr(dh_carry), _ptr(dc_carry), _ptr(start_flag),
                                    _stream()), "sn_recur_bwd_cl")
        return
    ws = _recur_ws(dZb.device, t1 + 1)
    check(lib().sn_recur_bwd_bf16(cell, H, B, _ptr(bs), _ptr(off), t0, t1, _ptr(_req(Whh_b, torch.bfloat16)),
                                  _ptr(c_init), _ptr(Call), _ptr(gates), _ptr(_req(dHall)), _ptr(dZ),
                                  _ptr(_req(dZb, torch.bfloat16)), _ptr(dh_carry), _ptr(dc_carry), _ptr(ws),
                                  _stream()), "sn_recur_bwd_bf16")


RECUR_GEMM_MIN_BATCH = [1024]


def _host_steps(plan):
    hs = plan.__dict__.get("_host_steps")
    if hs is None:
        T = plan.T
        hs = ((ctypes.c_int32 * T)(*[int(x) for x in plan.bs]), (ctypes.c_int32 * T)(*[int(x) for x in plan.off[:T]]))
        plan.__dict__["_host_steps"] = hs
    return hs


_zeros_b16 = {}


def _zeros_bf16(device, n):
    z = _zeros_b16.get(device)
    if z is None or z.numel() < n:
        z = torch.zeros(n, dtype=torch.bfloat16, device=device)
        _zeros_b16[device] = z
    return z


def cast_gate_interleave(W):
    H4, K = W.shape
    H = H4 // 4
    Kp = (K + 7) // 8 * 8
# ... 285 lines not shown
```

### include/sn100.h

```cpp
#ifndef SN100_H_
#define SN100_H_

#include <stdint.h>

#ifdef __cplusplus
extern "C" {
#endif

#define SN_VERSION 100

#define SN_OP_NT 0
#define SN_OP_NN 1
#define SN_OP_TN 2

#define SN_PREC_F32 0
#define SN_PREC_BF16X6 1
#define SN_PREC_BF16 2

#define SN_CELL_FACTORED 0
#define SN_CELL_LSTM 1

int32_t sn_version(void);
const char* sn_last_error(void);
int32_t sn_device_info(int32_t* sm_count, int32_t* smem_optin, int32_t* cc_major, int32_t* cc_minor);

int32_t sn_gather_pack_fwd(const int64_t* captions, int64_t cap_ld, const float* table, int64_t E,
                           const float* features, int64_t feat_ld, int32_t has_feat,
                           const int32_t* row_b, const int32_t* row_t, const int32_t* tok_override,
                           int64_t N, float* X, int64_t ldx, float p_drop, uint64_t seed,
                           const uint64_t* seed_dev, void* Xb, int64_t ldxb, void* stream);
int32_t sn_gather_pack_bwd(const int64_t* captions, int64_t cap_ld, float* dtable, int64_t E,
                           float* dfeatures, int64_t feat_ld, int32_t has_feat,
                           const int32_t* row_b, const int32_t* row_t, const int32_t* tok_override,
                           int64_t N, const float* dX, int64_t ldx, float p_drop, uint64_t seed,
                           const uint64_t* seed_dev, int64_t V, int32_t* ws_int, float* ws_part, void* stream);
int32_t sn_embed_plan(const int64_t* captions, int64_t cap_ld, int32_t has_feat, const int32_t* row_b,
                      const int32_t* row_t, const int32_t* tok_override, int64_t N, int64_t V, int32_t* ws_int,
                      void* stream);
int32_t sn_embed_grad(float* dtable, int64_t E, float* dfeatures, int64_t feat_ld, int32_t has_feat,
                      const int32_t* row_b, const int32_t* row_t, const int32_t* tok_override, int64_t N,
                      const float* dX, int64_t ldx, float p_drop, uint64_t seed, const uint64_t* seed_dev, int64_t V,
                      const int32_t* ws_int, float* ws_part, int32_t wide, void* stream);

int32_t sn_gemm(int32_t op, int64_t M, int64_t N, int64_t K, const float* A, int64_t lda,
                const float* B, int64_t ldb, float* C, int64_t ldc, const float* bias, float beta,
                int32_t batch, int64_t strideA, int64_t strideB, int64_t strideC, int64_t strideBias,
                void* stream);
int32_t sn_gemm_bf16(int32_t op, int64_t M, int64_t N, int64_t K, const void* A, int64_t lda,
                     const void* B, int64_t ldb, float* C, int64_t ldc, void* Cb, int64_t ldcb,
                     const float* bias, float beta, int32_t batch, int64_t strideA, int64_t strideB,
                     int64_t strideC, int64_t strideCb, int64_t strideBias, void* stream);
int32_t sn_gemm_bf16_splitk(int32_t op, int64_t M, int64_t N, int64_t K, const void* A, int64_t lda,
                            const void* B, int64_t ldb, float* C, int64_t ldc, void* Cb, int64_t ldcb,
                            const float* bias, float beta, int32_t batch, int64_t strideA,
                            int64_t strideB, int64_t strideC, int64_t strideCb, int64_t strideBias,
                            int32_t splits, void* stream);
int64_t sn_gemm2_ws_bytes(int64_t M, int64_t N, int32_t batch, int32_t splits);
int32_t sn_gemm2_bf16(int32_t op, int64_t M, int64_t N, int64_t K, const void* A, int64_t lda,
                      const void* B, int64_t ldb, float* C, int64_t ldc, void* Cb, int64_t ldcb,
                      const float* bias, float beta, int32_t batch, int64_t strideA, int64_t strideB,
                      int64_t strideC, int64_t strideCb, int64_t strideBias, int32_t splits, void* ws,
                      int64_t ws_bytes, int32_t max_pairs, void* stream);
int32_t sn_cast_bf16(const float* src, int64_t R, int64_t C, int64_t lds, void* dst, int64_t Cp,
                     int64_t ldd, void* stream);
int32_t sn_cast_bf16_ex(const float* src, int64_t R, int64_t C, int64_t lds, void* dst, int64_t Cp,
                        int64_t ldd, int32_t max_blocks, void* stream);
int32_t sn_colsum(const float* X, int64_t M, int64_t N, int64_t ldx, float* out, float beta,
                  void* stream);
int32_t sn_colsum_bf16(const void* X, int64_t M, int64_t N, int64_t ldx, float* out, float beta,
                       void* stream);
int32_t sn_colsum_ex(const float* X, int64_t M, int64_t N, int64_t ldx, float* out, float beta, int32_t wide,
                     void* stream);
int32_t sn_colsum_bf16_ex(const void* X, int64_t M, int64_t N, int64_t ldx, float* out, float beta, int32_t wide,
                          void* stream);

int64_t sn_recur_ws_bytes(int64_t B, int64_t T);
int32_t sn_recur_fwd(int32_t cell, int64_t H, int64_t B, const int32_t* batch_sizes,
                     const int32_t* offsets, int32_t t0, int32_t t1, const float* XP,
                     const float* Whh, const float* h_init, const float* bhh, float* Hall,
                     float* Call, float* Hprev, float* gates, float* c_state, void* ws,
                     void* stream);
int32_t sn_recur_bwd(int32_t cell, int64_t H, int64_t B, const int32_t* batch_sizes,
                     const int32_t* offsets, int32_t t0, int32_t t1, const float* Whh,
                     const float* c_init, const float* Call, const float* gates, const float* dHall,
                     float* dZ, float* dh_carry, float* dc_carry, void* ws, void* stream);

int32_t sn_recur_fwd_bf16(int32_t cell, int64_t H, int64_t B, const int32_t* batch_sizes,
                          const int32_t* offsets, int32_t t0, int32_t t1, const float* XP,
                          const void* Whh_bf16, const float* bhh, const float* h_init, float* Hall,
                          void* Hb, void* Hprevb, float* Call, float* gates, float* c_state, void* ws,
                          void* stream);
int32_t sn_recur_bwd_bf16(int32_t cell, int64_t H, int64_t B, const int32_t* batch_sizes,
                          const int32_t* offsets, int32_t t0, int32_t t1, const void* Whh_bf16,
                          const float* c_init, const float* Call, const float* gates,
                          const float* dHall, float* dZ, void* dZb, float* dh_carry, float* dc_carry,
                          void* ws, void* stream);

int32_t sn_recur_cl_max_clusters(int64_t H);
int32_t sn_recur_fwd_cl(int32_t cell, int64_t H, int64_t B, const int32_t* batch_sizes,
                        const int32_t* offsets, int32_t t0, int32_t t1, const float* XP,
                        const void* Whh_bf16, const float* bhh, const float* h_init, float* Hall,
                        void* Hb, void* Hprevb, float* Call, float* gates, float* c_state,
                        void* stream);
int32_t sn_recur_bwd_cl(int32_t cell, int64_t H, int64_t B, const int32_t* batch_sizes,
                        const int32_t* offsets, int32_t t0, int32_t t1, const void* Whh_bf16,
                        const float* c_init, const float* Call, const float* gates,
                        const float* dHall, float* dZ, void* dZb, float* dh_carry, float* dc_carry,
// ... 165 lines not shown
```

Baseline: 4.533 million.

## Enable programmatic dependent launch across custom kernels with fallback

Adds a launch helper that sets the programmatic stream serialization attribute, plus griddepcontrol wait and trigger calls in many kernels (elementwise, embed, adam, gemm2, reductions, recurrent cluster kernels). Each kernel's prologue can then overlap the tail of the previous kernel on the stream, hiding launch gaps. It also preallocates and zeroes the recurrent state buffers on a side stream instead of allocating zeros inline. The risk is placing waits after reads of producer data, and some added launch overhead if the attribute is rejected.

```diff
diff --git a/image-caption-emotion-indonesia_b200/_lib.py b/image-caption-emotion-indonesia_b200/_lib.py
--- a/image-caption-emotion-indonesia_b200/_lib.py
+++ b/image-caption-emotion-indonesia_b200/_lib.py
@@ -15,6 +15,8 @@
     "sn_version": (_I32, []),
     "sn_last_error": (c_char_p, []),
     "sn_device_info": (_I32, [_P, _P, _P, _P]),
+    "sn_set_pdl": (_I32, [_I32]),
+    "sn_pdl_fallbacks": (_I32, []),
     "sn_gather_pack_fwd": (_I32, [_P, _I64, _P, _I64, _P, _I64, _I32, _P, _P, _P, _I64, _P, _I64, _F, c_uint64, _P, _P, _I64, _P]),
     "sn_gather_pack_bwd": (_I32, [_P, _I64, _P, _I64, _P, _I64, _I32, _P, _P, _P, _I64, _P, _I64, _F, c_uint64, _P, _I64, _P, _P, _P]),
     "sn_gemm": (_I32, [_I32, _I64, _I64, _I64, _P, _I64, _P, _I64, _P, _I64, _P, _F, _I32, _I64, _I64, _I64, _I64, _P]),
diff --git a/image-caption-emotion-indonesia_b200/csrc/sn_common.cu b/image-caption-emotion-indonesia_b200/csrc/sn_common.cu
--- a/image-caption-emotion-indonesia_b200/csrc/sn_common.cu
+++ b/image-caption-emotion-indonesia_b200/csrc/sn_common.cu
@@ -4,6 +4,7 @@
 
 #include <cuda.h>
 
+#include <atomic>
 #include <mutex>
 #include <string.h>
 
@@ -55,12 +56,20 @@
   }();
   return coop;
 }
+
+static std::atomic<int> g_pdl{1};
+static std::atomic<int> g_pdl_fallbacks{0};
+bool pdl_enabled() { return g_pdl.load(std::memory_order_relaxed) != 0; }
+void pdl_record_fallback() { g_pdl_fallbacks.fetch_add(1, std::memory_order_relaxed); }
 }
 
 extern "C" {
 
 int32_t sn_version(void) { return SN_VERSION; }
 const char* sn_last_error(void) { return sn::err_buf(); }
+
+int32_t sn_set_pdl(int32_t on) { return sn::g_pdl.exchange(on ? 1 : 0); }
+int32_t sn_pdl_fallbacks(void) { return sn::g_pdl_fallbacks.load(); }
 
 int32_t sn_device_info(int32_t* sm_count, int32_t* smem_optin, int32_t* cc_major, int32_t* cc_minor) {
   int n = 0;
diff --git a/image-caption-emotion-indonesia_b200/csrc/sn_common.cuh b/image-caption-emotion-indonesia_b200/csrc/sn_common.cuh
--- a/image-caption-emotion-indonesia_b200/csrc/sn_common.cuh
+++ b/image-caption-emotion-indonesia_b200/csrc/sn_common.cuh
@@ -19,6 +19,53 @@
 };
 const DevInfo& dev_info();
 bool recur_cooperative();
+
+bool pdl_enabled();
+void pdl_record_fallback();
+
+struct LaunchCfg {
+  dim3 grid, block;
+  size_t smem;
+  cudaStream_t stream;
+  unsigned cluster_x;
+};
+
+template <typename... KArgs, typename... Args>
+cudaError_t launch(const LaunchCfg& c, void (*kernel)(KArgs...), Args... args) {
+  cudaLaunchConfig_t cfg = {};
+  cfg.gridDim = c.grid;
+  cfg.blockDim = c.block;
+  cfg.dynamicSmemBytes = c.smem;
+  cfg.stream = c.stream;
+  cudaLaunchAttribute attr[2];
+  unsigned n = 0;
+  if (c.cluster_x) {
+    attr[n].id = cudaLaunchAttributeClusterDimension;
+    attr[n].val.clusterDim.x = c.cluster_x;
+    attr[n].val.clusterDim.y = 1;
+    attr[n].val.clusterDim.z = 1;
+    ++n;
+  }
+  const unsigned plain = n;
+  if (pdl_enabled()) {
+    attr[n].id = cudaLaunchAttributeProgrammaticStreamSerialization;
+    attr[n].val.programmaticStreamSerializationAllowed = 1;
+    ++n;
+  }
+  cfg.attrs = attr;
+  cfg.numAttrs = n;
+  cudaError_t e = cudaLaunchKernelEx(&cfg, kernel, args...);
+  if (e != cudaSuccess && n != plain) {
+    cudaGetLastError();
+    pdl_record_fallback();
+    cfg.numAttrs = plain;
+    e = cudaLaunchKernelEx(&cfg, kernel, args...);
+  }
+  return e;
+}
+
+__device__ __forceinline__ void pdl_wait() { asm volatile("griddepcontrol.wait;" ::: "memory"); }
+__device__ __forceinline__ void pdl_trigger() { asm volatile("griddepcontrol.launch_dependents;" ::: "memory"); }
 
 #define SN_REQUIRE(cond, ...)                         \
   do {                                                \
diff --git a/image-caption-emotion-indonesia_b200/csrc/sn_elementwise.cu b/image-caption-emotion-indonesia_b200/csrc/sn_elementwise.cu
--- a/image-caption-emotion-indonesia_b200/csrc/sn_elementwise.cu
+++ b/image-caption-emotion-indonesia_b200/csrc/sn_elementwise.cu
@@ -14,6 +14,8 @@
                                        float* __restrict__ X, int64_t ldx, float p, float inv_keep,
                                        uint64_t seed, const uint64_t* __restrict__ seed_dev,
                                        __nv_bfloat16* __restrict__ Xb, int64_t ldxb, int Ep) {
+  sn::pdl_wait();
+  sn::pdl_trigger();
   if (seed_dev) seed += *seed_dev;
   int64_t row = (int64_t)blockIdx.x * (blockDim.x >> 5) + (threadIdx.x >> 5);
   if (row >= N) return;
@@ -183,6 +185,8 @@
     const int32_t* __restrict__ sorted, int64_t V, const int32_t* __restrict__ tok_override,
     const float* __restrict__ dX, int64_t ldx, int E, float p, float inv_keep, uint64_t seed,
     const uint64_t* __restrict__ seed_dev, float* __restrict__ dtable, float* __restrict__ part) {
+  sn::pdl_wait();
+  sn::pdl_trigger();
   __shared__ int32_t rows[EB_CHUNK];
   __shared__ float rate[EB_CHUNK];
   const int64_t i = blockIdx.x;
@@ -222,6 +226,8 @@
 
 __global__ void embed_combine_kernel(const int32_t* __restrict__ cnt, const int32_t* __restrict__ cstart, int64_t V,
                                      int E, const float* __restrict__ part, float* __restrict__ dtable) {
+  sn::pdl_wait();
+  sn::pdl_trigger();
   const int64_t t = (int64_t)blockIdx.x * (blockDim.x >> 5) + (threadIdx.x >> 5);
   if (t >= V || cnt[t] <= EB_CHUNK) return;
   const int lane = threadIdx.x & 31;
@@ -349,6 +355,8 @@
 
 __global__ void adam_prepare_kernel(AdamRanges R, int32_t* __restrict__ steps, const float* __restrict__ lr,
                                     float* __restrict__ coef, float beta1, float beta2) {
+  sn::pdl_wait();
+  sn::pdl_trigger();
   int r = threadIdx.x;
   if (r >= R.n) return;
   int st = steps[R.step_idx[r]] + 1;
@@ -365,6 +373,7 @@
                                                          float* __restrict__ m, float* __restrict__ v,
                                                          AdamRanges R, const float* __restrict__ coef, float beta1,
                                                          float beta2, float eps, float clip) {
+  sn::pdl_wait();
   const int64_t total_chunks = R.chunk_start[R.n];
   for (int64_t ch = blockIdx.x; ch < total_chunks; ch += gridDim.x) {
     int r = 0;
@@ -735,10 +744,9 @@
   if (N == 0) return 0;
   float inv_keep = 1.f / (1.f - p_drop);
   unsigned grid = (unsigned)((N + 7) / 8);
-  gather_pack_fwd_kernel<<<grid, 256, 0, (cudaStream_t)stream>>>(captions, cap_ld, table, (int)E, features, feat_ld,
-                                                                 has_feat, row_b, row_t, tok_override, N, X, ldx,
-                                                                 p_drop, inv_keep, seed, seed_dev,
-                                                                 (__nv_bfloat16*)Xb, ldxb, Xb ? (int)ldxb : (int)E);
+  sn::launch({grid, 256, 0, (cudaStream_t)stream, 0}, gather_pack_fwd_kernel, captions, cap_ld, table, (int)E, features,
+             feat_ld, has_feat, row_b, row_t, tok_override, N, X, ldx, p_drop, inv_keep, seed, seed_dev,
+             (__nv_bfloat16*)Xb, ldxb, Xb ? (int)ldxb : (int)E);
   return sn::check_launch("sn_gather_pack_fwd");
 }
 
@@ -799,14 +807,14 @@
                                                                      dX, ldx, p_drop, inv_keep, seed, seed_dev);
   EmbedWs w(const_cast<int32_t*>(ws_int), V, N);
   if (wide && E <= 512)
-    embed_chunk_wide_kernel<<<(unsigned)N, (unsigned)((E + 31) / 32 * 32), 0, st>>>(
+    sn::launch({(unsigned)N, (unsigned)((E + 31) / 32 * 32), 0, st, 0}, embed_chunk_wide_kernel,
         w.tok32, w.start, w.cstart, w.sorted, V, tok_override, dX, ldx, (int)E, p_drop, inv_keep, seed, seed_dev,
         dtable, ws_part);
   else
     embed_chunk_kernel<<<(unsigned)((N + 7) / 8), 256, 0, st>>>(w.tok32, w.start, w.cstart, w.sorted, V, tok_override,
                                                                  dX, ldx, (int)E, p_drop, inv_keep, seed, seed_dev,
                                                                  dtable, ws_part);
-  embed_combine_kernel<<<(unsigned)((V + 7) / 8), 256, 0, st>>>(w.cnt, w.cstart, V, (int)E, ws_part, dtable);
+  sn::launch({(unsigned)((V + 7) / 8), 256, 0, st, 0}, embed_combine_kernel, w.cnt, w.cstart, V, (int)E, ws_part, dtable);
   return sn::check_launch("sn_embed_grad");
 }
 
@@ -859,7 +867,7 @@
     if (chunks == 0) continue;
     int64_t cap = (int64_t)sn::dev_info().sm_count * 8;
     unsigned grid = (unsigned)(chunks < cap ? chunks : cap);
-    adam_clamp_kernel<<<grid, 256, 0, (cudaStream_t)stream>>>(p, g, m, v, R, nullptr, beta1, beta2, eps, clip);
+    sn::launch({grid, 256, 0, (cudaStream_t)stream, 0}, adam_clamp_kernel, p, g, m, v, R, nullptr, beta1, beta2, eps, clip);
     int32_t rc = sn::check_launch("sn_adam_clamp");
     if (rc) return rc;
   }
@@ -890,13 +898,13 @@
     R.chunk_start[i + 1] = R.chunk_start[i] + (R.len[i] + ADAM_CHUNK - 1) / ADAM_CHUNK;
   }
   cudaStream_t st = (cudaStream_t)stream;
-  adam_prepare_kernel<<<1, AdamRanges::MAX, 0, st>>>(R, steps_dev, lr_dev, coef_ws, beta1, beta2);
+  sn::launch({1, AdamRanges::MAX, 0, st, 0}, adam_prepare_kernel, R, steps_dev, lr_dev, coef_ws, beta1, beta2);
   int64_t chunks = R.chunk_start[R.n];
   if (chunks == 0) return sn::check_launch("sn_adam_clamp_dev");
   int64_t cap = (int64_t)sn::dev_info().sm_count * 8;
   if (max_ctas > 0 && max_ctas < cap) cap = max_ctas;
   unsigned grid = (unsigned)(chunks < cap ? chunks : cap);
-  adam_clamp_kernel<<<grid, 256, 0, st>>>(p, g, m, v, R, coef_ws, beta1, beta2, eps, clip);
+  sn::launch({grid, 256, 0, st, 0}, adam_clamp_kernel, p, g, m, v, R, coef_ws, beta1, beta2, eps, clip);
   return sn::check_launch("sn_adam_clamp_dev");
 }
 
@@ -940,7 +948,7 @@
         (R.len[i] > 0 ? (R.off[i] + R.len[i] - 1) / ADAM_CHUNK - R.off[i] / ADAM_CHUNK + 1 : 0);
   }
   cudaStream_t st = (cudaStream_t)stream;
-  if (n_ranges > 0) adam_prepare_kernel<<<1, AdamRanges::MAX, 0, st>>>(R, steps_dev, lr_dev, coef_ws, beta1, beta2);
+  if (n_ranges > 0) sn::launch({1, AdamRanges::MAX, 0, st, 0}, adam_prepare_kernel, R, steps_dev, lr_dev, coef_ws, beta1, beta2);
   int64_t mine = (R.chunk_start[R.n] + world - 1) / world;
   int64_t cap = (int64_t)sn::dev_info().sm_count * 3;
   unsigned grid = (unsigned)(mine < 1 ? 1 : (mine < cap ? mine : cap));
@@ -1049,7 +1057,7 @@
     R.chunk_start[i + 1] = R.chunk_start[i] + own;
   }
   cudaStream_t st = (cudaStream_t)stream;
-  adam_prepare_kernel<<<1, AdamRanges::MAX, 0, st>>>(R, steps_dev, lr_dev, coef_ws, beta1, beta2);
+  sn::launch({1, AdamRanges::MAX, 0, st, 0}, adam_prepare_kernel, R, steps_dev, lr_dev, coef_ws, beta1, beta2);
   int64_t mine = (R.chunk_start[R.n] + DP_RSUB - 1) / DP_RSUB;
   int64_t cap = (int64_t)sn::dev_info().sm_count * 2;
   if (max_ctas > 0 && max_ctas < cap) cap = max_ctas;
diff --git a/image-caption-emotion-indonesia_b200/csrc/sn_gemm2.cu b/image-caption-emotion-indonesia_b200/csrc/sn_gemm2.cu
--- a/image-caption-emotion-indonesia_b200/csrc/sn_gemm2.cu
+++ b/image-caption-emotion-indonesia_b200/csrc/sn_gemm2.cu
@@ -280,6 +280,7 @@
   cluster_sync();
   tc_fence_after();
   const uint32_t tmem_base = *tmem_slot;
+  sn::pdl_wait();
 
   if (warp == 0) {
     if (lane == 0) {
@@ -311,6 +312,7 @@
           if (++s == STAGES) { s = 0; ph ^= 1; }
         }
       }
+      sn::pdl_trigger();
     }
   } else if (warp == 1) {
     if (rank == 0 && lane == 0) {
@@ -340,6 +342,7 @@
         }
         if (++as == ACC_STAGES) { as = 0; aph ^= 1; }
       }
+      sn::pdl_trigger();
     }
     __syncwarp();
   } else {
@@ -746,6 +749,8 @@
 __global__ void __launch_bounds__(256) splitk_reduce_kernel(const float* __restrict__ ws, int splits, int64_t M, int64_t N,
                                                             float* C, int64_t ldc, __nv_bfloat16* Cb, int64_t ldcb,
                                                             const float* __restrict__ bias, float beta) {
+  sn::pdl_wait();
+  sn::pdl_trigger();
   const int64_t total4 = M * N / 4;
   const int64_t MN = M * N;
   for (int64_t i = (int64_t)blockIdx.x * blockDim.x + threadIdx.x; i < total4; i += (int64_t)gridDim.x * blockDim.x) {
@@ -774,6 +779,8 @@
                                                             const float* __restrict__ tlogit, float* __restrict__ lse,
                                                             float* __restrict__ row_loss, int64_t* __restrict__ argmax,
                                                             int32_t* __restrict__ above) {
+  sn::pdl_wait();
+  sn::pdl_trigger();
   const int lane = threadIdx.x & 31;
   const int64_t row = (int64_t)blockIdx.x * 8 + (threadIdx.x >> 5);
   if (row >= N) return;
@@ -803,6 +810,8 @@
 }
 
 __global__ void rank_hit_kernel(const int32_t* __restrict__ above, int64_t N, int32_t k, int32_t* __restrict__ hit) {
+  sn::pdl_wait();
+  sn::pdl_trigger();
   const int64_t i = (int64_t)blockIdx.x * blockDim.x + threadIdx.x;
   if (i < N) hit[i] = above[i] < k ? 1 : 0;
 }
@@ -872,7 +881,7 @@
   int64_t pairs = sn::dev_info().sm_count / 2;
   if (max_pairs > 0 && max_pairs < pairs) pairs = max_pairs;
   if (tiles < pairs) pairs = tiles;
-  gemm2_kernel<EPI, BN_><<<(unsigned)(2 * pairs), NTHREADS, Geo<BN_>::SMEM_BYTES, st>>>(ta, tb, g);
+  sn::launch({(unsigned)(2 * pairs), NTHREADS, Geo<BN_>::SMEM_BYTES, st, 0}, gemm2_kernel<EPI, BN_>, ta, tb, g);
   return sn::check_launch(what);
 }
 
@@ -927,7 +936,7 @@
     int64_t blocks = (M * N / 4 + 255) / 256;
     int64_t cap = (int64_t)sn::dev_info().sm_count * 8;
     if (blocks > cap) blocks = cap;
-    splitk_reduce_kernel<<<(unsigned)blocks, 256, 0, st>>>(
+    sn::launch({(unsigned)blocks, 256, 0, st, 0}, splitk_reduce_kernel,
         g.ws + (int64_t)gi * splits * M * N, splits, M, N, C ? C + gi * strideC : nullptr, ldc,
         Cb ? (__nv_bfloat16*)Cb + gi * strideCb : nullptr, ldcb, bias ? bias + gi * strideBias : nullptr, beta);
     rc = sn::check_launch("sn_gemm2_bf16(reduce)");
@@ -963,8 +972,8 @@
   cudaStream_t st = (cudaStream_t)stream;
   rc = launch<EPI_STATS>(ta, tb, g, st, "sn_vocab_nll_fwd");
   if (rc) return rc;
-  vocab_combine_kernel<<<(unsigned)((N + 7) / 8), 256, 0, st>>>(g.pmax, g.psum, g.pidx, nchunks, N, tlogit, lse, row_loss,
-                                                               argmax, above);
+  sn::launch({(unsigned)((N + 7) / 8), 256, 0, st, 0}, vocab_combine_kernel, g.pmax, g.psum, g.pidx, nchunks, N, tlogit,
+             lse, row_loss, argmax, above);
   return sn::check_launch("sn_vocab_nll_fwd(combine)");
 }
 
@@ -992,7 +1001,7 @@
   rc = row_weight ? launch<EPI_GRADW>(ta, tb, g, st, "sn_vocab_nll_bwd") : launch<EPI_GRAD>(ta, tb, g, st, "sn_vocab_nll_bwd");
   if (rc) return rc;
   if (top5hit) {
-    rank_hit_kernel<<<(unsigned)((N + 255) / 256), 256, 0, st>>>(above, N, 5, top5hit);
+    sn::launch({(unsigned)((N + 255) / 256), 256, 0, st, 0}, rank_hit_kernel, above, N, 5, top5hit);
     return sn::check_launch("sn_vocab_nll_bwd(top5)");
   }
   return 0;
diff --git a/image-caption-emotion-indonesia_b200/csrc/sn_gemm_tc.cu b/image-caption-emotion-indonesia_b200/csrc/sn_gemm_tc.cu
--- a/image-caption-emotion-indonesia_b200/csrc/sn_gemm_tc.cu
+++ b/image-caption-emotion-indonesia_b200/csrc/sn_gemm_tc.cu
@@ -372,6 +372,7 @@
 namespace {
 __global__ void cast_pad_kernel(const float* __restrict__ src, int64_t R, int64_t Cc, int64_t lds,
                                 __nv_bfloat16* __restrict__ dst, int64_t Cp, int64_t ldd) {
+  sn::pdl_wait();
   const int64_t total = R * Cp;
   for (int64_t i = (int64_t)blockIdx.x * blockDim.x + threadIdx.x; i < total; i += (int64_t)gridDim.x * blockDim.x) {
     int64_t r = i / Cp, c = i - r * Cp;
@@ -379,6 +380,7 @@
   }
 }
 __global__ void cast_vec8_kernel(const float* __restrict__ src, int64_t n8, __nv_bfloat16* __restrict__ dst) {
+  sn::pdl_wait();
   for (int64_t i = (int64_t)blockIdx.x * blockDim.x + threadIdx.x; i < n8; i += (int64_t)gridDim.x * blockDim.x) {
     const float4 a = __ldg(reinterpret_cast<const float4*>(src) + 2 * i);
     const float4 b = __ldg(reinterpret_cast<const float4*>(src) + 2 * i + 1);
@@ -404,12 +406,12 @@
   if (dense) {
     int64_t blocks = (total / 8 + 255) / 256;
     if (blocks > cap) blocks = cap;
-    cast_vec8_kernel<<<(unsigned)blocks, 256, 0, (cudaStream_t)stream>>>(src, total / 8, (__nv_bfloat16*)dst);
+    sn::launch({(unsigned)blocks, 256, 0, (cudaStream_t)stream, 0}, cast_vec8_kernel, src, total / 8, (__nv_bfloat16*)dst);
     return sn::check_launch("sn_cast_bf16");
   }
   int64_t blocks = (total + 255) / 256;
   if (blocks > cap) blocks = cap;
-  cast_pad_kernel<<<(unsigned)blocks, 256, 0, (cudaStream_t)stream>>>(src, R, Cc, lds, (__nv_bfloat16*)dst, Cp, ldd);
+  sn::launch({(unsigned)blocks, 256, 0, (cudaStream_t)stream, 0}, cast_pad_kernel, src, R, Cc, lds, (__nv_bfloat16*)dst, Cp, ldd);
   return sn::check_launch("sn_cast_bf16");
 }
 
diff --git a/image-caption-emotion-indonesia_b200/csrc/sn_recur_cl.cu b/image-caption-emotion-indonesia_b200/csrc/sn_recur_cl.cu
--- a/image-caption-emotion-indonesia_b200/csrc/sn_recur_cl.cu
+++ b/image-caption-emotion-indonesia_b200/csrc/sn_recur_cl.cu
@@ -123,6 +123,16 @@
   const int oct = warp & 3, kq = warp >> 2;
   const int pos_o = a.cell == SN_CELL_LSTM ? 3 : 2, pos_c = a.cell == SN_CELL_LSTM ? 2 : 3;
 
+  int2* tab = reinterpret_cast<int2*>(smem + FwdSmem<H>::tab);
+  for (int i = tid; i < a.t1 - a.t0; i += NTH)
+    tab[i] = make_int2(clampi(a.bs[a.t0 + i] - s0, 0, NS), a.off[a.t0 + i] + s0);
+  if (tid == 0) {
+    mbar_init(bar0, 1);
+    mbar_init(bar0 + 8, 1);
+    asm volatile("fence.mbarrier_init.release.cluster;" ::: "memory");
+  }
+  sn::pdl_wait();
+
   uint32_t Wr[4][KT][2];
   {
     const uint32_t stage = smem_u32(smem);
@@ -152,10 +162,6 @@
   float bh[4];
 #pragma unroll
   for (int g = 0; g < 4; ++g) bh[g] = a.bhh ? __ldg(a.bhh + g * H + ug) : 0.f;
-
-  int2* tab = reinterpret_cast<int2*>(smem + FwdSmem<H>::tab);
-  for (int i = tid; i < a.t1 - a.t0; i += NTH)
-    tab[i] = make_int2(clampi(a.bs[a.t0 + i] - s0, 0, NS), a.off[a.t0 + i] + s0);
   {
     const int p0 = a.t0 & 1;
     for (int i = tid; i < NS * (H / 2); i += NTH) {
@@ -166,11 +172,6 @@
       *reinterpret_cast<__nv_bfloat162*>(hbuf + ((size_t)(p0 ^ 1) * NS + r) * HP + c) = __floats2bfloat162_rn(0.f, 0.f);
     }
   }
-  if (tid == 0) {
-    mbar_init(bar0, 1);
-    mbar_init(bar0 + 8, 1);
-    asm volatile("fence.mbarrier_init.release.cluster;" ::: "memory");
-  }
   cluster_sync();
 
   uint32_t ph0 = 0, ph1 = 0;
@@ -178,6 +179,7 @@
     const int2 tb = tab[t - a.t0];
     const int nv = tb.x;
     if (nv == 0) break;
+    if (t + 1 == a.t1) sn::pdl_trigger();
     const int nvn = (t + 1 < a.t1) ? tab[t + 1 - a.t0].x : 0;
     const int p = t & 1, pn = p ^ 1;
     if (tid == 0 && nvn > 0) mbar_expect_tx(bar0 + 8 * pn, (uint32_t)(CS * nvn * 64));
@@ -315,7 +317,6 @@
   const int fs = warp, fu = lane, gs = s0 + fs, ug = u0 + fu;
   const bool live = gs < a.B;
   const int64_t sidx = (int64_t)gs * H + ug;
-  float dc_reg = live ? a.dc_carry[sidx] : 0.f;
   const int fpos = (((fu >> 4) * 2 + ((fu >> 2) & 1)) * 8) + ((fu >> 3) & 1) * 4 + (fu & 3);
 
   int2* tab = reinterpret_cast<int2*>(smem + BwdSmem<H>::total);
@@ -328,12 +329,15 @@
     mbar_init(bar0 + 8, 1);
     asm volatile("fence.mbarrier_init.release.cluster;" ::: "memory");
   }
+  sn::pdl_wait();
+  float dc_reg = live ? a.dc_carry[sidx] : 0.f;
   cluster_sync();
 
   uint32_t ph0 = 0, ph1 = 0;
   for (int t = a.t1 - 1; t >= a.t0; --t) {
     const int2 tb = tab[t - a.t0];
     const int nv = tb.x;
+    if (t == a.t0) sn::pdl_trigger();
     if (nv == 0) continue;
     const int nrec = (t + 1 < a.t1) ? tab[t + 1 - a.t0].x : 0;
     const int p = t & 1, pr = p ^ 1;
@@ -475,31 +479,30 @@
 
 template <typename Kern>
 int32_t launch_cl(Kern kernel, int CS, size_t smem, const CArgs& a, cudaStream_t stream, const char* what, int* max_clusters) {
-  cudaLaunchConfig_t cfg = {};
   const int nclusters = (a.B + NS - 1) / NS;
-  cfg.gridDim = dim3((unsigned)(nclusters * CS));
-  cfg.blockDim = dim3(NTH);
   smem += (size_t)(a.t1 - a.t0 + 1) * 8;
-  cfg.dynamicSmemBytes = smem;
-  cfg.stream = stream;
-  cudaLaunchAttribute attr[1];
-  attr[0].id = cudaLaunchAttributeClusterDimension;
-  attr[0].val.clusterDim.x = (unsigned)CS;
-  attr[0].val.clusterDim.y = 1;
-  attr[0].val.clusterDim.z = 1;
-  cfg.attrs = attr;
-  cfg.numAttrs = 1;
+  const sn::LaunchCfg lc = {dim3((unsigned)(nclusters * CS)), dim3(NTH), smem, stream, (unsigned)CS};
   SN_CUDA(cudaFuncSetAttribute(kernel, cudaFuncAttributeMaxDynamicSharedMemorySize, (int)smem));
   if (CS > 8) SN_CUDA(cudaFuncSetAttribute(kernel, cudaFuncAttributeNonPortableClusterSizeAllowed, 1));
   if (max_clusters) {
+    cudaLaunchConfig_t cfg = {};
+    cfg.gridDim = lc.grid;
+    cfg.blockDim = lc.block;
+    cfg.dynamicSmemBytes = smem;
+    cudaLaunchAttribute attr[1];
+    attr[0].id = cudaLaunchAttributeClusterDimension;
+    attr[0].val.clusterDim.x = (unsigned)CS;
+    attr[0].val.clusterDim.y = 1;
+    attr[0].val.clusterDim.z = 1;
+    cfg.attrs = attr;
+    cfg.numAttrs = 1;
     int n = 0;
     cudaError_t e = cudaOccupancyMaxActiveClusters(&n, kernel, &cfg);
     if (e != cudaSuccess) { cudaGetLastError(); n = 0; }
     *max_clusters = n;
     return 0;
   }
-  CArgs args = a;
-  cudaError_t e = cudaLaunchKernelEx(&cfg, kernel, args);
+  cudaError_t e = sn::launch(lc, kernel, a);
   if (e != cudaSuccess) return sn::fail((int32_t)e, "%s: cluster launch failed: %s", what, cudaGetErrorString(e));
   return 0;
 }
diff --git a/image-caption-emotion-indonesia_b200/decoders.py b/image-caption-emotion-indonesia_b200/decoders.py
--- a/image-caption-emotion-indonesia_b200/decoders.py
+++ b/image-caption-emotion-indonesia_b200/decoders.py
@@ -244,6 +244,11 @@
             if early:
                 c.ev_early = self._shadows_async(early)
             if late:
+                c.zero_state = torch.empty(3, B, H, dtype=torch.float32, device=dev)
+                side = self._side(2)
+                side.wait_stream(torch.cuda.current_stream())
+                with torch.cuda.stream(side):
+                    c.zero_state.zero_()
                 c.ev_late = self._shadows_async(late)
             self.__dict__["_out_w16_ev"] = self._shadows_async([(self.__dict__, "_out_w16_pref", self._out().weight)])
         if self.bf16:
@@ -261,7 +266,8 @@
         c.Call = torch.empty(N, H, dtype=torch.float32, device=dev) if save else None
         c.Hprev = torch.empty(N, H, dtype=torch.float32, device=dev) if save else None
         c.gates = torch.empty(N, 4 * H, dtype=torch.float32, device=dev) if save else None
-        c_state = torch.zeros(B, H, dtype=torch.float32, device=dev)
+        zs = c.__dict__.get("zero_state")
+        c_state = zs[0] if zs is not None else torch.zeros(B, H, dtype=torch.float32, device=dev)
         c.aux_argmax = None
         Whh, bhh = self._recurrent_weights()
         c.Whh, c.bhh = Whh, bhh
@@ -367,7 +373,8 @@
         L = getattr(cl, "layer", 0)
         Whh, _ = self._recurrent_weights(L)
         dZ = torch.empty(N, 4 * H, dtype=torch.float32, device=dev)
-        dhc = torch.zeros(2, B, H, dtype=torch.float32, device=dev)
+        zs = c.__dict__.get("zero_state") if cl is c else None
+        dhc = zs[1:] if zs is not None else torch.zeros(2, B, H, dtype=torch.float32, device=dev)
         dh, dc = dhc[0], dhc[1]
         gW, gbW = self._recurrent_grads(gbuf, L)
         if cl.Hpb is not None:
diff --git a/image-caption-emotion-indonesia_b200/ops.py b/image-caption-emotion-indonesia_b200/ops.py
--- a/image-caption-emotion-indonesia_b200/ops.py
+++ b/image-caption-emotion-indonesia_b200/ops.py
@@ -1,4 +1,5 @@
 import ctypes
+import os as _os
 
 import torch
 
@@ -49,7 +50,14 @@
 def lib():
     l = _lib.load()
     _lib.require_device(torch.cuda.current_device())
+    if _pdl_sent[0] != PDL[0]:
+        l.sn_set_pdl(PDL[0])
+        _pdl_sent[0] = PDL[0]
     return l
+
+
+PDL = [int(_os.environ.get("SN_PDL", "1"))]
+_pdl_sent = [None]
 
 
 FP32_GEMM = ["split"]
@@ -399,7 +407,6 @@
     return out
 
 
-import os as _os
 DC_SCHEDULE = [int(_os.environ.get("SN_DC_SCHEDULE", "0"))]
 DC_MAX_PAIRS = [int(_os.environ.get("SN_DC_MAX_PAIRS", "37"))]
 
diff --git a/include/sn100.h b/include/sn100.h
--- a/include/sn100.h
+++ b/include/sn100.h
@@ -23,6 +23,8 @@
 int32_t sn_version(void);
 const char* sn_last_error(void);
 int32_t sn_device_info(int32_t* sm_count, int32_t* smem_optin, int32_t* cc_major, int32_t* cc_minor);
+int32_t sn_set_pdl(int32_t on);
+int32_t sn_pdl_fallbacks(void);
 
 int32_t sn_gather_pack_fwd(const int64_t* captions, int64_t cap_ld, const float* table, int64_t E,
                            const float* features, int64_t feat_ld, int32_t has_feat,
diff --git a/profiles/pdl_ab.py b/profiles/pdl_ab.py
--- /dev/null
+++ b/profiles/pdl_ab.py
@@ -0,0 +1,41 @@
+import json, os, statistics, subprocess, sys, tempfile
+import numpy as np
+
+out = sys.argv[1]
+runs = int(sys.argv[2]) if len(sys.argv) > 2 else 5
+arms = {"pdl0": {"SN_PDL": "0"}, "pdl1": {"SN_PDL": "1"}}
+os.makedirs(out, exist_ok=True)
+gpu = subprocess.run(["nvidia-smi", "--query-gpu=name,power.limit,clocks.sm,clocks.max.sm", "--format=csv,noheader"],
+                     capture_output=True, text=True).stdout.strip()
+res = {a: [] for a in arms}
+with open(os.path.join(out, "pdl_ab_runs.jsonl"), "w") as f:
+    for i in range(runs):
+        for a, env in arms.items():
+            p = subprocess.run([sys.executable, "bench.py", "--no-extras", "--no-cpu-baseline"], capture_output=True,
+                               text=True, env=dict(os.environ, **env))
+            line = [l for l in p.stdout.splitlines() if l.startswith("{")][-1]
+            d = json.loads(line)
+            res[a].append(d["ms_per_step"])
+            f.write(json.dumps({"arm": a, "env": env, "run": i, "ms_per_step": d["ms_per_step"],
+                                "clocks": d.get("clocks"), "gpu": gpu}) + "\n")
+            f.flush()
+summary = {"gpu": gpu, "runs_per_arm": runs}
+for a, v in res.items():
+    summary[a] = {"median": statistics.median(v), "min": min(v), "max": max(v), "all": v}
+summary["median_gain_us"] = 1000 * (summary["pdl0"]["median"] - summary["pdl1"]["median"])
+summary["ranges_disjoint"] = summary["pdl1"]["max"] < summary["pdl0"]["min"]
+dumps = {}
+with tempfile.TemporaryDirectory() as td:
+    for a in arms:
+        d = os.path.join(td, a)
+        subprocess.run([sys.executable, "bench.py", "--no-extras", "--no-cpu-baseline", "--steps", "5",
+                        "--dump-outputs", d], capture_output=True, text=True, check=True,
+                       env=dict(os.environ, **arms[a]))
+        dumps[a] = {n: np.load(os.path.join(d, n)) for n in sorted(os.listdir(d)) if n.endswith(".npy")}
+    same = sorted(dumps["pdl0"]) == sorted(dumps["pdl1"]) and all(
+        np.array_equal(dumps["pdl0"][n], dumps["pdl1"][n]) for n in dumps["pdl0"])
+summary["dump_outputs_identical"] = bool(same)
+summary["dump_outputs_files"] = len(dumps["pdl0"])
+print(json.dumps(summary))
+with open(os.path.join(out, "pdl_ab_summary.json"), "w") as f:
+    json.dump(summary, f, indent=1)
```

Measured after the change: 4.555 million, median of 6. No clear change (+0.5%).
